# joeyz0z/ConZIC

Measured on AMD Instinct MI355X. Metric: captions/sec (L=10, K=200, seq order), higher is better.
Workload: dtype bf16

## Files before the change

conzic_amd/csrc/bridge.hip:

```cpp
#include "kernels.h"
#include "bridge_hash.h"

namespace czc {

constexpr int BR_THREADS = 64;
constexpr int BR_MAXB = 512;
constexpr int BR_MAXSYM = 64;
constexpr int BR_LEN = 77;
constexpr int BR_MAXP = 64;

__device__ __forceinline__ bool merge_lookup(const BridgeDev& bd, int l, int r, unsigned& rank, int& out) {
  const unsigned long long key = ((unsigned long long)(unsigned)l << 32) | (unsigned)r;
  unsigned h = bridge_hash(key) & bd.hmask;
  for (;;) {
    const unsigned long long k = bd.hkeys[h];
    if (k == key) {
      const unsigned long long v = bd.hvals[h];
      rank = (unsigned)(v >> 32);
      out = (int)(v & 0xFFFFFFFFu);
      return true;
    }
    if (k == ~0ull) return false;
    h = (h + 1) & bd.hmask;
  }
// ... 90 lines not shown
    if (j == 0) {
      j = i + 1;
      if (c == 0) { while (j < n && (cls[j] & 3) == 0) ++j; }
      else if (c == 1) { while (j < n && !(cls[j] & 4)) ++j; }
      else { while (j < n && (cls[j] & 3) == 2) ++j; }
    }
    if (bd.tok_bpe_len && c == 0) {
      while (pp < np && pl_beg[pp] < i) ++pp;
      if (pp < np && pl_beg[pp] == i && pl_end[pp] == j) {
        const int id = pl_id[pp];
        const int tl = bd.tok_bpe_len[id];
        if (tl) {
          for (int q = 0; q < tl && nt < BR_LEN - 2; ++q) outp[1 + nt++] = bd.tok_bpe[id * BR_TOKMAX + q];
          i = j;
          continue;
        }
      }
    }
    int m = j - i;
    if (m > BR_MAXSYM) { ovf = true; m = BR_MAXSYM; }
    for (int q = 0; q < m; ++q) sym[q] = bd.byte_sym[txt[i + q]];
    sym[m - 1] = bd.byte_sym_eow[txt[i + m - 1]];
    while (m > 1) {
      unsigned best = 0xFFFFFFFFu;
      int bi = -1, bo = 0;
      for (int q = 0; q + 1 < m; ++q) {
        unsigned rk; int o;
        if (merge_lookup(bd, sym[q], sym[q + 1], rk, o) && rk < best) { best = rk; bi = q; bo = o; }
      }
      if (bi < 0) break;
      sym[bi] = bo;
      for (int q = bi + 1; q + 1 < m; ++q) sym[q] = sym[q + 1];
      --m;
    }
    for (int q = 0; q < m && nt < BR_LEN - 2; ++q) outp[1 + nt++] = sym[q];
    i = j;
  }
  outp[1 + nt] = bd.eos_id;
  for (int q = nt + 2; q < BR_LEN; ++q) outp[q] = bd.eos_id;
  clip_len[row] = nt + 2;
  if (pos.tag_of_token) {
    for (int w = n_words; w < pos.n; ++w) pos_ok += (pos.masks[w] & 0x8000u) ? 1 : 0;
    if (senti_raw) senti_raw[row] = (float)pos_ok / (float)pos.n;
  } else if (senti_raw) {
    senti_raw[row] = negative ? -senti : senti;
  }
  if (repeats) repeats[row] = (float)(rep - 1);
  if (ovf) atomicAdd(overflow, 1);
}

__global__ void bridge_precompute_kernel(BridgeDev bd, int* tok_ids, uint8_t* tok_len) {
  const int id = blockIdx.x * blockDim.x + threadIdx.x;
  if (id >= bd.bert_vocab) return;
  tok_len[id] = 0;
  const unsigned o0 = bd.piece_off[id], o1 = bd.piece_off[id + 1];
  int m = (int)(o1 - o0);
  if (m <= 0 || m > BR_MAXSYM || (bd.piece_flags[id] & 1u)) return;
  for (unsigned o = o0; o < o1; ++o)
    if ((bd.piece_class[o] & 3) != 0) return;
  int sym[BR_MAXSYM];
  for (int q = 0; q < m; ++q) sym[q] = bd.byte_sym[bd.piece_bytes[o0 + q]];
  sym[m - 1] = bd.byte_sym_eow[bd.piece_bytes[o0 + m - 1]];
  while (m > 1) {
    unsigned best = 0xFFFFFFFFu;
    int bi = -1, bo = 0;
    for (int q = 0; q + 1 < m; ++q) {
      unsigned rk; int o;
      if (merge_lookup(bd, sym[q], sym[q + 1], rk, o) && rk < best) { best = rk; bi = q; bo = o; }
    }
    if (bi < 0) break;
    sym[bi] = bo;
    for (int q = bi + 1; q + 1 < m; ++q) sym[q] = sym[q + 1];
    --m;
  }
  if (m > BR_TOKMAX) return;
  for (int q = 0; q < m; ++q) tok_ids[id * BR_TOKMAX + q] = sym[q];
  tok_len[id] = (uint8_t)m;
}

int launch_bridge_precompute(const BridgeDev& bd, int* tok_ids, uint8_t* tok_len, hipStream_t st) {
  hipLaunchKernelGGL(bridge_precompute_kernel, dim3(cdiv(bd.bert_vocab, 64)), dim3(64), 0, st, bd, tok_ids, tok_len);
  CZC_HIP_CHECK(hipGetLastError());
  return 0;
}

template <bool ROWS, bool HP>
static int launch_bridge_t(const BridgeDev& bd, const int* inp, int B, int T, int gen_idx, const int* gen_rows, const int* row_len, const int* cand, int K,
                           const float* lexicon, const float* lex_pos, const uint8_t* lex_cls, int negative, const RowHyper* hp_rows, const PosDev& pos,
                           int* clip_ids, int* clip_len, float* senti_raw, float* repeats, int* overflow_flag, hipStream_t st) {
  const long rows = (long)B * K;
  if (rows <= 0) return 0;
  const size_t shmem = (size_t)BR_THREADS * (2 * BR_MAXB + BR_MAXSYM * 4 + BR_MAXP * 8);
  CZC_HIP_CHECK(hipFuncSetAttribute((const void*)bridge_kernel<ROWS, HP>, hipFuncAttributeMaxDynamicSharedMemorySize, (int)shmem));
  hipLaunchKernelGGL((bridge_kernel<ROWS, HP>), dim3(cdiv(rows, BR_THREADS)), dim3(BR_THREADS), shmem, st, bd, inp, B, T, gen_idx, gen_rows,
                     row_len, cand, K, lexicon, lex_pos, lex_cls, negative, hp_rows, pos, clip_ids, clip_len, senti_raw, repeats, overflow_flag);
  CZC_HIP_CHECK(hipGetLastError());
  return 0;
}

int launch_bridge(const BridgeDev& bd, const int* inp, int B, int T, int gen_idx, const int* cand, int K,
                  const float* lexicon, const float* lex_pos, const uint8_t* lex_cls, int negative, const PosDev& pos, int* clip_ids, int* clip_len, float* senti_raw,
                  float* repeats, int* overflow_flag, hipStream_t st) {
  return launch_bridge_t<false, false>(bd, inp, B, T, gen_idx, nullptr, nullptr, cand, K, lexicon, lex_pos, lex_cls, negative, nullptr, pos, clip_ids, clip_len,
                                senti_raw, repeats, overflow_flag, st);
}

int launch_bridge_rows(const BridgeDev& bd, const int* inp, int B, int T, const int* gen_rows, const int* cand, int K,
                       const float* lexicon, const float* lex_pos, const uint8_t* lex_cls, int negative, const PosDev& pos, int* clip_ids, int* clip_len,
                       float* senti_raw, float* repeats, int* overflow_flag, hipStream_t st, const int* row_len) {
  if (!gen_rows || !cand) { snprintf(g_err, sizeof(g_err), "bridge: the per-row form needs gen_rows and cand"); return 1; }
  return launch_bridge_t<true, false>(bd, inp, B, T, 0, gen_rows, row_len, cand, K, lexicon, lex_pos, lex_cls, negative, nullptr, pos, clip_ids, clip_len,
                               senti_raw, repeats, overflow_flag, st);
}

int launch_bridge_rows_hp(const BridgeDev& bd, const int* inp, int B, int T, const int* gen_rows, const int* cand, int K,
                          const float* lexicon, const float* lex_pos, const uint8_t* lex_cls, const RowHyper* hp_rows, const PosDev& pos,
                          int* clip_ids, int* clip_len, float* senti_raw, float* repeats, int* overflow_flag, hipStream_t st,
                          const int* row_len) {
  if (!gen_rows || !cand || !hp_rows) { snprintf(g_err, sizeof(g_err), "bridge: the per-row form needs gen_rows, cand and hp_rows"); return 1; }
  return launch_bridge_t<true, true>(bd, inp, B, T, 0, gen_rows, row_len, cand, K, lexicon, lex_pos, lex_cls, 0, hp_rows, pos, clip_ids, clip_len,
                                     senti_raw, repeats, overflow_flag, st);
}

__global__ __launch_bounds__(1024) void scan_kernel(const int* len, int n, int* off, int* totals) {
  __shared__ int part[1024];
  __shared__ int pmax[1024];
  const int tid = threadIdx.x;
  const int per = (n + 1023) / 1024;
  const int lo = tid * per, hi = min(n, lo + per);
  int s = 0, mx = 0;
  for (int i = lo; i < hi; ++i) { s += len[i]; mx = max(mx, len[i]); }
  part[tid] = s;
  pmax[tid] = mx;
  __syncthreads();
  for (int o = 1; o < 1024; o <<= 1) {
    const int v = tid >= o ? part[tid - o] : 0;
    const int w = tid >= o ? pmax[tid - o] : 0;
    __syncthreads();
    part[tid] += v;
    pmax[tid] = max(pmax[tid], w);
    __syncthreads();
  }
  int run = part[tid] - s;
  for (int i = lo; i < hi; ++i) { off[i] = run; run += len[i]; }
  if (tid == 1023) { off[n] = part[1023]; totals[0] = part[1023]; totals[1] = pmax[1023]; }
}

int launch_scan(const int* len, int n, int* off, int* totals, hipStream_t st) {
  hipLaunchKernelGGL(scan_kernel, dim3(1), dim3(1024), 0, st, len, n, off, totals);
  CZC_HIP_CHECK(hipGetLastError());
  return 0;
}

__global__ __launch_bounds__(256) void prefix_plan_kernel(const int* cids, const int* clen, int B, int K, int share,
                                                          int* own_len, int* pre_len, int* seg_src, int* seg_pos0,
                                                          int* max_len_out, int* img_max, int* rep, int* n_dup_out) {
  __shared__ int s_p, s_max, s_keys, s_dup;
  __shared__ unsigned long long s_hash[1024];
  __shared__ short s_len[1024];
  const int b = blockIdx.x, tid = threadIdx.x;
  if (tid == 0) { s_p = 1 << 30; s_max = 0; s_keys = 0; s_dup = 0; }
  __syncthreads();
  const int* r0 = cids + (long)b * K * BR_LEN;
  const int l0 = clen[b * K];
  int p = 1 << 30, mx = 0;
  for (int k = tid; k < K; k += blockDim.x) {
    const int* rk = r0 + (long)k * BR_LEN;
    const int lk = clen[b * K + k];
    const int lim = min(lk, l0);
    int c = 0;
    while (c < lim && rk[c] == r0[c]) ++c;
    p = min(p, min(c, lk - 1));
    mx = max(mx, lk);
    if (rep) {
      unsigned long long h = 1469598103934665603ull ^ (unsigned)lk;
      for (int c2 = 0; c2 < lk; ++c2) { h ^= (unsigned)rk[c2]; h *= 1099511628211ull; }
      s_hash[k] = h;
      s_len[k] = (short)lk;
    }
  }
  atomicMin(&s_p, p);
  atomicMax(&s_max, mx);
  __syncthreads();
  const int pb = share ? s_p : 0;
  if (tid == 0) {
    own_len[b] = pb; pre_len[b] = 0; seg_src[b] = b * K; seg_pos0[b] = 0;
    atomicMax(max_len_out, s_max);
    atomicMax(max_len_out + 1, s_max - pb);
    if (img_max) img_max[b] = s_max - pb;
  }
  int keys = 0;
  int dups = 0;
  for (int k = tid; k < K; k += blockDim.x) {
    const int s = B + b * K + k;
    const int lk = clen[b * K + k];
    int own = lk - pb;
    if (rep) {
      int r = k;
      const unsigned long long hk = s_hash[k];
      const int* rk = r0 + (long)k * BR_LEN;
      for (int j = 0; j < k; ++j) {
        if (s_hash[j] != hk || s_len[j] != lk) continue;
        const int* rj = r0 + (long)j * BR_LEN;
        int c = pb;
        while (c < lk && rj[c] == rk[c]) ++c;
        if (c == lk) { r = j; break; }
      }
      rep[b * K + k] = r;
      if (r != k) { own = 0; ++dups; }
    }
    own_len[s] = own;
    pre_len[s] = pb;
    seg_src[s] = b * K + k;
    seg_pos0[s] = pb;
    keys += own * pb + own * (own + 1) / 2;
  }
  atomicAdd(&s_keys, keys);
  if (dups) atomicAdd(&s_dup, dups);
  __syncthreads();
  if (tid == 0) {
    atomicAdd(max_len_out + 4, s_keys + pb * (pb + 1) / 2);
    if (n_dup_out && s_dup) atomicAdd(n_dup_out, s_dup);
  }
}

int launch_prefix_plan(const int* clip_ids, const int* clip_len, int B, int K, int share, int* own_len, int* pre_len,
                       int* seg_src, int* seg_pos0, int* max_len_out, int* img_max, hipStream_t st, int* rep, int* n_dup_out) {
  if (rep && K > 1024) { snprintf(g_err, sizeof(g_err), "prefix plan: de-duplication needs K <= 1024"); return 1; }
  hipLaunchKernelGGL(prefix_plan_kernel, dim3(B), dim3(256), 0, st, clip_ids, clip_len, B, K, share, own_len, pre_len,
                     seg_src, seg_pos0, max_len_out, img_max, rep, n_dup_out);
  CZC_HIP_CHECK(hipGetLastError());
  return 0;
}

__global__ void prefix_finish_kernel(const int* own_off, const int* own_len, int B, int K, int* pre_off, int* eos_idx,
                                     int* n_trunk_rows, const int* rep) {
  const int i = blockIdx.x * blockDim.x + threadIdx.x;
  if (i == 0 && n_trunk_rows) *n_trunk_rows = own_off[B];
  if (i < B) pre_off[i] = 0;
  if (i < B * K) {
    const int s = B + i;
    pre_off[s] = own_off[i / K];
    const int sr = rep ? B + (i / K) * K + rep[i] : s;
    eos_idx[i] = own_off[sr] + own_len[sr] - 1;
  }
}

int launch_prefix_finish(const int* own_off, const int* own_len, int B, int K, int* pre_off, int* eos_idx,
                         int* n_trunk_rows, hipStream_t st, const int* rep) {
  hipLaunchKernelGGL(prefix_finish_kernel, dim3(cdiv((long)B * K, 256)), dim3(256), 0, st, own_off, own_len, B, K,
                     pre_off, eos_idx, n_trunk_rows, rep);
  CZC_HIP_CHECK(hipGetLastError());
  return 0;
}

__device__ __forceinline__ int layer0_rep(const int* cid, const int* own, int pb, int k, int i) {
  const int id = cid[(long)k * BR_LEN + pb + i];
  for (int j = 0; j < k; ++j)
    if (own[j] > i && cid[(long)j * BR_LEN + pb + i] == id) return j;
  return k;
}

__global__ __launch_bounds__(256) void layer0_count_kernel(const int* cids, const int* own_len, const int* pre_len, int B, int K,
                                                           int* dcount, int* total) {
  __shared__ int s_n;
  const int b = blockIdx.x;
  if (threadIdx.x == 0) s_n = 0;
  __syncthreads();
  const int* cid = cids + (long)b * K * BR_LEN;
  const int* own = own_len + B + b * K;
  const int pb = pre_len[B + b * K];
  int n = 0;
  for (int k = threadIdx.x; k < K; k += blockDim.x)
    for (int i = 0; i < min(own[k], 32); ++i) n += layer0_rep(cid, own, pb, k, i) == k;
  if (n) atomicAdd(&s_n, n);
  __syncthreads();
  if (threadIdx.x == 0) { dcount[b] = s_n; if (s_n) atomicAdd(total, s_n); }
}

int launch_layer0_count(const int* clip_ids, const int* own_len, const int* pre_len, int B, int K, int* dcount, int* total, hipStream_t st) {
  hipLaunchKernelGGL(layer0_count_kernel, dim3(B), dim3(256), 0, st, clip_ids, own_len, pre_len, B, K, dcount, total);
  CZC_HIP_CHECK(hipGetLastError());
  return 0;
}

__global__ __launch_bounds__(256) void layer0_map_kernel(const int* cids, const int* own_off, const int* own_len, const int* pre_len,
                                                         const int* dcount, int B, int K, int* rowmap, int* dist) {
  __shared__ unsigned s_mask[1024];
  __shared__ int s_pref[1024];
  __shared__ int s_base;
  const int b = blockIdx.x;
  if (threadIdx.x == 0) s_base = own_off[B];
  __syncthreads();
  {
    int n = 0;
    for (int j = threadIdx.x; j < b; j += blockDim.x) n += dcount[j];
    if (n) atomicAdd(&s_base, n);
  }
  for (int r = own_off[b] + threadIdx.x; r < own_off[b] + own_len[b]; r += blockDim.x) { rowmap[r] = r; dist[r] = r; }
  const int* cid = cids + (long)b * K * BR_LEN;
  const int* own = own_len + B + b * K;
  const int* off = own_off + B + b * K;
  const int pb = pre_len[B + b * K];
  for (int k = threadIdx.x; k < K; k += blockDim.x) {
    unsigned m = 0;
    for (int i = 0; i < min(own[k], 32); ++i) m |= (unsigned)(layer0_rep(cid, own, pb, k, i) == k) << i;
    s_mask[k] = m;
  }
  __syncthreads();
  if (threadIdx.x == 0) {
    int run = 0;
    for (int k = 0; k < K; ++k) { s_pref[k] = run; run += __popc(s_mask[k]); }
  }
  __syncthreads();
  const int base = s_base;
  for (int k = threadIdx.x; k < K; k += blockDim.x) {
    for (int i = 0; i < min(own[k], 32); ++i) {
      const int j = (s_mask[k] >> i) & 1 ? k : layer0_rep(cid, own, pb, k, i);
      const int c = base + s_pref[j] + __popc(s_mask[j] & ((1u << i) - 1u));
      rowmap[off[k] + i] = c;
      if (j == k) dist[c] = off[k] + i;
    }
  }
}

int launch_layer0_map(const int* clip_ids, const int* own_off, const int* own_len, const int* pre_len, const int* dcount, int B, int K,
                      int* rowmap, int* dist, hipStream_t st) {
  if (K > 1024) { snprintf(g_err, sizeof(g_err), "layer-0 row map: K <= 1024"); return 1; }
  hipLaunchKernelGGL(layer0_map_kernel, dim3(B), dim3(256), 0, st, clip_ids, own_off, own_len, pre_len, dcount, B, K, rowmap, dist);
  CZC_HIP_CHECK(hipGetLastError());
  return 0;
}

__global__ __launch_bounds__(256) void refine_plan_kernel(const int* clen, const int* trunk_len, const int* list, const int* count,
                                                          const int* count_off, const int* kr, int B, int K, int* own_len, int* pre_len,
                                                          int* seg_src, int* seg_pos0, int* rlist, int* max_len_out, int* img_max) {
  __shared__ int s_mxb;
  const int b = blockIdx.x, tid = threadIdx.x;
  if (tid == 0) s_mxb = 0;
  __syncthreads();
  const int n = count[b], o = count_off[b], Kr = *kr;
  const int pb = n > 0 ? trunk_len[b] : 0;
  if (tid == 0) { own_len[b] = pb; pre_len[b] = 0; seg_src[b] = b * K; seg_pos0[b] = 0; }
  int mx = 0, mxb = 0;
  for (int i = tid; i < Kr; i += blockDim.x) {
    const int s = B + b * Kr + i;
    if (i >= n) {
      pre_len[s] = pb; seg_src[s] = b * K; seg_pos0[s] = pb;
      continue;
    }
    const int flat = b * K + list[(long)b * K + i];
    const int len = clen[flat];
    own_len[s] = len - pb;
    pre_len[s] = pb;
    seg_src[s] = flat;
    seg_pos0[s] = pb;
    rlist[o + i] = flat;
    mx = max(mx, len);
    mxb = max(mxb, len - pb);
    atomicAdd(max_len_out + 4, (len - pb) * pb + (len - pb) * (len - pb + 1) / 2);
  }
  if (tid == 0 && n > 0) atomicAdd(max_len_out + 4, pb * (pb + 1) / 2);
  if (mx) { atomicMax(max_len_out, mx); atomicMax(max_len_out + 1, mxb); atomicMax(&s_mxb, mxb); }
  __syncthreads();
  if (tid == 0 && img_max) img_max[b] = s_mxb;
}

int launch_refine_plan(const int* clip_len, const int* trunk_len, const int* list, const int* count, const int* count_off,
                       const int* kr_dev, int B, int K, int* own_len, int* pre_len, int* seg_src, int* seg_pos0, int* rlist,
                       int* max_len_out, int* img_max, hipStream_t st) {
  hipLaunchKernelGGL(refine_plan_kernel, dim3(B), dim3(256), 0, st, clip_len, trunk_len, list, count, count_off, kr_dev, B, K, own_len,
                     pre_len, seg_src, seg_pos0, rlist, max_len_out, img_max);
  CZC_HIP_CHECK(hipGetLastError());
  return 0;
}

__global__ void refine_finish_kernel(const int* own_off, const int* own_len, const int* count, const int* count_off, const int* kr,
                                     int B, int* pre_off, int* eos_idx) {
  const int i = blockIdx.x * blockDim.x + threadIdx.x;
  const int Kr = *kr;
  if (i < B) pre_off[i] = 0;
  if (i < B * Kr) {
    const int b = i / Kr, j = i - b * Kr;
    const int s = B + i;
    pre_off[s] = own_off[b];
    if (j < count[b]) eos_idx[count_off[b] + j] = own_off[s] + own_len[s] - 1;
  }
}

int launch_refine_finish(const int* own_off, const int* own_len, const int* count, const int* count_off, const int* kr_dev, int B, int K,
                         int* pre_off, int* eos_idx, hipStream_t st) {
  hipLaunchKernelGGL(refine_finish_kernel, dim3(cdiv((long)B * K, 256)), dim3(256), 0, st, own_off, own_len, count, count_off, kr_dev, B,
                     pre_off, eos_idx);
  CZC_HIP_CHECK(hipGetLastError());
  return 0;
}

}
```

conzic_amd/csrc/engine.hip:

```cpp
#include <algorithm>
#include <map>
#include <string>
#include <vector>
#include <cmath>
#include <cstddef>
#include <cstring>

#include "../../include/conzic_hip.h"
#include "kernels.h"
#include "bridge_hash.h"

namespace czc {
thread_local char g_err[512] = {0};
thread_local int g_gemm_family = 0;
}
using namespace czc;

namespace {

struct Tensor {
  float* p = nullptr;
  std::vector<int64_t> shape;
  size_t numel = 0;
};

struct LayerW {
  void* qkv_w = nullptr; float* qkv_b = nullptr;
  void* o_w = nullptr; float* o_b = nullptr;
  float *ln1_g = nullptr, *ln1_b = nullptr;
  void* fc1_w = nullptr; float* fc1_b = nullptr;
  void* fc2_w = nullptr; float* fc2_b = nullptr;
  float *ln2_g = nullptr, *ln2_b = nullptr;
  void *qkv_wf = nullptr, *fc1_wf = nullptr;
  float *qkv_bf = nullptr, *fc1_bf = nullptr;
};

struct Buf {
  void* p = nullptr;
  size_t bytes = 0;
};

struct ProfKind {
  std::vector<hipEvent_t> ev;
  size_t used = 0;
  double flops = 0;
  int64_t launches = 0;
};

struct RowRecords {
  const RowHyper* hp = nullptr;
  const RowDraw* draw = nullptr; unsigned step = 0;
  const int* rival = nullptr; const float* delta = nullptr; int M = 0;
  const float* img_all = nullptr; int n_img = 0;
  const int* vset = nullptr; const unsigned* vbits = nullptr; int vwords = 0; const RowHyper* vhp = nullptr;
};

}

struct czc_engine {
  czc_config cfg;
  int dev = 0;
  hipStream_t st = nullptr;
  bool shares_weights = false;
  hipEvent_t prof_ref = nullptr;
  char err[512] = {0};
  bool finalized = false;
  size_t esz = 2;
  int pb = PREC_F32, pc = PREC_BF16;
  int pv = PREC_BF16;
  size_t eb = 4;
  bool refine = false;
  float refine_theta_x = 2.0f;
  float refine_theta_gen = 4.0f;
  bool in_generate = false;
  int refine_samples = 12;
  int refine_samples_step = 24;
  float refine_guard_dev = 2.0e-4f;
  float guard_max_dev = 0.f; int64_t guard_trips = 0;
  float refine_gate_delta = 4.0e-4f;
  int refine_rows16 = 1;
  float refine_rows16_factor = 1.75f;
  bool gate_now = false, gate_need_cos = true;
  int64_t stat_gated = 0, stat_gate_images = 0;

  std::map<std::string, Tensor> w;
  std::vector<LayerW> bert, ctext, cvis, ctext_x;
  void* mlm_dense_w = nullptr; void* decoder_w = nullptr; void* tproj_w = nullptr; void* vproj_w = nullptr;
  void* patch_w = nullptr; void* tproj_wx = nullptr;

  std::map<std::string, Buf> ws;
  float* d_mask = nullptr; int mask_vocab = 0;
  float* d_lex = nullptr;
  float* d_lex_pos = nullptr; uint8_t* d_lex_cls = nullptr;
  uint8_t* d_pos_tags = nullptr; uint16_t* d_pos_masks = nullptr; int pos_n = 0;
  BridgeDev bd; bool has_bridge = false;
  std::vector<void*> bridge_allocs;
  float* d_img_n = nullptr; int img_B = 0;
  float logit_scale_exp = 1.f;
  double plan_pairs = 0;
  int* h_totals = nullptr;
  int last_BT = 0, last_B = 0, last_T = 0;
  int bert_prune = 1;
  int bert_pruned_idx = -1;
  const int32_t* bert_pruned_rows = nullptr;
  int bert_fuse_splitk_ln = 1;
  int share_prefix = 1;
  int dedup = 1;
  float* d_staged = nullptr; int staged_cap = 0, staged_n = 0;
  int pack_branches = 1;
  int pool_last_layer = 1;
  int share_layer0 = 1;
  int pool_last_qkv = 1;
  int fuse_ln = 1;
  int resid16 = 1;
  int fold_ln = 1;
  int prof = 0;
  std::map<std::string, ProfKind> pk;
  int64_t stat_clip_rows = 0, stat_clip_seqs = 0, stat_bert_rows = 0, stat_steps = 0;
  int64_t stat_refine_rows = 0, stat_refine_seqs = 0;
  int64_t stat_dedup_seqs = 0;
  czc_control_fn ctl_fn = nullptr; void* ctl_user = nullptr;
  int32_t* h_ctl_ids = nullptr; float* h_ctl_scores = nullptr; size_t h_ctl_cap = 0;
  int memo = 0;
  RowRecords rec;
  int memo_branch_floor = 0;
  int64_t stat_memo_hits = 0, stat_memo_images = 0;
  int memo_rows = 0;
  int64_t stat_memo_row_hits = 0, stat_memo_row_steps = 0;
  int32_t* h_memo_list = nullptr; size_t h_memo_list_cap = 0;
  split_t* d_index = nullptr; int64_t index_n = 0;
  int index_groups = 0;
  int fluency_chunk = 1024;
  int regions_chunk = 64;
};

namespace {

constexpr int PRUNED_ROWS = 1 << 30;

#define E_CHECK(expr)                                                                         \
  do {                                                                                        \
    int _r = (expr);                                                                          \
    if (_r) {                                                                                 \
      if (!e->err[0]) snprintf(e->err, sizeof(e->err), "%s", czc::g_err);                     \
      return _r;                                                                              \
    }                                                                                         \
  } while (0)

#define E_HIP(expr)                                                                           \
  do {                                                                                        \
    hipError_t _h = (expr);                                                                   \
    if (_h != hipSuccess) {                                                                   \
      snprintf(e->err, sizeof(e->err), "%s:%d %s -> %s", __FILE__, __LINE__, #expr,           \
               hipGetErrorString(_h));                                                        \
      return CZC_ERR_HIP;                                                                     \
    }                                                                                         \
  } while (0)

int fail(czc_engine* e, int code, const char* fmt, const char* a = "") {
  snprintf(e->err, sizeof(e->err), fmt, a);
  return code;
}

int ensure(czc_engine* e, const char* name, size_t bytes, void** out) {
  Buf& b = e->ws[name];
  if (b.bytes < bytes) {
    if (b.p) {
      E_HIP(hipStreamSynchronize(e->st));
      E_HIP(hipFree(b.p));
    }
    size_t want = bytes + bytes / 4 + 256;
    E_HIP(hipMalloc(&b.p, want));
    b.bytes = want;
  }
  *out = b.p;
  return 0;
}

struct ProfScope {
  czc_engine* e;
  ProfKind* k = nullptr;
  ProfScope(czc_engine* e_, const char* kind, double flops) : e(e_) {
    if (!e->prof) return;
    if (e->prof == 2 && strncmp(kind, "gemm_clip_text", 14) != 0 && strcmp(kind, "gemm_clip_refine") != 0 &&
        !strstr(kind, "_clip_text")) return;
    k = &e->pk[kind];
    if (k->used + 2 > k->ev.size()) {
      for (int i = 0; i < 2; ++i) {
        hipEvent_t ev;
        if (hipEventCreate(&ev) != hipSuccess) { k = nullptr; return; }
        k->ev.push_back(ev);
      }
    }
    k->flops += flops;
    k->launches += 1;
    (void)hipEventRecord(k->ev[k->used], e->st);
  }
  ~ProfScope() {
    if (!k) return;
    (void)hipEventRecord(k->ev[k->used + 1], e->st);
    k->used += 2;
  }
};

const Tensor* find(czc_engine* e, const std::string& n) {
  auto it = e->w.find(n);
  return it == e->w.end() ? nullptr : &it->second;
}

int need(czc_engine* e, const std::string& n, size_t numel, float** out) {
  const Tensor* t = find(e, n);
  if (!t) return fail(e, CZC_ERR_STATE, "missing tensor %s", n.c_str());
  if (t->numel != numel) return fail(e, CZC_ERR_STATE, "tensor %s has the wrong size", n.c_str());
  *out = t->p;
  return 0;
}

int to_act(czc_engine* e, int prec, const float* src, size_t numel, void** out) {
  void* p = nullptr;
  E_HIP(hipMalloc(&p, numel * prec_bytes(prec)));
  E_CHECK(launch_convert(prec, src, p, (long)numel, e->st));
  *out = p;
  return 0;
}

int build_layers(czc_engine* e, std::vector<LayerW>& L, int n_layers, int H, int I, bool bert_style,
                 const std::string& prefix, int prec) {
  const size_t es = prec_bytes(prec);
  L.resize(n_layers);
  for (int n = 0; n < n_layers; ++n) {
    LayerW& l = L[n];
    std::string p = prefix + std::to_string(n);
    std::string q, k, v, o, ln1, fc1, fc2, ln2;
    if (bert_style) {
      q = p + ".attention.self.query"; k = p + ".attention.self.key"; v = p + ".attention.self.value";
      o = p + ".attention.output.dense"; ln1 = p + ".attention.output.LayerNorm";
      fc1 = p + ".intermediate.dense"; fc2 = p + ".output.dense"; ln2 = p + ".output.LayerNorm";
    } else {
      q = p + ".self_attn.q_proj"; k = p + ".self_attn.k_proj"; v = p + ".self_attn.v_proj";
      o = p + ".self_attn.out_proj"; ln1 = p + ".layer_norm1";
      fc1 = p + ".mlp.fc1"; fc2 = p + ".mlp.fc2"; ln2 = p + ".layer_norm2";
    }
    float *qw, *kw, *vw, *qb, *kb, *vb, *t;
    E_CHECK(need(e, q + ".weight", (size_t)H * H, &qw));
    E_CHECK(need(e, k + ".weight", (size_t)H * H, &kw));
    E_CHECK(need(e, v + ".weight", (size_t)H * H, &vw));
    E_CHECK(need(e, q + ".bias", H, &qb));
    E_CHECK(need(e, k + ".bias", H, &kb));
    E_CHECK(need(e, v + ".bias", H, &vb));
    E_HIP(hipMalloc(&l.qkv_w, (size_t)3 * H * H * es));
    char* base = (char*)l.qkv_w;
    E_CHECK(launch_convert(prec, qw, base, (long)H * H, e->st));
    E_CHECK(launch_convert(prec, kw, base + (size_t)H * H * es, (long)H * H, e->st));
    E_CHECK(launch_convert(prec, vw, base + (size_t)2 * H * H * es, (long)H * H, e->st));
    E_HIP(hipMalloc((void**)&l.qkv_b, (size_t)3 * H * 4));
    E_HIP(hipMemcpyAsync(l.qkv_b, qb, (size_t)H * 4, hipMemcpyDeviceToDevice, e->st));
    E_HIP(hipMemcpyAsync(l.qkv_b + H, kb, (size_t)H * 4, hipMemcpyDeviceToDevice, e->st));
    E_HIP(hipMemcpyAsync(l.qkv_b + 2 * H, vb, (size_t)H * 4, hipMemcpyDeviceToDevice, e->st));
    E_CHECK(need(e, o + ".weight", (size_t)H * H, &t)); E_CHECK(to_act(e, prec, t, (size_t)H * H, &l.o_w));
    E_CHECK(need(e, o + ".bias", H, &l.o_b));
    E_CHECK(need(e, ln1 + ".weight", H, &l.ln1_g)); E_CHECK(need(e, ln1 + ".bias", H, &l.ln1_b));
    E_CHECK(need(e, fc1 + ".weight", (size_t)I * H, &t)); E_CHECK(to_act(e, prec, t, (size_t)I * H, &l.fc1_w));
    E_CHECK(need(e, fc1 + ".bias", I, &l.fc1_b));
    E_CHECK(need(e, fc2 + ".weight", (size_t)H * I, &t)); E_CHECK(to_act(e, prec, t, (size_t)H * I, &l.fc2_w));
    E_CHECK(need(e, fc2 + ".bias", H, &l.fc2_b));
    E_CHECK(need(e, ln2 + ".weight", H, &l.ln2_g)); E_CHECK(need(e, ln2 + ".bias", H, &l.ln2_b));
  }
  return 0;
}

int gemm(czc_engine* e, int prec, const char* kind, const void* A, int lda, const void* W, int ldw, const float* bias,
         const float* resid, int ldr, void* out_act, float* out_f32, int ldc, int M, int N, int K, int act) {
  GemmArgs g;
  g.A = A; g.lda = lda; g.W = W; g.ldw = ldw; g.bias = bias; g.resid = resid; g.ldr = ldr;
  g.out_act = out_act; g.out_f32 = out_f32; g.ldc = ldc; g.M = M; g.N = N; g.K = K; g.act = act;
  ProfScope ps(e, kind, 2.0 * M * (double)N * K);
  E_CHECK(launch_gemm(prec, g, e->st));
  return 0;
}

int gemm_x16(czc_engine* e, int prec, const char* kind, const void* A, int lda, const void* W, const float* bias, void* x16, int M,
             int N, int K, float* part = nullptr, long part_ld = 0) {
  GemmArgs g;
  g.A = A; g.lda = lda; g.W = W; g.ldw = K; g.bias = bias; g.resid = (const float*)x16; g.ldr = N;
  g.out_act = nullptr; g.out_f32 = (float*)x16; g.ldc = N; g.M = M; g.N = N; g.K = K; g.act = ACT_NONE; g.x16 = 1;
  g.row_part = part; g.part_ld = part_ld;
  ProfScope ps(e, kind, 2.0 * M * (double)N * K);
  E_CHECK(launch_gemm(prec, g, e->st));
  return 0;
}

int gemm_ex(czc_engine* e, int prec, const char* kind, const GemmArgs& g) {
  ProfScope ps(e, kind, 2.0 * g.M * (double)g.N * g.K);
  E_CHECK(launch_gemm(prec, g, e->st));
  return 0;
}

struct Layer0Rows { const int* rowmap = nullptr; const int* dist = nullptr; int n = 0; };

int clip_stack(czc_engine* e, int P, const char* gk, std::vector<LayerW>& L, float* x, int M, int H, int I, int heads,
               float eps, const SegTable& tab, int max_keys, int causal, int plan_B = 0, int plan_K = 0,
               int plan_max_own = 0, const int* pool_idx = nullptr, int n_pool = 0, float** pooled = nullptr, bool r16 = false,
               const float* ln_stat0 = nullptr, const Layer0Rows& l0 = Layer0Rows(), const int* pool_rep = nullptr) {
  const size_t esz = prec_bytes(P);
  void *y, *qkv, *ctx, *hbuf;
  E_CHECK(ensure(e, "cs_y", (size_t)M * H * esz, &y));
  E_CHECK(ensure(e, "cs_qkv", (size_t)M * 3 * H * esz, &qkv));
  E_CHECK(ensure(e, "cs_ctx", (size_t)M * H * esz, &ctx));
  E_CHECK(ensure(e, "cs_h", (size_t)M * I * esz, &hbuf));
  const float scale = 1.0f / sqrtf(64.0f);
  const bool text = !strcmp(gk, "gemm_clip_text") || !strcmp(gk, "gemm_clip_refine");
  const char* ak = text ? "attention_clip_text" : "attention";
  const char* rk = text ? "rowops_clip_text" : "rowops";
  const double attn_flops = text ? 4.0 * H * e->plan_pairs : 0.0;
  const bool rowln = !r16 && prec_is_half(P) && e->fuse_ln && H == 512 && M >= g_rowln_min_m && I % 32 == 0;
  const bool fold = r16 && e->fold_ln && !L.empty() && L[0].qkv_wf && ln_stat0;
  float *part = nullptr, *stat = nullptr;
  if (fold) {
    E_CHECK(ensure(e, "cs_part", (size_t)(H / 32) * M * 8, (void**)&part));
    E_CHECK(ensure(e, "cs_stat", (size_t)M * 8 + 256, (void**)&stat));
  }
  auto finalize = [&](int rows, int N) -> int {
    if (gemm_wreg_stats_in_kernel(rows, N)) return 0;
    ProfScope ps(e, rk, 0);
    E_CHECK(launch_ln_finalize(part, M, H / 32, rows, eps, stat, e->st));
    return 0;
  };
  auto folded_gemm = [&](const void* Ax, const void* Wf, const float* bf, const float* st_, void* out, int rows, int N,
                         int act, int ldc = 0) -> int {
    GemmArgs g;
    g.A = Ax; g.lda = H; g.W = Wf; g.ldw = H; g.bias = bf; g.resid = nullptr; g.ldr = 0; g.out_act = out; g.out_f32 = nullptr; g.ldc = ldc ? ldc : N;
    g.M = rows; g.N = N; g.K = H; g.act = act;
    g.ln_stat = st_ ? st_ : stat;
    if (!st_ && gemm_wreg_stats_in_kernel(rows, N)) { g.ln_part = part; g.ln_part_ld = M; g.ln_eps = eps; }
    ProfScope ps(e, gk, 2.0 * rows * (double)N * H);
    E_CHECK(launch_gemm(P, g, e->st));
    return 0;
  };
  auto ln = [&](const float* gm, const float* bt, int rows, const void* src, void* dst) -> int {
    ProfScope ps(e, rk, 0);
    if (r16) E_CHECK(launch_layernorm_x16(P, src, nullptr, gm, bt, eps, rows, H, dst, e->st));
    else E_CHECK(launch_layernorm(P, (const float*)src, nullptr, gm, bt, eps, rows, H, dst, nullptr, e->st));
    return 0;
  };
  auto resid_gemm = [&](const void* A, int lda, const void* W, const float* b, int K) -> int {
    if (r16) return gemm_x16(e, P, gk, A, lda, W, b, x, M, H, K);
    return gemm(e, P, gk, A, lda, W, K, b, x, H, nullptr, x, H, M, H, K, ACT_NONE);
  };
  auto resid_ln_gemm = [&](const void* A, int lda, const void* W, const float* b, int K, const float* gm,
                           const float* bt) -> int {
    GemmArgs g;
    g.A = A; g.lda = lda; g.W = W; g.ldw = K; g.bias = b; g.resid = x; g.ldr = H; g.out_act = y; g.out_f32 = x;
    g.ldc = H; g.M = M; g.N = H; g.K = K; g.act = ACT_NONE; g.f16 = P == PREC_F16;
    g.ln_gamma = gm; g.ln_beta = bt; g.ln_eps = eps;
    ProfScope ps(e, gk, 2.0 * M * (double)H * K);
    E_CHECK(launch_gemm_rowln(g, e->st));
    return 0;
  };
  const bool pool_qkv = pool_idx && e->pool_last_layer && e->pool_last_qkv && fold && plan_B > 0 && n_pool == plan_B * plan_K &&
                        prec_is_half(P) && g_use_mfma_attention && e->pack_branches &&
                        attention_image_serves(plan_B, plan_K, plan_max_own, max_keys, heads);
  bool have_y = false;
  for (size_t n = 0; n < L.size(); ++n) {
    LayerW& l = L[n];
    if (pool_qkv && n + 1 == L.size()) {
      void *ctx_e, *q_e, *h_e; float *x_e, *stat_e;
      E_CHECK(ensure(e, "cs_ctx_e", (size_t)n_pool * H * esz, &ctx_e));
      E_CHECK(ensure(e, "cs_q_e", (size_t)n_pool * H * esz, &q_e));
      E_CHECK(ensure(e, "cs_h_e", (size_t)n_pool * I * esz, &h_e));
      E_CHECK(ensure(e, "cs_x_e", (size_t)n_pool * H * 4, (void**)&x_e));
      E_CHECK(ensure(e, "cs_stat_e", (size_t)n_pool * 8 + 256, (void**)&stat_e));
      const float* st_all = n == 0 ? ln_stat0 : stat;
      { ProfScope ps(e, rk, 0);
        E_CHECK(launch_gather_rows_bytes(x, pool_idx, n_pool, H * 2, x_e, e->st));
        E_CHECK(launch_gather_rows_w32(st_all, pool_idx, n_pool, 2, stat_e, e->st)); }
      E_CHECK(folded_gemm(x, (const char*)l.qkv_wf + (size_t)H * H * 2, l.qkv_bf + H, st_all, (char*)qkv + (size_t)H * esz, M, 2 * H,
                          ACT_NONE, 3 * H));
      E_CHECK(folded_gemm(x_e, l.qkv_wf, l.qkv_bf, stat_e, q_e, n_pool, H, ACT_NONE));
      { ProfScope ps(e, ak, attn_flops);
        E_CHECK(launch_attention_image_pooled(qkv, q_e, tab, pool_rep, plan_B, plan_K, plan_max_own, max_keys, heads, scale, ctx_e,
                                              e->st, P == PREC_F16)); }
      E_CHECK(gemm_x16(e, P, gk, ctx_e, H, l.o_w, l.o_b, x_e, n_pool, H, H, part, M));
      E_CHECK(finalize(n_pool, I));
      E_CHECK(folded_gemm(x_e, l.fc1_wf, l.fc1_bf, nullptr, h_e, n_pool, I, ACT_QUICK_GELU));
      E_CHECK(gemm_x16(e, P, gk, h_e, I, l.fc2_w, l.fc2_b, x_e, n_pool, H, I));
      *pooled = x_e;
      return 0;
    }
    const bool l0_rows = fold && n == 0 && l0.n > 0;
    if (l0_rows) {
      void* xg; float* sg;
      E_CHECK(ensure(e, "cs_xg", (size_t)l0.n * H * 2, &xg));
      E_CHECK(ensure(e, "cs_sg", (size_t)l0.n * 8 + 256, (void**)&sg));
      { ProfScope ps(e, rk, 0);
        E_CHECK(launch_gather_rows_bytes(x, l0.dist, l0.n, H * 2, xg, e->st));
        E_CHECK(launch_gather_rows_w32(ln_stat0, l0.dist, l0.n, 2, sg, e->st)); }
      E_CHECK(folded_gemm(xg, l.qkv_wf, l.qkv_bf, sg, qkv, l0.n, 3 * H, ACT_NONE));
    } else if (fold) {
      E_CHECK(folded_gemm(x, l.qkv_wf, l.qkv_bf, n == 0 ? ln_stat0 : nullptr, qkv, M, 3 * H, ACT_NONE));
    } else {
      if (!have_y) E_CHECK(ln(l.ln1_g, l.ln1_b, M, x, y));
      E_CHECK(gemm(e, P, gk, y, H, l.qkv_w, H, l.qkv_b, nullptr, 0, qkv, nullptr, 3 * H, M, 3 * H, H, ACT_NONE));
    }
    { ProfScope ps(e, ak, attn_flops);
      int rc = -1;
      if (l0_rows)
        rc = launch_attention_shared_mapped(qkv, l0.n, l0.rowmap, tab, plan_B, plan_K, plan_max_own, max_keys, heads, scale, ctx, e->st,
                                            P == PREC_F16);
      else if (plan_B > 0 && prec_is_half(P) && g_use_mfma_attention && e->pack_branches)
        rc = launch_attention_shared(qkv, tab, plan_B, plan_K, plan_max_own, max_keys, heads, scale, ctx, e->st, P == PREC_F16);
      else if (plan_B > 0 && P == PREC_F16X3 && g_use_mfma_attention && e->pack_branches)
        rc = launch_attention_shared_split(qkv, tab, plan_B, plan_K, plan_max_own, max_keys, heads, scale, ctx, e->st);
      if (rc > 0) E_CHECK(rc);
      if (rc < 0) E_CHECK(launch_attention(P, qkv, tab, max_keys, heads, causal, scale, ctx, e->st)); }
    if (pool_idx && n + 1 == L.size() && e->pool_last_layer) {
      void *ctx_e, *y_e, *h_e; float* x_e;
      E_CHECK(ensure(e, "cs_ctx_e", (size_t)n_pool * H * esz, &ctx_e));
      E_CHECK(ensure(e, "cs_y_e", (size_t)n_pool * H * esz, &y_e));
      E_CHECK(ensure(e, "cs_h_e", (size_t)n_pool * I * esz, &h_e));
      E_CHECK(ensure(e, "cs_x_e", (size_t)n_pool * H * 4, (void**)&x_e));
      { ProfScope ps(e, rk, 0);
        E_CHECK(launch_gather_rows_bytes(ctx, pool_idx, n_pool, H * (int)esz, ctx_e, e->st));
        if (r16) E_CHECK(launch_gather_rows_bytes(x, pool_idx, n_pool, H * 2, x_e, e->st));
        else E_CHECK(launch_gather_rows_f32(x, pool_idx, n_pool, H, x_e, e->st)); }
      if (fold) {
        E_CHECK(gemm_x16(e, P, gk, ctx_e, H, l.o_w, l.o_b, x_e, n_pool, H, H, part, M));
        E_CHECK(finalize(n_pool, I));
        E_CHECK(folded_gemm(x_e, l.fc1_wf, l.fc1_bf, nullptr, h_e, n_pool, I, ACT_QUICK_GELU));
      } else {
        if (r16) E_CHECK(gemm_x16(e, P, gk, ctx_e, H, l.o_w, l.o_b, x_e, n_pool, H, H));
        else E_CHECK(gemm(e, P, gk, ctx_e, H, l.o_w, H, l.o_b, x_e, H, nullptr, x_e, H, n_pool, H, H, ACT_NONE));
        E_CHECK(ln(l.ln2_g, l.ln2_b, n_pool, x_e, y_e));
        E_CHECK(gemm(e, P, gk, y_e, H, l.fc1_w, H, l.fc1_b, nullptr, 0, h_e, nullptr, I, n_pool, I, H, ACT_QUICK_GELU));
      }
      if (r16) E_CHECK(gemm_x16(e, P, gk, h_e, I, l.fc2_w, l.fc2_b, x_e, n_pool, H, I));
      else E_CHECK(gemm(e, P, gk, h_e, I, l.fc2_w, I, l.fc2_b, x_e, H, nullptr, x_e, H, n_pool, H, I, ACT_NONE));
      *pooled = x_e;
      return 0;
    }
    if (fold) {
      E_CHECK(gemm_x16(e, P, gk, ctx, H, l.o_w, l.o_b, x, M, H, H, part, M));
      E_CHECK(finalize(M, I));
      E_CHECK(folded_gemm(x, l.fc1_wf, l.fc1_bf, nullptr, hbuf, M, I, ACT_QUICK_GELU));
      const bool more = n + 1 < L.size();
      E_CHECK(gemm_x16(e, P, gk, hbuf, I, l.fc2_w, l.fc2_b, x, M, H, I, more ? part : nullptr, M));
      if (more && pool_qkv && n + 2 == L.size()) {
        ProfScope ps(e, rk, 0);
        E_CHECK(launch_ln_finalize(part, M, H / 32, M, eps, stat, e->st));
      } else if (more) E_CHECK(finalize(M, 3 * H));
      continue;
    }
    if (rowln) E_CHECK(resid_ln_gemm(ctx, H, l.o_w, l.o_b, H, l.ln2_g, l.ln2_b));
    else {
      E_CHECK(resid_gemm(ctx, H, l.o_w, l.o_b, H));
      E_CHECK(ln(l.ln2_g, l.ln2_b, M, x, y));
    }
    E_CHECK(gemm(e, P, gk, y, H, l.fc1_w, H, l.fc1_b, nullptr, 0, hbuf, nullptr, I, M, I, H, ACT_QUICK_GELU));
    have_y = rowln && e->fuse_ln >= 2 && n + 1 < L.size();
    if (have_y) E_CHECK(resid_ln_gemm(hbuf, I, l.fc2_w, l.fc2_b, I, L[n + 1].ln1_g, L[n + 1].ln1_b));
    else E_CHECK(resid_gemm(hbuf, I, l.fc2_w, l.fc2_b, I));
  }
  return 0;
}

struct Ragged { const int* off; const int* len; int M; int max_T; };

int bert_forward(czc_engine* e, const int* d_inp, int B, int T, int keep_idx = -1, const int* keep_rows = nullptr,
                 const int32_t* keep_rows_host = nullptr, const Ragged* rag = nullptr) {
  const czc_config& c = e->cfg;
  const int P = e->pb, M = rag ? rag->M : B * T, H = c.bert_hidden, I = c.bert_inter;
  if (rag && keep_idx >= 0 && !keep_rows) return fail(e, CZC_ERR_STATE, "ragged BERT rows keep a row per sequence (keep_rows)%s");
  void *xa, *qkv, *ctx, *hbuf; float *x, *tmp;
  E_CHECK(ensure(e, "b_x", (size_t)M * H * 4, (void**)&x));
  E_CHECK(ensure(e, "b_tmp", (size_t)M * H * 4, (void**)&tmp));
  E_CHECK(ensure(e, "b_xa", (size_t)M * H * e->eb, &xa));
  E_CHECK(ensure(e, "b_qkv", (size_t)M * 3 * H * e->eb, &qkv));
  E_CHECK(ensure(e, "b_ctx", (size_t)M * H * e->eb, &ctx));
  E_CHECK(ensure(e, "b_h", (size_t)M * I * e->eb, &hbuf));
  float *word, *pos, *typ, *g, *b;
  E_CHECK(need(e, "bert.embeddings.word_embeddings.weight", (size_t)c.bert_vocab * H, &word));
  E_CHECK(need(e, "bert.embeddings.position_embeddings.weight", (size_t)c.bert_max_pos * H, &pos));
  E_CHECK(need(e, "bert.embeddings.token_type_embeddings.weight", (size_t)2 * H, &typ));
  E_CHECK(need(e, "bert.embeddings.LayerNorm.weight", H, &g));
  E_CHECK(need(e, "bert.embeddings.LayerNorm.bias", H, &b));
  { ProfScope ps(e, "rowops", 0);
    if (rag) E_CHECK(launch_bert_embed_ragged(P, d_inp, T, nullptr, rag->off, rag->len, B, rag->max_T, H, word, pos, typ, g, b, c.bert_eps, xa, x, e->st));
    else E_CHECK(launch_bert_embed(P, d_inp, B, T, H, word, pos, typ, g, b, c.bert_eps, xa, x, e->st)); }
  const float scale = 1.0f / sqrtf(64.0f);
  e->bert_pruned_idx = -1;
  e->bert_pruned_rows = nullptr;
  auto fc2_ln = [&](const void* h, LayerW& l, float* xr, int rows) -> int {
    SplitkPending pend;
    GemmArgs g;
    g.A = h; g.lda = I; g.W = l.fc2_w; g.ldw = I; g.bias = l.fc2_b; g.resid = xr; g.ldr = H; g.out_act = nullptr; g.out_f32 = tmp; g.ldc = H;
    g.M = rows; g.N = H; g.K = I; g.act = ACT_NONE;
    g.splitk_pending = e->bert_fuse_splitk_ln ? &pend : nullptr;
    E_CHECK(gemm_ex(e, P, "gemm_bert", g));
    ProfScope ps(e, "rowops", 0);
    if (pend.nslab > 0) E_CHECK(launch_layernorm_splitk(P, pend, l.fc2_b, xr, H, l.ln2_g, l.ln2_b, c.bert_eps, rows, H, xa, xr, e->st));
    else E_CHECK(launch_layernorm(P, tmp, nullptr, l.ln2_g, l.ln2_b, c.bert_eps, rows, H, xa, xr, e->st));
    return 0;
  };
  for (int n = 0; n < c.bert_layers; ++n) {
    LayerW& l = e->bert[n];
    E_CHECK(gemm(e, P, "gemm_bert", xa, H, l.qkv_w, H, l.qkv_b, nullptr, 0, qkv, nullptr, 3 * H, M, 3 * H, H, ACT_NONE));
    { ProfScope ps(e, "attention", 0);
      SegTable tab{nullptr, nullptr, rag ? rag->off : nullptr, rag ? rag->len : nullptr, B, rag ? 0 : T};
      E_CHECK(launch_attention(P, qkv, tab, rag ? rag->max_T : T, c.bert_heads, 0, scale, ctx, e->st)); }
    if (keep_idx >= 0 && n + 1 == c.bert_layers) {
      int* idx; void* ctx_g; float* x_g;
      E_CHECK(ensure(e, "b_pidx", (size_t)B * 4, (void**)&idx));
      E_CHECK(ensure(e, "b_cg", (size_t)B * H * e->eb, &ctx_g));
      E_CHECK(ensure(e, "b_xg", (size_t)B * H * 4, (void**)&x_g));
      { ProfScope ps(e, "rowops", 0);
        if (rag) E_CHECK(launch_ragged_row_index(idx, B, rag->off, keep_rows, e->st));
        else if (keep_rows) E_CHECK(launch_make_row_index_rows(idx, B, T, keep_rows, e->st));
        else E_CHECK(launch_make_row_index(idx, B, T, keep_idx, e->st));
        E_CHECK(launch_gather_rows_bytes(ctx, idx, B, H * (int)e->eb, ctx_g, e->st));
        E_CHECK(launch_gather_rows_f32(x, idx, B, H, x_g, e->st)); }
      E_CHECK(gemm(e, P, "gemm_bert", ctx_g, H, l.o_w, H, l.o_b, x_g, H, nullptr, tmp, H, B, H, H, ACT_NONE));
      { ProfScope ps(e, "rowops", 0); E_CHECK(launch_layernorm(P, tmp, nullptr, l.ln1_g, l.ln1_b, c.bert_eps, B, H, xa, x_g, e->st)); }
      E_CHECK(gemm(e, P, "gemm_bert", xa, H, l.fc1_w, H, l.fc1_b, nullptr, 0, hbuf, nullptr, I, B, I, H, ACT_GELU_ERF));
      E_CHECK(fc2_ln(hbuf, l, x_g, B));
      e->bert_pruned_idx = keep_rows ? PRUNED_ROWS : keep_idx;
      e->bert_pruned_rows = keep_rows ? keep_rows_host : nullptr;
      break;
    }
    E_CHECK(gemm(e, P, "gemm_bert", ctx, H, l.o_w, H, l.o_b, x, H, nullptr, tmp, H, M, H, H, ACT_NONE));
    { ProfScope ps(e, "rowops", 0); E_CHECK(launch_layernorm(P, tmp, nullptr, l.ln1_g, l.ln1_b, c.bert_eps, M, H, xa, x, e->st)); }
    E_CHECK(gemm(e, P, "gemm_bert", xa, H, l.fc1_w, H, l.fc1_b, nullptr, 0, hbuf, nullptr, I, M, I, H, ACT_GELU_ERF));
    E_CHECK(fc2_ln(hbuf, l, x, M));
  }
  return 0;
}

int mlm_head(czc_engine* e, int B, int T, int gen_idx, float** logits_out, const int* gen_rows = nullptr,
             const int32_t* gen_rows_host = nullptr, const Ragged* rag = nullptr) {
  const czc_config& c = e->cfg;
  const int P = e->pb, H = c.bert_hidden, V = c.bert_vocab;
  float* x = (float*)e->ws["b_x"].p;
  int* idx; float *gx, *t32, *logits; void *ga, *ta;
  E_CHECK(ensure(e, "h_idx", (size_t)B * 4, (void**)&idx));
  E_CHECK(ensure(e, "h_gx", (size_t)B * H * 4, (void**)&gx));
  E_CHECK(ensure(e, "h_ga", (size_t)B * H * e->eb, &ga));
  E_CHECK(ensure(e, "h_t32", (size_t)B * H * 4, (void**)&t32));
  E_CHECK(ensure(e, "h_ta", (size_t)B * H * e->eb, &ta));
  E_CHECK(ensure(e, "b_logits", (size_t)B * V * 4, (void**)&logits));
  float *db, *g, *b, *bias;
  E_CHECK(need(e, "cls.predictions.transform.dense.bias", H, &db));
  E_CHECK(need(e, "cls.predictions.transform.LayerNorm.weight", H, &g));
  E_CHECK(need(e, "cls.predictions.transform.LayerNorm.bias", H, &b));
  E_CHECK(need(e, "cls.predictions.bias", V, &bias));
  const bool kept_same = gen_rows ? (e->bert_pruned_idx == PRUNED_ROWS && e->bert_pruned_rows && gen_rows_host &&
                                     !memcmp(e->bert_pruned_rows, gen_rows_host, (size_t)B * 4))
                                  : e->bert_pruned_idx == gen_idx;
  if (e->bert_pruned_idx >= 0 && !kept_same)
    return fail(e, CZC_ERR_STATE, "n_mask=0 re-use of a forward that kept one row only (it follows an n_mask >= 2 step, gen_utils.py:164-166)%s");
  { ProfScope ps(e, "rowops", 0);
    if (e->bert_pruned_idx >= 0) {
      gx = (float*)e->ws["b_xg"].p;
    } else {
      if (rag && !gen_rows) return fail(e, CZC_ERR_STATE, "ragged BERT rows are read by a row per sequence (gen_rows)%s");
      if (rag) E_CHECK(launch_ragged_row_index(idx, B, rag->off, gen_rows, e->st));
      else if (gen_rows) E_CHECK(launch_make_row_index_rows(idx, B, T, gen_rows, e->st));
      else E_CHECK(launch_make_row_index(idx, B, T, gen_idx, e->st));
      E_CHECK(launch_gather_rows_f32(x, idx, B, H, gx, e->st));
    }
    E_CHECK(launch_convert(P, gx, ga, (long)B * H, e->st)); }
  E_CHECK(gemm(e, P, "gemm_bert", ga, H, e->mlm_dense_w, H, db, nullptr, 0, nullptr, t32, H, B, H, H, ACT_GELU_ERF));
  { ProfScope ps(e, "rowops", 0); E_CHECK(launch_layernorm(P, t32, nullptr, g, b, c.bert_eps, B, H, ta, nullptr, e->st)); }
  E_CHECK(gemm(e, P, "gemm_bert", ta, H, e->decoder_w, H, bias, nullptr, 0, nullptr, logits, V, B, V, H, ACT_NONE));
  *logits_out = logits;
  return 0;
}

constexpr int HT_PLAN = 48;
constexpr int PLAN_TOTALS = 48;
struct PlanBufs { int *own_len, *pre_len, *src, *pos0, *own_off, *pre_off, *eidx, *img_max, *rep; };

static inline bool refine_rows16_now(const czc_engine* e) {
  return e->refine && e->in_generate && e->refine_rows16 && e->cfg.clip_hidden == 512;
}

int plan_bufs(czc_engine* e, int B, int K, PlanBufs* p, const char* pfx = "p") {
  const int n_seq = B * K, S = B + n_seq;
  const std::string q(pfx);
  E_CHECK(ensure(e, (q + "_own_len").c_str(), (size_t)S * 4, (void**)&p->own_len));
  E_CHECK(ensure(e, (q + "_pre_len").c_str(), (size_t)S * 4, (void**)&p->pre_len));
  E_CHECK(ensure(e, (q + "_src").c_str(), (size_t)S * 4, (void**)&p->src));
  E_CHECK(ensure(e, (q + "_pos0").c_str(), (size_t)S * 4, (void**)&p->pos0));
  E_CHECK(ensure(e, (q + "_own_off").c_str(), (size_t)(S + 1) * 4, (void**)&p->own_off));
  E_CHECK(ensure(e, (q + "_pre_off").c_str(), (size_t)S * 4, (void**)&p->pre_off));
  E_CHECK(ensure(e, (q + "_eidx").c_str(), (size_t)n_seq * 4, (void**)&p->eidx));
  E_CHECK(ensure(e, (q + "_img_max").c_str(), (size_t)B * 4, (void**)&p->img_max));
  E_CHECK(ensure(e, (q + "_rep").c_str(), (size_t)n_seq * 4, (void**)&p->rep));
  return 0;
}

int clip_plan(czc_engine* e, const int* cids, const int* clen, int B, int K, int share, int* totals) {
  PlanBufs p;
  E_CHECK(plan_bufs(e, B, K, &p));
  const int S = B + B * K;
  { ProfScope ps(e, "bridge", 0);
    int* rep = e->dedup && share && K > 1 ? p.rep : nullptr;
    E_CHECK(launch_prefix_plan(cids, clen, B, K, share, p.own_len, p.pre_len, p.src, p.pos0, totals + 3, p.img_max, e->st, rep, totals + 5));
    E_CHECK(launch_scan(p.own_len, S, p.own_off, totals, e->st));
    E_CHECK(launch_prefix_finish(p.own_off, p.own_len, B, K, p.pre_off, p.eidx, totals + 6, e->st, rep));
    if (e->share_layer0 && share && K > 1 && K <= 1024 && e->fold_ln && e->pack_branches) {
      int* dcount;
      E_CHECK(ensure(e, "p_dcount", (size_t)B * 4, (void**)&dcount));
      E_CHECK(launch_layer0_count(cids, p.own_len, p.pre_len, B, K, dcount, totals + 8, e->st));
    } }
  E_HIP(hipMemcpyAsync(e->h_totals + HT_PLAN, totals, PLAN_TOTALS, hipMemcpyDeviceToHost, e->st));
  int* flag;
  E_CHECK(ensure(e, "s_nonfinite", 32, (void**)&flag));
  E_HIP(hipMemcpyAsync(e->h_totals + 8, flag, 4, hipMemcpyDeviceToHost, e->st));
  return 0;
}

int clip_tower_on(czc_engine* e, int P, std::vector<LayerW>& L, const void* tproj, const char* gk, const int* cids,
                  const PlanBufs& p, int n_seg, int n_pool, int M, int max_len, int plan_B, int plan_K, int max_branch,
                  const char* feat_name, float** feat_out, int n_dist = 0, const int* rep = nullptr) {
  const czc_config& c = e->cfg;
  const int H = c.clip_hidden;
  float *x, *feat, *tok, *pos, *fg, *fb; void* pa;
  E_CHECK(ensure(e, "c_x", (size_t)M * H * 4, (void**)&x));
  E_CHECK(ensure(e, "c_pa", (size_t)n_pool * H * prec_bytes(P), &pa));
  E_CHECK(ensure(e, feat_name, (size_t)n_pool * c.clip_proj * 4, (void**)&feat));
  E_CHECK(need(e, "text_model.embeddings.token_embedding.weight", (size_t)c.clip_vocab * H, &tok));
  E_CHECK(need(e, "text_model.embeddings.position_embedding.weight", (size_t)c.clip_max_pos * H, &pos));
  E_CHECK(need(e, "text_model.final_layer_norm.weight", H, &fg));
  E_CHECK(need(e, "text_model.final_layer_norm.bias", H, &fb));
  const bool r16 = H == 512 && ((e->resid16 >= 1 && P == PREC_BF16) || (e->resid16 >= 2 && P == PREC_F16) ||
                                (P == PREC_F16 && refine_rows16_now(e)));
  float* stat0 = nullptr;
  if (r16 && e->fold_ln && !L.empty() && L[0].qkv_wf) E_CHECK(ensure(e, "c_stat0", (size_t)M * 8 + 256, (void**)&stat0));
  { ProfScope ps(e, "rowops_clip_text", 0);
    E_CHECK(launch_clip_embed(cids, CZC_CLIP_MAX_LEN, p.src, p.pos0, p.own_off, p.own_len, n_seg, max_len, H, tok, pos, x, e->st, r16 ? 1 : 0,
                              stat0, c.clip_eps)); }
  SegTable tab{p.pre_off, p.pre_len, p.own_off, p.own_len, n_seg, 0, plan_B > 0 ? p.img_max : nullptr};
  float* pooled = nullptr;
  Layer0Rows l0;
  if (n_dist > 0 && n_dist <= M && e->share_layer0 && stat0 && L.size() > 1 && plan_B > 0 && prec_is_half(P) && g_use_mfma_attention &&
      e->pack_branches && attention_image_serves(plan_B, plan_K, max_branch, max_len, c.clip_heads) &&
      (long)n_dist * 3 * H * 2 < (1L << 31)) {
    int *rowmap, *dist, *dcount;
    E_CHECK(ensure(e, "c_l0map", (size_t)M * 4, (void**)&rowmap));
    E_CHECK(ensure(e, "c_l0dist", (size_t)n_dist * 4, (void**)&dist));
    E_CHECK(ensure(e, "p_dcount", (size_t)plan_B * 4, (void**)&dcount));
    { ProfScope ps(e, "bridge", 0);
      E_CHECK(launch_layer0_map(cids, p.own_off, p.own_len, p.pre_len, dcount, plan_B, plan_K, rowmap, dist, e->st)); }
    l0.rowmap = rowmap; l0.dist = dist; l0.n = n_dist;
  }
  E_CHECK(clip_stack(e, P, gk, L, x, M, H, c.clip_inter, c.clip_heads, c.clip_eps, tab, max_len, 1, plan_B,
                     plan_K, max_branch, p.eidx, n_pool, &pooled, r16, stat0, l0, rep));
  { ProfScope ps(e, "rowops_clip_text", 0);
    if (r16) {
      if (pooled) E_CHECK(launch_layernorm_x16(P, pooled, nullptr, fg, fb, c.clip_eps, n_pool, H, pa, e->st));
      else E_CHECK(launch_layernorm_x16(P, x, p.eidx, fg, fb, c.clip_eps, n_pool, H, pa, e->st));
    } else if (pooled) E_CHECK(launch_layernorm(P, pooled, nullptr, fg, fb, c.clip_eps, n_pool, H, pa, nullptr, e->st));
    else E_CHECK(launch_layernorm(P, x, p.eidx, fg, fb, c.clip_eps, n_pool, H, pa, nullptr, e->st)); }
  E_CHECK(gemm(e, P, gk, pa, H, tproj, H, nullptr, nullptr, 0, nullptr, feat, c.clip_proj, n_pool, c.clip_proj, H, ACT_NONE));
  *feat_out = feat;
  return 0;
}

int clip_tower(czc_engine* e, const int* cids, int B, int K, int share, int M, int max_len, int max_branch, int n_trunk, int n_dist,
               float** feat_out, bool exact = false) {
  PlanBufs p;
  E_CHECK(plan_bufs(e, B, K, &p));
  const bool x = exact && e->refine;
  return clip_tower_on(e, x ? (int)PREC_F16X3 : e->pc, x ? e->ctext_x : e->ctext, x ? e->tproj_wx : e->tproj_w, "gemm_clip_text",
                       cids, p, B + B * K, B * K, M, max_len, B, K, max_branch, "c_feat", feat_out,
                       n_dist > 0 ? n_trunk + n_dist : 0, e->dedup && share && K > 1 ? p.rep : nullptr);
}

int read_totals(czc_engine* e, int* M, int* max_len, int* max_branch, int* n_trunk, int* n_dist) {
  const czc_config& c = e->cfg;
  const int* t = e->h_totals + HT_PLAN;
  *M = t[0]; *max_len = t[3]; *max_branch = t[4]; *n_trunk = t[6];
  *n_dist = t[8];
  if (e->memo_branch_floor > 32 && *max_branch < e->memo_branch_floor) *max_branch = e->memo_branch_floor;
  e->plan_pairs = (double)t[7];
  if (e->h_totals[8]) return fail(e, CZC_ERR_OVERFLOW, "non-finite CLIP cosine: an fp16 quantity overflowed in a tower (fp16 residual rows: set option resid16 = 0 on the bf16 engine, refine_rows16 = 0 on the refine engine; fp16 operands: use CZC_PREC_SPLIT)%s");
  if (t[2]) return fail(e, CZC_ERR_OVERFLOW, "text bridge overflow (row text > CZC_BRIDGE_MAX_BYTES)%s");
  if (*max_len > c.clip_max_pos || *max_len > CZC_CLIP_MAX_LEN)
    return fail(e, CZC_ERR_ARG, "CLIP sequence longer than max_position_embeddings%s");
  return 0;
}

int clip_text_forward(czc_engine* e, const int* cids, const int* clen, int B, int K, int share, int* totals,
                      float** feat_out, bool exact = false) {
  E_CHECK(clip_plan(e, cids, clen, B, K, share, totals));
  E_HIP(hipStreamSynchronize(e->st));
  int M, max_len, max_branch, n_trunk, n_dist;
  E_CHECK(read_totals(e, &M, &max_len, &max_branch, &n_trunk, &n_dist));
  E_CHECK(clip_tower(e, cids, B, K, share, M, max_len, max_branch, n_trunk, n_dist, feat_out, exact));
  e->stat_clip_rows += M;
  e->stat_clip_seqs += B * K;
  return 0;
}

struct StepArgs {
  int* d_inp; int B, T, gen_idx, n_mask, dot_allowed, K;
  czc_hyper hp;
  const int* gen_rows = nullptr; const int* dot_rows = nullptr; const int32_t* gen_rows_host = nullptr;
  const Ragged* rag = nullptr; int ctl_T = 0;
};
struct StepBufs { float *probs, *senti, *reps; int *idxs, *cand, *cids, *clen, *totals; };

int step_bufs(czc_engine* e, int n_seq, StepBufs* b) {
  E_CHECK(ensure(e, "s_probs", (size_t)n_seq * 4, (void**)&b->probs));
  E_CHECK(ensure(e, "s_idxs", (size_t)n_seq * 4, (void**)&b->idxs));
  E_CHECK(ensure(e, "s_cand", (size_t)n_seq * 4, (void**)&b->cand));
  E_CHECK(ensure(e, "s_cids", (size_t)n_seq * CZC_CLIP_MAX_LEN * 4, (void**)&b->cids));
  E_CHECK(ensure(e, "s_clen", (size_t)n_seq * 4, (void**)&b->clen));
  E_CHECK(ensure(e, "s_tot", PLAN_TOTALS, (void**)&b->totals));
  E_CHECK(ensure(e, "s_senti", (size_t)n_seq * 4, (void**)&b->senti));
  E_CHECK(ensure(e, "s_reps", (size_t)n_seq * 4, (void**)&b->reps));
  return 0;
}

int step_phase_a(czc_engine* e, const StepArgs& a) {
  const czc_config& c = e->cfg;
  const czc_hyper* hp = &a.hp;
  if (a.n_mask > 0) {
    const bool prune = e->bert_prune && a.n_mask == 1;
    if (a.gen_rows) {
      E_CHECK(launch_mask_positions_rows(a.d_inp, a.B, a.T, a.gen_rows, a.n_mask, c.mask_id, e->st));
      E_CHECK(bert_forward(e, a.d_inp, a.B, a.T, prune ? a.gen_idx : -1, prune ? a.gen_rows : nullptr, a.gen_rows_host, a.rag));
    } else {
      E_CHECK(launch_mask_positions(a.d_inp, a.B, a.T, a.gen_idx, a.n_mask, c.mask_id, e->st));
      E_CHECK(bert_forward(e, a.d_inp, a.B, a.T, prune ? a.gen_idx : -1));
    }
  }
  float* logits;
  E_CHECK(mlm_head(e, a.B, a.T, a.gen_idx, &logits, a.gen_rows, a.gen_rows_host, a.rag));
  StepBufs b;
  E_CHECK(step_bufs(e, a.B * a.K, &b));
  { ProfScope ps(e, "topk", 0);
    if (e->rec.vset) E_CHECK(launch_softmax_mask_topk_rows_vocab(logits, a.B, c.bert_vocab, a.K, e->d_mask, e->rec.hp ? e->rec.hp : e->rec.vhp, c.dot_id,
                                                                 a.dot_rows, e->rec.vset, e->rec.vbits, e->rec.vwords, b.probs, b.idxs, b.cand, e->st));
    else if (e->rec.hp) E_CHECK(launch_softmax_mask_topk_rows_hp(logits, a.B, c.bert_vocab, a.K, e->d_mask, e->rec.hp, c.dot_id, a.dot_rows,
                                                             b.probs, b.idxs, b.cand, e->st));
    else if (a.dot_rows) E_CHECK(launch_softmax_mask_topk_rows(logits, a.B, c.bert_vocab, a.K, e->d_mask, hp->temperature, c.dot_id, a.dot_rows,
                                                          b.probs, b.idxs, b.cand, e->st));
    else E_CHECK(launch_softmax_mask_topk(logits, a.B, c.bert_vocab, a.K, e->d_mask, hp->temperature, c.dot_id, a.dot_allowed,
                                          b.probs, b.idxs, b.cand, e->st)); }
  E_HIP(hipMemsetAsync(b.totals, 0, PLAN_TOTALS, e->st));
  { ProfScope ps(e, "bridge", 0);
    PosDev pos{hp->control == 2 ? e->d_pos_tags : nullptr, e->d_pos_masks, e->pos_n};
    if (e->rec.hp) E_CHECK(launch_bridge_rows_hp(e->bd, a.d_inp, a.B, a.T, a.gen_rows, b.cand, a.K, e->d_lex, e->d_lex_pos, e->d_lex_cls, e->rec.hp,
                                                  PosDev{e->d_pos_tags, e->d_pos_masks, e->pos_n}, b.cids, b.clen, b.senti, b.reps,
                                                  b.totals + 2, e->st, a.rag ? a.rag->len : nullptr));
    else if (a.gen_rows) E_CHECK(launch_bridge_rows(e->bd, a.d_inp, a.B, a.T, a.gen_rows, b.cand, a.K, hp->control == 1 ? e->d_lex : nullptr,
                                               hp->control == 1 ? e->d_lex_pos : nullptr, e->d_lex_cls, hp->negative,
                                               pos, b.cids, b.clen, b.senti, b.reps, b.totals + 2, e->st, a.rag ? a.rag->len : nullptr));
    else E_CHECK(launch_bridge(e->bd, a.d_inp, a.B, a.T, a.gen_idx, b.cand, a.K, hp->control == 1 ? e->d_lex : nullptr,
                               hp->control == 1 ? e->d_lex_pos : nullptr, e->d_lex_cls, hp->negative,
                               pos, b.cids, b.clen, b.senti, b.reps, b.totals + 2, e->st)); }
  E_CHECK(clip_plan(e, b.cids, b.clen, a.B, a.K, e->share_prefix, b.totals));
  return 0;
}

int control_pinned(czc_engine* e, size_t n_inp, size_t n_seq) {
  const size_t want = (n_inp + n_seq) * 4 + n_seq * 4;
  if (e->h_ctl_cap < want) {
    E_HIP(hipStreamSynchronize(e->st));
    if (e->h_ctl_ids) (void)hipHostFree(e->h_ctl_ids);
    e->h_ctl_ids = nullptr; e->h_ctl_cap = 0;
    E_HIP(hipHostMalloc((void**)&e->h_ctl_ids, want + want / 4));
    e->h_ctl_cap = want + want / 4;
  }
  e->h_ctl_scores = (float*)(e->h_ctl_ids + n_inp + n_seq);
  return 0;
}

int control_fetch(czc_engine* e, const StepArgs& a) {
  StepBufs b;
  const int Tc = a.ctl_T > 0 ? a.ctl_T : a.T;
  const size_t n_seq = (size_t)a.B * a.K, n_inp = (size_t)a.B * Tc;
  E_CHECK(step_bufs(e, (int)n_seq, &b));
  E_CHECK(control_pinned(e, n_inp, n_seq));
  if (Tc == a.T) E_HIP(hipMemcpyAsync(e->h_ctl_ids, a.d_inp, n_inp * 4, hipMemcpyDeviceToHost, e->st));
  else E_HIP(hipMemcpy2DAsync(e->h_ctl_ids, (size_t)Tc * 4, a.d_inp, (size_t)a.T * 4, (size_t)Tc * 4, a.B, hipMemcpyDeviceToHost, e->st));
  E_HIP(hipMemcpyAsync(e->h_ctl_ids + n_inp, b.cand, n_seq * 4, hipMemcpyDeviceToHost, e->st));
  return 0;
}

int control_score(czc_engine* e, const StepArgs& a) {
  StepBufs b;
  const int Tc = a.ctl_T > 0 ? a.ctl_T : a.T;
  const size_t n_seq = (size_t)a.B * a.K, n_inp = (size_t)a.B * Tc;
  E_CHECK(step_bufs(e, (int)n_seq, &b));
  memset(e->h_ctl_scores, 0, n_seq * 4);
  const int rc = e->ctl_fn(e->ctl_user, e->h_ctl_ids, e->h_ctl_ids + n_inp, a.B, Tc, a.K, a.gen_idx, e->h_ctl_scores);
  if (rc) return fail(e, CZC_ERR_STATE, "the control callback reported an error%s");
  E_HIP(hipMemcpyAsync(b.senti, e->h_ctl_scores, n_seq * 4, hipMemcpyHostToDevice, e->st));
  return 0;
}

int step_phase_b(czc_engine* e, const StepArgs& a, int M, int max_len, int max_branch, int n_trunk, int n_dist) {
  const czc_config& c = e->cfg;
  const czc_hyper* hp = &a.hp;
  const int n_seq = a.B * a.K;
// ... 1807 lines not shown
  { int* flag; E_CHECK(ensure(e, "s_nonfinite", 32, (void**)&flag)); E_HIP(hipMemsetAsync(flag, 0, 32, e->st)); }
  E_CHECK(ensure(e, "sc_rows", n * 4, (void**)&d_rows));
  E_CHECK(ensure(e, "sc_cos", (size_t)R * 4, (void**)&d_cos));
  E_HIP(hipMemcpyAsync(d_rows, rows, n * 4, hipMemcpyDefault, e->st));
  std::vector<int32_t> len_t;
  if (len_of_row_host) {
    len_t.resize(R);
    for (int r = 0; r < R; ++r) len_t[r] = seed_len + len_of_row_host[r] + 1;
    E_CHECK(ensure(e, "sc_len", (size_t)R * 4, (void**)&d_len));
    E_HIP(hipMemcpyAsync(d_len, len_t.data(), (size_t)R * 4, hipMemcpyHostToDevice, e->st));
  }
  if (image_of_row_host) {
    E_CHECK(ensure(e, "sc_ior", (size_t)R * 4, (void**)&d_ior));
    E_CHECK(ensure(e, "sc_img_r", (size_t)R * D * 4, (void**)&img_r));
    E_HIP(hipMemcpyAsync(d_ior, image_of_row_host, (size_t)R * 4, hipMemcpyHostToDevice, e->st));
    E_CHECK(launch_gather_rows_f32(e->d_img_n, d_ior, R, D, img_r, e->st));
  }
  int* d_rival = nullptr; float* d_disc = nullptr;
  if (rival_of_row_host) {
    E_CHECK(ensure(e, "sc_rival", (size_t)R * M * 4, (void**)&d_rival));
    E_CHECK(ensure(e, "sc_disc", (size_t)R * 4, (void**)&d_disc));
    E_HIP(hipMemcpyAsync(d_rival, rival_of_row_host, (size_t)R * M * 4, hipMemcpyHostToDevice, e->st));
  }
  E_CHECK(score_rows_device(e, d_rows, R, T, d_len, img_r, d_cos, d_rival, M, d_disc));
  if (out_cos) E_HIP(hipMemcpyAsync(out_cos, d_cos, (size_t)R * 4, hipMemcpyDefault, e->st));
  if (out_disc && d_disc) E_HIP(hipMemcpyAsync(out_disc, d_disc, (size_t)R * 4, hipMemcpyDefault, e->st));
  if (out_disc && !d_disc)
    for (int r = 0; r < R; ++r) out_disc[r] = 1.0f;
  E_HIP(hipMemcpyAsync(e->h_totals + 9, e->ws["s_nonfinite"].p, 4, hipMemcpyDeviceToHost, e->st));
  E_HIP(hipStreamSynchronize(e->st));
  if (e->h_totals[9]) return fail(e, CZC_ERR_OVERFLOW, "non-finite CLIP cosine: an fp16 quantity overflowed in a tower (fp16 residual rows: set option resid16 = 0 on the bf16 engine, refine_rows16 = 0 on the refine engine; fp16 operands: use CZC_PREC_SPLIT)%s");
  return CZC_OK;
}

int czc_fluency_rows(czc_engine* e, const int32_t* rows, int R, int T, int seed_len, const int32_t* len_of_row_host, float temperature,
                     float* out_logp, int32_t* out_rank, float* out_pll) {
  if (!e || !rows) return CZC_ERR_ARG;
  E_HIP(hipSetDevice(e->dev));
  e->err[0] = 0;
  if (R < 1 || R > CZC_MAX_ROWS || T < 1 || T > CZC_MAX_BERT_LEN || seed_len < 0 || T - seed_len - 1 < 1)
    return fail(e, CZC_ERR_ARG, "fluency_rows: R outside [1, CZC_MAX_ROWS], T outside [1, CZC_MAX_BERT_LEN], seed_len < 0 or T - seed_len - 1 < 1%s");
  if (!out_logp && !out_rank && !out_pll) return fail(e, CZC_ERR_ARG, "fluency_rows: every output is NULL%s");
  if (!std::isfinite(temperature) || !(temperature > 0.f)) return fail(e, CZC_ERR_ARG, "fluency_rows: temperature must be finite and > 0%s");
  const czc_config& c = e->cfg;
  const int Lmax = T - seed_len - 1, V = c.bert_vocab;
  bool dense = true;
  if (len_of_row_host)
    for (int r = 0; r < R; ++r) {
      if (len_of_row_host[r] < 1 || len_of_row_host[r] > Lmax) return fail(e, CZC_ERR_ARG, "fluency_rows: len_of_row outside [1, T - seed_len - 1]%s");
      dense = dense && len_of_row_host[r] == Lmax;
    }
  if (!e->finalized) return fail(e, CZC_ERR_STATE, "weights not finalized%s");
  if (c.bert_layers <= 0) return fail(e, CZC_ERR_STATE, "this engine was created without the BERT tower%s");
  const size_t n_ids = (size_t)R * T;
  std::vector<int32_t> host;
  const int32_t* h = rows;
  if (is_device_ptr(rows)) {
    host.resize(n_ids);
    E_HIP(hipMemcpyAsync(host.data(), rows, n_ids * 4, hipMemcpyDeviceToHost, e->st));
    E_HIP(hipStreamSynchronize(e->st));
    h = host.data();
  }
  for (int r = 0; r < R; ++r) {
    const int Tr = len_of_row_host ? seed_len + len_of_row_host[r] + 1 : T;
    for (int t = 0; t < Tr; ++t)
      if (h[(size_t)r * T + t] < 0 || h[(size_t)r * T + t] >= V) return fail(e, CZC_ERR_ARG, "fluency_rows: a row holds an id outside the BERT vocabulary%s");
  }
  std::vector<int32_t> tab((size_t)R * Lmax * 2);
  const int N = fluency_expand_tables(R, seed_len, Lmax, len_of_row_host, tab.data(), tab.data() + (size_t)R * Lmax);
  const int chunk = e->fluency_chunk, n_chunk = (N + chunk - 1) / chunk;
  {
    std::vector<int32_t> t2((size_t)5 * N + n_chunk + R);
    int32_t *ros = t2.data(), *cos_ = ros + N, *oidx = cos_ + N, *slen = oidx + N, *soff = slen + N, *lrow = soff + N + n_chunk;
    memcpy(ros, tab.data(), (size_t)N * 4);
    memcpy(cos_, tab.data() + (size_t)R * Lmax, (size_t)N * 4);
    for (int n = 0; n < N; ++n) {
      oidx[n] = ros[n] * Lmax + (cos_[n] - seed_len);
      slen[n] = len_of_row_host ? seed_len + len_of_row_host[ros[n]] + 1 : T;
    }
    for (int k = 0; k < n_chunk; ++k) {
      const int n0 = k * chunk, cn = std::min(chunk, N - n0);
      int32_t* off = soff + n0 + k;
      off[0] = 0;
      for (int i = 0; i < cn; ++i) off[i + 1] = off[i] + slen[n0 + i];
    }
    for (int r = 0; r < R; ++r) lrow[r] = len_of_row_host ? len_of_row_host[r] : Lmax;
    tab.swap(t2);
  }
  const int32_t *h_col = tab.data() + N, *h_slen = tab.data() + (size_t)3 * N, *h_soff = tab.data() + (size_t)4 * N;
  int *d_tab, *d_rows, *d_ids, *d_target, *d_gen, *d_rank, *flag; float *d_logp, *d_pll;
  E_CHECK(ensure(e, "s_nonfinite", 32, (void**)&flag));
  E_CHECK(ensure(e, "fl_tab", tab.size() * 4, (void**)&d_tab));
  E_CHECK(ensure(e, "fl_rows", n_ids * 4, (void**)&d_rows));
  E_CHECK(ensure(e, "fl_ids", (size_t)std::min(chunk, N) * T * 4, (void**)&d_ids));
  E_CHECK(ensure(e, "fl_target", (size_t)std::min(chunk, N) * 4, (void**)&d_target));
  E_CHECK(ensure(e, "fl_gen", (size_t)std::min(chunk, N) * 4, (void**)&d_gen));
  E_CHECK(ensure(e, "fl_logp", (size_t)R * Lmax * 4, (void**)&d_logp));
  E_CHECK(ensure(e, "fl_rank", (size_t)R * Lmax * 4, (void**)&d_rank));
  E_CHECK(ensure(e, "fl_pll", (size_t)R * 4, (void**)&d_pll));
  const int *d_ros = d_tab, *d_col = d_tab + N, *d_oidx = d_tab + (size_t)2 * N, *d_slen = d_tab + (size_t)3 * N,
            *d_soff = d_tab + (size_t)4 * N, *d_lrow = d_tab + (size_t)5 * N + n_chunk;
  struct EndReuse {
    czc_engine* e;
    ~EndReuse() { (void)hipStreamSynchronize(e->st); e->bert_pruned_idx = PRUNED_ROWS; e->bert_pruned_rows = nullptr; }
  } end_reuse{e};
  E_HIP(hipMemsetAsync(flag, 0, 32, e->st));
  E_HIP(hipMemcpyAsync(d_tab, tab.data(), tab.size() * 4, hipMemcpyHostToDevice, e->st));
  E_HIP(hipMemcpyAsync(d_rows, rows, n_ids * 4, hipMemcpyDefault, e->st));
  E_HIP(hipMemsetAsync(d_logp, 0, (size_t)R * Lmax * 4, e->st));
  E_HIP(hipMemsetAsync(d_rank, 0xff, (size_t)R * Lmax * 4, e->st));
  const bool prune = e->bert_prune != 0;
  for (int k = 0; k < n_chunk; ++k) {
    const int n0 = k * chunk, cn = std::min(chunk, N - n0);
    { ProfScope ps(e, "rowops", 0);
      E_CHECK(launch_expand_mask_rows(d_rows, T, d_ros + n0, d_col + n0, cn, c.mask_id, d_ids, d_target, d_gen, e->st)); }
    Ragged rag{d_soff + n0 + k, d_slen + n0, h_soff[n0 + k + cn], 0};
    for (int i = 0; i < cn; ++i) rag.max_T = std::max(rag.max_T, h_slen[n0 + i]);
    const Ragged* rg = dense ? nullptr : &rag;
    E_CHECK(bert_forward(e, d_ids, cn, T, prune ? h_col[n0] : -1, prune ? d_gen : nullptr, h_col + n0, rg));
    float* logits;
    E_CHECK(mlm_head(e, cn, T, h_col[n0], &logits, d_gen, h_col + n0, rg));
    { ProfScope ps(e, "topk", 0);
      E_CHECK(launch_logprob_target(logits, cn, V, d_target, temperature, d_oidx + n0, d_logp, d_rank, flag, e->st)); }
  }
  if (out_pll) {
    ProfScope ps(e, "rowops", 0);
    E_CHECK(launch_pll_sum(d_logp, R, Lmax, d_lrow, d_pll, e->st));
    E_HIP(hipMemcpyAsync(out_pll, d_pll, (size_t)R * 4, hipMemcpyDefault, e->st));
  }
  if (out_logp) E_HIP(hipMemcpyAsync(out_logp, d_logp, (size_t)R * Lmax * 4, hipMemcpyDefault, e->st));
  if (out_rank) E_HIP(hipMemcpyAsync(out_rank, d_rank, (size_t)R * Lmax * 4, hipMemcpyDefault, e->st));
  E_HIP(hipMemcpyAsync(e->h_totals + 9, flag, 4, hipMemcpyDeviceToHost, e->st));
  E_HIP(hipStreamSynchronize(e->st));
  if (e->h_totals[9]) return fail(e, CZC_ERR_OVERFLOW, "fluency_rows: non-finite log-probability (a non-finite BERT logit)%s");
  return CZC_OK;
}

int czc_set_control_callback(czc_engine* e, czc_control_fn fn, void* user) {
  if (!e) return CZC_ERR_ARG;
  e->ctl_fn = fn;
  e->ctl_user = fn ? user : nullptr;
  return CZC_OK;
}

int czc_set_option(czc_engine* e, const char* name, int value) {
  if (!e || !name) return CZC_ERR_ARG;
  if (!strcmp(name, "share_prefix")) { e->share_prefix = value ? 1 : 0; return CZC_OK; }
  if (!strcmp(name, "dedup")) { e->dedup = value ? 1 : 0; return CZC_OK; }
  if (!strcmp(name, "bert_prune")) { e->bert_prune = value ? 1 : 0; return CZC_OK; }
  if (!strcmp(name, "bert_fuse_splitk_ln")) { e->bert_fuse_splitk_ln = value ? 1 : 0; return CZC_OK; }
  if (!strcmp(name, "pack_branches")) { e->pack_branches = value ? 1 : 0; return CZC_OK; }
  if (!strcmp(name, "pool_last_layer")) { e->pool_last_layer = value ? 1 : 0; return CZC_OK; }
  if (!strcmp(name, "share_layer0")) { e->share_layer0 = value ? 1 : 0; return CZC_OK; }
  if (!strcmp(name, "pool_last_qkv")) { e->pool_last_qkv = value ? 1 : 0; return CZC_OK; }
  if (!strcmp(name, "fuse_ln")) { e->fuse_ln = value; return CZC_OK; }
  const auto fold_ready = [&]() -> int {
    if (e->finalized && wants_folded_ln(e) && (e->ctext.empty() || !e->ctext[0].qkv_wf))
      return fail(e, CZC_ERR_STATE, "option %s: this engine was finalized without the folded-LayerNorm operands (set it before czc_finalize_weights)", name);
    return CZC_OK;
  };
  if (!strcmp(name, "resid16")) { const int old = e->resid16; e->resid16 = value < 0 ? 0 : value; const int rc = fold_ready(); if (rc) e->resid16 = old; return rc; }
  if (!strcmp(name, "fold_ln")) { const int old = e->fold_ln; e->fold_ln = value ? 1 : 0; const int rc = fold_ready(); if (rc) e->fold_ln = old; return rc; }
  if (!strcmp(name, "refine_samples")) { e->refine_samples = value < 0 ? 0 : value; return CZC_OK; }
  if (!strcmp(name, "refine_samples_step")) { e->refine_samples_step = value < 0 ? 0 : value; return CZC_OK; }
  if (!strcmp(name, "refine_theta_x1000")) { e->refine_theta_x = (float)value / 1000.f; return CZC_OK; }
  if (!strcmp(name, "refine_theta_gen_x1000")) { e->refine_theta_gen = (float)value / 1000.f; return CZC_OK; }
  if (!strcmp(name, "refine_guard_x1e6")) { e->refine_guard_dev = (float)value * 1e-6f; return CZC_OK; }
  if (!strcmp(name, "refine_gate_x1e6")) { e->refine_gate_delta = value < 0 ? 0.f : (float)value * 1e-6f; return CZC_OK; }
  if (!strcmp(name, "refine_rows16")) { const int old = e->refine_rows16; e->refine_rows16 = value ? 1 : 0; const int rc = fold_ready(); if (rc) e->refine_rows16 = old; return rc; }
  if (!strcmp(name, "memo")) { e->memo = value ? 1 : 0; return CZC_OK; }
  if (!strcmp(name, "memo_rows")) { e->memo_rows = value ? 1 : 0; return CZC_OK; }
  if (!strcmp(name, "index_groups")) {
    if (value < 0 || value > 1024) return fail(e, CZC_ERR_ARG, "option %s: 0 (chosen by the launcher) or 1..1024", name);
    e->index_groups = value;
    return CZC_OK;
  }
  if (!strcmp(name, "fluency_chunk")) {
    if (value < 1 || value > 16384) return fail(e, CZC_ERR_ARG, "option %s: 1..16384", name);
    e->fluency_chunk = value;
    return CZC_OK;
  }
  if (!strcmp(name, "regions_chunk")) {
    if (value < 1 || value > CZC_MAX_REGIONS) return fail(e, CZC_ERR_ARG, "option %s: 1..1024", name);
    e->regions_chunk = value;
    return CZC_OK;
  }
  if (!strcmp(name, "refine_rows16_x1000")) { e->refine_rows16_factor = value < 1000 ? 1.f : (float)value / 1000.f; return CZC_OK; }
  return fail(e, CZC_ERR_ARG, "unknown option %s", name);
}

int czc_get_option(czc_engine* e, const char* name, int* value) {
  if (!e || !name || !value) return CZC_ERR_ARG;
  const bool r16 = e->refine && e->refine_rows16 && e->cfg.clip_hidden == 512;
  const float f16x = r16 ? e->refine_rows16_factor : 1.f;
  struct { const char* n; int v; } tab[] = {
      {"share_prefix", e->share_prefix}, {"bert_prune", e->bert_prune}, {"pack_branches", e->pack_branches},
      {"dedup", e->dedup}, {"pool_last_layer", e->pool_last_layer}, {"pool_last_qkv", e->pool_last_qkv}, {"share_layer0", e->share_layer0}, {"bert_fuse_splitk_ln", e->bert_fuse_splitk_ln}, {"fuse_ln", e->fuse_ln}, {"resid16", e->resid16}, {"fold_ln", e->fold_ln},
      {"refine_samples", e->refine_samples}, {"refine_samples_step", e->refine_samples_step}, {"refine_theta_x1000", (int)lrintf(e->refine_theta_x * 1000.f)},
      {"refine_theta_gen_x1000", (int)lrintf(e->refine_theta_gen * 1000.f)},
      {"refine_guard_x1e6", (int)lrintf(e->refine_guard_dev * 1e6f)}, {"refine_gate_x1e6", (int)lrintf(e->refine_gate_delta * 1e6f)},
      {"refine_rows16", e->refine_rows16}, {"memo", e->memo}, {"memo_rows", e->memo_rows}, {"index_groups", e->index_groups}, {"fluency_chunk", e->fluency_chunk}, {"regions_chunk", e->regions_chunk}, {"refine_rows16_x1000", (int)lrintf(e->refine_rows16_factor * 1000.f)},
      {"refine_guard_generate_x1e6", (int)lrintf(e->refine_guard_dev * f16x * 1e6f)},
      {"refine_gate_generate_x1e6", (int)lrintf(e->refine_gate_delta * f16x * 1e6f)},
      {"has_folded_ln_weights", !e->ctext.empty() && e->ctext[0].qkv_wf ? 1 : 0},
  };
  for (auto& t : tab) if (!strcmp(name, t.n)) { *value = t.v; return CZC_OK; }
  return fail(e, CZC_ERR_ARG, "unknown option %s", name);
}

int czc_sync(czc_engine* e) {
  if (!e) return CZC_ERR_ARG;
  E_HIP(hipSetDevice(e->dev));
  E_HIP(hipStreamSynchronize(e->st));
  return CZC_OK;
}

int czc_profile_enable(czc_engine* e, int on) {
  if (!e) return CZC_ERR_ARG;
  e->prof = on < 0 ? 0 : (on > 2 ? 1 : on);
  return CZC_OK;
}

int czc_profile_reset(czc_engine* e) {
  if (!e) return CZC_ERR_ARG;
  (void)hipSetDevice(e->dev);
  (void)hipStreamSynchronize(e->st);
  if (!e->prof_ref) (void)hipEventCreate(&e->prof_ref);
  if (e->prof_ref) (void)hipEventRecord(e->prof_ref, e->st);
  for (auto& kv : e->pk) { kv.second.used = 0; kv.second.flops = 0; kv.second.launches = 0; }
  e->stat_clip_rows = e->stat_clip_seqs = e->stat_bert_rows = e->stat_steps = 0;
  e->stat_refine_rows = e->stat_refine_seqs = 0;
  e->stat_dedup_seqs = 0;
  e->stat_gated = e->stat_gate_images = 0;
  e->stat_memo_hits = e->stat_memo_images = 0;
  e->stat_memo_row_hits = e->stat_memo_row_steps = 0;
  return CZC_OK;
}

int czc_profile_get(czc_engine* e, const char* kind, double* total_ms, int64_t* launches, double* flops) {
  if (!e || !kind) return CZC_ERR_ARG;
  E_HIP(hipSetDevice(e->dev));
  E_HIP(hipStreamSynchronize(e->st));
  double ms = 0;
  int64_t n = 0;
  double fl = 0;
  auto it = e->pk.find(kind);
  if (it != e->pk.end()) {
    ProfKind& k = it->second;
    for (size_t i = 0; i + 1 < k.used; i += 2) {
      float t = 0;
      if (hipEventElapsedTime(&t, k.ev[i], k.ev[i + 1]) == hipSuccess) ms += t;
    }
    n = k.launches;
    fl = k.flops;
  }
  if (total_ms) *total_ms = ms;
  if (launches) *launches = n;
  if (flops) *flops = fl;
  return CZC_OK;
}

int czc_profile_intervals(czc_engine* e, czc_engine* ref, const char* kind, double* start_ms, double* end_ms, int cap,
                          int* n_out) {
  if (!e || !ref || !kind || !n_out || cap < 0 || (cap > 0 && (!start_ms || !end_ms))) return CZC_ERR_ARG;
  if (!ref->prof_ref) return fail(e, CZC_ERR_STATE, "czc_profile_intervals: czc_profile_reset the reference engine first%s");
  if (ref->dev != e->dev) return fail(e, CZC_ERR_ARG, "czc_profile_intervals: engines on different devices%s");
  E_HIP(hipSetDevice(e->dev));
  E_HIP(hipStreamSynchronize(e->st));
  E_HIP(hipStreamSynchronize(ref->st));
  int n = 0;
  auto it = e->pk.find(kind);
  if (it != e->pk.end()) {
    ProfKind& k = it->second;
    for (size_t i = 0; i + 1 < k.used; i += 2, ++n) {
      if (n >= cap) continue;
      float a = 0, b = 0;
      E_HIP(hipEventElapsedTime(&a, ref->prof_ref, k.ev[i]));
      E_HIP(hipEventElapsedTime(&b, ref->prof_ref, k.ev[i + 1]));
      start_ms[n] = a; end_ms[n] = b;
    }
  }
  *n_out = n;
  return CZC_OK;
}

int czc_stats(czc_engine* e, int64_t* clip_rows, int64_t* clip_seqs, int64_t* bert_rows, int64_t* steps) {
  if (!e) return CZC_ERR_ARG;
  if (clip_rows) *clip_rows = e->stat_clip_rows;
  if (clip_seqs) *clip_seqs = e->stat_clip_seqs;
  if (bert_rows) *bert_rows = e->stat_bert_rows;
  if (steps) *steps = e->stat_steps;
  return CZC_OK;
}

int czc_dedup_stats(czc_engine* e, int64_t* dedup_seqs, int64_t* clip_seqs) {
  if (!e) return CZC_ERR_ARG;
  if (dedup_seqs) *dedup_seqs = e->stat_dedup_seqs;
  if (clip_seqs) *clip_seqs = e->stat_clip_seqs;
  return CZC_OK;
}

int czc_refine_stats(czc_engine* e, int64_t* refine_seqs, int64_t* refine_rows) {
  if (!e) return CZC_ERR_ARG;
  if (refine_seqs) *refine_seqs = e->stat_refine_seqs;
  if (refine_rows) *refine_rows = e->stat_refine_rows;
  return CZC_OK;
}

int czc_refine_gate_stats(czc_engine* e, int64_t* gated, int64_t* image_steps) {
  if (!e) return CZC_ERR_ARG;
  if (gated) *gated = e->stat_gated;
  if (image_steps) *image_steps = e->stat_gate_images;
  return CZC_OK;
}

int czc_memo_stats(czc_engine* e, int64_t* hit_image_steps, int64_t* image_steps) {
  if (!e) return CZC_ERR_ARG;
  if (hit_image_steps) *hit_image_steps = e->stat_memo_hits;
  if (image_steps) *image_steps = e->stat_memo_images;
  return CZC_OK;
}

int czc_memo_rows_stats(czc_engine* e, int64_t* hit_row_steps, int64_t* row_steps) {
  if (!e) return CZC_ERR_ARG;
  if (hit_row_steps) *hit_row_steps = e->stat_memo_row_hits;
  if (row_steps) *row_steps = e->stat_memo_row_steps;
  return CZC_OK;
}

int czc_refine_guard(czc_engine* e, int reset, float* max_dev, int64_t* tripped) {
  if (!e) return CZC_ERR_ARG;
  if (max_dev) *max_dev = e->guard_max_dev;
  if (tripped) *tripped = e->guard_trips;
  if (reset) { e->guard_max_dev = 0.f; e->guard_trips = 0; }
  return CZC_OK;
}

static int test_text_tower(void* engine, const int32_t* clip_ids, const int32_t* clip_len, int B, int K, float* out, int32_t* n_dup) {
  czc_engine* e = (czc_engine*)engine;
  if (!e || !clip_ids || !clip_len || B <= 0 || K <= 0 || K > CZC_MAX_TOPK || !out) return CZC_ERR_ARG;
  if (!e->finalized) return fail(e, CZC_ERR_STATE, "weights not finalized%s");
  E_HIP(hipSetDevice(e->dev));
  e->err[0] = 0;
  const int n = B * K;
  int *cids, *clen, *totals;
  E_CHECK(ensure(e, "s_cids", (size_t)n * CZC_CLIP_MAX_LEN * 4, (void**)&cids));
  E_CHECK(ensure(e, "s_clen", (size_t)n * 4, (void**)&clen));
  E_CHECK(ensure(e, "s_tot", PLAN_TOTALS, (void**)&totals));
  E_HIP(hipMemcpyAsync(cids, clip_ids, (size_t)n * CZC_CLIP_MAX_LEN * 4, hipMemcpyDefault, e->st));
  E_HIP(hipMemcpyAsync(clen, clip_len, (size_t)n * 4, hipMemcpyDefault, e->st));
  E_HIP(hipMemsetAsync(totals, 0, PLAN_TOTALS, e->st));
  { int* flag; E_CHECK(ensure(e, "s_nonfinite", 32, (void**)&flag)); E_HIP(hipMemsetAsync(flag, 0, 32, e->st)); }
  float* feat;
  E_CHECK(clip_text_forward(e, cids, clen, B, K, e->share_prefix, totals, &feat));
  if (n_dup) *n_dup = e->h_totals[HT_PLAN + 5];
  E_HIP(hipMemcpyAsync(out, feat, (size_t)n * e->cfg.clip_proj * 4, hipMemcpyDefault, e->st));
  E_HIP(hipStreamSynchronize(e->st));
  return CZC_OK;
}

const void* czc_internal_hooks(int abi) {
  static const Hooks h = {
      []() -> char* { return czc::g_err; },
      &launch_gemm, &launch_gemm_rowln, &launch_layernorm, &launch_convert, &launch_act_to_f32, &launch_attention,
      &launch_attention_shared, &launch_attention_shared_split,
      &launch_softmax_mask_topk, &launch_bridge_precompute, &launch_bridge, &launch_l2_normalize, &launch_combine,
      &launch_layernorm_x16, &launch_ln_finalize, &launch_fold_ln, &gemm_wreg_stats_in_kernel,
      &g_use_gemm256, &g_use_skinny, &g_use_splitk, &g_gemm_deep, &g_gemm_small_tiles, &g_use_wreg, &g_use_gemm256s,
      &g_rowln_min_m, &g_wreg_min_m, &g_gemm256_min_m, &g_use_mfma_attention, &g_use_attention_image, &g_wreg_resid_min_m,
      &g_wreg_stats_in_kernel, &g_gemm256s_min_m,
      &launch_scan, &launch_prefix_plan, &launch_prefix_finish, &launch_refine_select, &launch_refine_select_rows,
      &launch_refine_select_draw, &launch_refine_plan, &launch_refine_finish, &launch_refine_cosine,
      &launch_attention_image_pooled, &launch_attention_shared_mapped, &launch_layer0_count, &launch_layer0_map,
      &test_text_tower,
      &launch_layernorm_splitk, &launch_bert_embed, &launch_bert_embed_ragged, &launch_clip_embed, &launch_im2col, &launch_vision_assemble,
      &launch_gather_rows_f32, &launch_gather_rows_bytes, &launch_gather_rows_w32, &launch_mask_positions, &launch_mask_positions_rows,
      &launch_tie_rows, &launch_memo_check, &launch_memo_gather, &launch_memo_scatter, &launch_memo_fill, &launch_memo_rows_check,
      &launch_memo_rows_gather, &launch_memo_rows_scatter, &launch_memo_rows_fill,
      &fluency_expand_tables, &launch_expand_mask_rows, &launch_logprob_target,
      &launch_bridge_rows, &launch_bridge_rows_hp, &launch_softmax_mask_topk_rows, &launch_softmax_mask_topk_rows_hp,
      &launch_softmax_mask_topk_rows_vocab,
      []() -> int { return czc::g_gemm_family; }};
  return abi == HOOKS_ABI ? &h : nullptr;
}

}
```

conzic_amd/csrc/kernels.h:

```cpp
#pragma once
#include <vector>

#include "common.h"

namespace czc {

struct GemmArgs {
  const void* A = nullptr; int lda = 0;
  const void* W = nullptr; int ldw = 0;
  const float* bias = nullptr;
  const float* resid = nullptr; int ldr = 0;
  void* out_act = nullptr; float* out_f32 = nullptr; int ldc = 0;
  int M = 0, N = 0, K = 0;
  int act = 0;
  int f16 = 0;
  int x16 = 0;
  float* row_part = nullptr;
  long part_ld = 0;
  const float* ln_stat = nullptr;
  const float* ln_part = nullptr;
  long ln_part_ld = 0;
  const float* ln_gamma = nullptr;
  const float* ln_beta = nullptr;
  float ln_eps = 0.f;
  struct SplitkPending* splitk_pending = nullptr;
};
struct SplitkPending { const float* slabs = nullptr; int nslab = 0; long slab_stride = 0; int ld = 0; };
enum GemmFamily {
  GF_NONE = 0, GF_TILED_VEC = 1, GF_TILED_SCALAR = 2, GF_SPLITK = 3, GF_SKINNY = 4, GF_RING_LOADER = 5, GF_RING_PINGPONG = 6,
  GF_RING_SPLIT = 7, GF_WREG = 8, GF_WREG_LNF = 9, GF_WREG_RESID = 10, GF_ROWLN = 11
};
int launch_gemm(int prec, const GemmArgs& g, hipStream_t st);
bool gemm256_eligible(const GemmArgs& g);
int launch_gemm256(const GemmArgs& g, hipStream_t st);
extern int g_use_gemm256;
bool gemm256s_eligible(const GemmArgs& g);
int launch_gemm256s(const GemmArgs& g, hipStream_t st);
extern int g_use_gemm256s, g_gemm256s_min_m;
bool gemm_rowln_eligible(const GemmArgs& g);
int launch_gemm_rowln(const GemmArgs& g, hipStream_t st);
extern int g_rowln_min_m;
extern int g_use_skinny;
extern int g_use_splitk;
extern int g_gemm_deep;
extern int g_gemm_small_tiles;
bool gemm_wreg_eligible(const GemmArgs& g);
int launch_gemm_wreg(const GemmArgs& g, hipStream_t st);
bool gemm_wreg_resid_eligible(const GemmArgs& g);
int launch_gemm_wreg_resid(const GemmArgs& g, hipStream_t st);
extern int g_use_wreg;
extern int g_wreg_resid_min_m;
extern int g_wreg_stats_in_kernel;
bool gemm_wreg_stats_in_kernel(int M, int N);
extern int g_wreg_min_m, g_gemm256_min_m;

size_t imageproc_scratch_bytes(int H, int W, int S);
int launch_clip_preprocess(const unsigned char* rgb_dev, int H, int W, int S, const float* mean, const float* stdv,
                           unsigned char* scratch, float* out, hipStream_t st);
struct RegionsPlan {
  std::vector<unsigned char> host;
  size_t tables_off = 0, tmp_off = 0, scratch_bytes = 0;
  int n = 0, max_rows = 0, any_h = 0;
};
int plan_clip_regions(int S, const int* boxes, int n, RegionsPlan& plan);
int launch_clip_regions(const unsigned char* rgb_dev, int W, int S, const RegionsPlan& plan, const float* mean, const float* stdv,
                        unsigned char* scratch, float* out, hipStream_t st);

int launch_layernorm_splitk(int prec, const SplitkPending& sk, const float* bias, const float* resid, int ldr, const float* gamma,
                            const float* beta, float eps, int M, int H, void* y_act, float* y_f32, hipStream_t st);
int launch_layernorm(int prec, const float* x, const int* row_idx, const float* gamma, const float* beta, float eps,
                     int M, int H, void* y_act, float* y_f32, hipStream_t st);
int launch_layernorm_x16(int prec, const void* x16, const int* row_idx, const float* gamma, const float* beta, float eps, int M,
                         int H, void* y_act, hipStream_t st);
int launch_bert_embed(int prec, const int* ids, int B, int T, int H, const float* word, const float* pos,
                      const float* type0, const float* gamma, const float* beta, float eps, void* y_act, float* y_f32,
                      hipStream_t st);
int launch_clip_embed(const int* ids, int ids_stride, const int* seg_src, const int* seg_pos0, const int* own_off,
                      const int* own_len, int n_seg, int max_len, int H, const float* tok, const float* pos, float* x,
                      hipStream_t st, int x16 = 0, float* stat = nullptr, float eps = 0.f);
int launch_ln_finalize(const float* part, long part_ld, int nblk, int M, float eps, float* stat, hipStream_t st);
int launch_fold_ln(const float* W, const float* gamma, const float* beta, const float* b, int N, int K, void* Wf16, float* rowsum, float* bf,
                   hipStream_t st);
int launch_im2col(int prec, const float* pixels, int B, int S, int p, void* out, hipStream_t st);
int launch_vision_assemble(const float* patch_out, int B, int P, int H, const float* cls, const float* pos, float* x,
                           hipStream_t st);
int launch_convert(int prec, const float* src, void* dst, long n, hipStream_t st);
int launch_act_to_f32(int prec, const void* src, float* dst, long n, hipStream_t st);
int launch_gather_rows_f32(const float* src, const int* idx, int M, int H, float* dst, hipStream_t st);
int launch_gather_rows_bytes(const void* src, const int* idx, int M, int row_bytes, void* dst, hipStream_t st);
int launch_make_row_index(int* idx, int B, int T, int gen_idx, hipStream_t st);
int launch_make_row_index_rows(int* idx, int B, int T, const int* gen, hipStream_t st);
int launch_eos_index(const int* off, const int* len, int n, int* idx, hipStream_t st);
int launch_l2_normalize(const float* x, int M, int D, float* y, hipStream_t st);
int launch_mask_positions(int* inp, int B, int T, int gen_idx, int n_mask, int mask_id, hipStream_t st);
int launch_mask_positions_rows(int* inp, int B, int T, const int* gen, int n_mask, int mask_id, hipStream_t st);
int launch_broadcast_rows_i32(const int* row, int T, int B, int* dst, hipStream_t st);
int launch_gather_rows_w32(const void* src, const int* idx, int M, int W, void* dst, hipStream_t st);
int launch_tie_rows(int* inp, int R, int T, const int* col, const int* grp_of_row, const int* grp_off, const int* grp_rows, hipStream_t st);

int launch_bert_embed_ragged(int prec, const int* ids, int ids_stride, const int* run, const int* row_off, const int* row_len, int n,
                             int max_T, int H, const float* word, const float* pos, const float* type0, const float* gamma,
                             const float* beta, float eps, void* y_act, float* y_f32, hipStream_t st);
int launch_ragged_row_index(int* idx, int n, const int* row_off, const int* gen, hipStream_t st);

int launch_memo_check(const int* inp, int B, int T, int gen_idx, int n_mask, int mask_id, const int* key, const int* img_max,
                      int n_sub, int* hit, int* list, int* tot, hipStream_t st);
int launch_memo_gather(const int* inp, const int* list, int n, int T, int gen_idx, int n_mask, int mask_id, int* key, int* inp_c,
                       const float* img_n, int D, float* img_c, hipStream_t st);
int launch_memo_scatter(const int* rows, const float* bcos, const int* img_max, const int* list, int n, int T, int* inp,
                        float* bcos_full, int* out_rows, float* out_cos, int* out_max, hipStream_t st);
int launch_memo_fill(const int* hit, int B, int T, const int* out_rows, const float* out_cos, int* inp, float* bcos_full,
                     hipStream_t st);

constexpr int MEMO_ROWS_SUB = 2;
struct MemoRowsTab {
  int* valid; int* sig;
  int* key;
  int* rows; float* cos; int* imax;
  int R, T, L, seed_len;
};
struct RowDraw;
int launch_memo_rows_check(const int* inp, const MemoRowsTab& m, const int* col0, const int* col1, int n_mask0, int n_sub,
                           int mask_id, int* hit, int* cnt, int* list, int* tot, hipStream_t st, const RowDraw* draw_rows = nullptr);
int launch_memo_rows_gather(const int* inp, const int* list, int n, const MemoRowsTab& m, const int* col0, const int* col1,
                            int n_mask0, int n_sub, int mask_id, int record, const int* col, const int* dot, int* inp_c,
                            const float* img_n, int D, float* img_c, int* col_c, int* dot_c, hipStream_t st);
int launch_memo_rows_scatter(const int* rows, const float* bcos, const int* img_max, const int* list, int n, const MemoRowsTab& m,
                             const int* col0, int j, int record, int* inp, float* bcos_full, hipStream_t st);
int launch_memo_rows_fill(const int* hit, const MemoRowsTab& m, const int* col0, int j, int* inp, float* bcos_full, hipStream_t st);

struct SegTable {
  const int* pre_off; const int* pre_len; const int* own_off; const int* own_len;
  int n_seg; int fixed_T;
  const int* img_max = nullptr;
};
int launch_attention(int prec, const void* qkv, const SegTable& tab, int max_keys, int heads, int causal, float scale,
                     void* out, hipStream_t st);
extern int g_use_mfma_attention;
extern int g_use_attention_image;
int launch_attention_shared(const void* qkv, const SegTable& tab, int B, int K, int max_own, int max_keys, int heads,
                            float scale, void* out, hipStream_t st, int f16 = 0);
bool attention_image_serves(int B, int K, int max_own, int max_keys, int heads);
int launch_attention_shared_mapped(const void* qkv, int n_rows, const int* rowmap, const SegTable& tab, int B, int K, int max_own,
                                   int max_keys, int heads, float scale, void* out, hipStream_t st, int f16 = 0);
int launch_attention_image_pooled(const void* qkv, const void* qc, const SegTable& tab, const int* rep, int B, int K, int max_own,
                                  int max_keys, int heads, float scale, void* ctx_c, hipStream_t st, int f16 = 0);

int launch_attention_shared_split(const void* qkv, const SegTable& tab, int B, int K, int max_own, int max_keys, int heads,
                                  float scale, void* out, hipStream_t st);

struct RowHyper { float alpha, beta, gamma, temperature; int control, negative; };

int launch_gather_row_hyper(const RowHyper* src, const int* idx, int n, RowHyper* dst, hipStream_t st);

struct RowDraw { unsigned seed_lo, seed_hi; float tau; unsigned step0; };

int launch_gather_row_draw(const RowDraw* src, const int* idx, int n, RowDraw* dst, hipStream_t st);

int launch_softmax_mask_topk(const float* logits, int B, int V, int K, const float* mask, float temperature, int dot_id,
                             int dot_allowed, float* probs, int* idxs, int* cand, hipStream_t st);
int launch_softmax_mask_topk_rows(const float* logits, int B, int V, int K, const float* mask, float temperature, int dot_id,
                                  const int* dot_rows, float* probs, int* idxs, int* cand, hipStream_t st);
int launch_softmax_mask_topk_rows_hp(const float* logits, int B, int V, int K, const float* mask, const RowHyper* hp_rows, int dot_id,
                                     const int* dot_rows, float* probs, int* idxs, int* cand, hipStream_t st);
int launch_softmax_mask_topk_rows_vocab(const float* logits, int B, int V, int K, const float* mask, const RowHyper* hp_rows, int dot_id,
                                        const int* dot_rows, const int* set_rows, const unsigned* bits, int W, float* probs, int* idxs,
                                        int* cand, hipStream_t st);

struct BridgeDev {
  int bert_vocab;
  const uint32_t* piece_off;
  const uint8_t* piece_bytes;
  const uint8_t* piece_class;
  const uint8_t* piece_flags;
  const int* byte_sym;
  const int* byte_sym_eow;
  const unsigned long long* hkeys;
  const unsigned long long* hvals;
  unsigned hmask;
  int bos_id, eos_id;
  const int* tok_bpe = nullptr;
  const uint8_t* tok_bpe_len = nullptr;
};
constexpr int BR_TOKMAX = 8;
int launch_bridge_precompute(const BridgeDev& bd, int* tok_ids, uint8_t* tok_len, hipStream_t st);
struct PosDev {
  const uint8_t* tag_of_token;
  const uint16_t* masks;
  int n;
};
int launch_bridge(const BridgeDev& bd, const int* inp, int B, int T, int gen_idx, const int* cand, int K,
                  const float* lexicon, const float* lex_pos, const uint8_t* lex_cls, int negative, const PosDev& pos, int* clip_ids, int* clip_len, float* senti_raw,
                  float* repeats, int* overflow_flag, hipStream_t st);
int launch_bridge_rows(const BridgeDev& bd, const int* inp, int B, int T, const int* gen_rows, const int* cand, int K,
                       const float* lexicon, const float* lex_pos, const uint8_t* lex_cls, int negative, const PosDev& pos, int* clip_ids, int* clip_len,
                       float* senti_raw, float* repeats, int* overflow_flag, hipStream_t st, const int* row_len = nullptr);
int launch_bridge_rows_hp(const BridgeDev& bd, const int* inp, int B, int T, const int* gen_rows, const int* cand, int K,
                          const float* lexicon, const float* lex_pos, const uint8_t* lex_cls, const RowHyper* hp_rows, const PosDev& pos,
                          int* clip_ids, int* clip_len, float* senti_raw, float* repeats, int* overflow_flag, hipStream_t st,
                          const int* row_len = nullptr);
int launch_scan(const int* len, int n, int* off, int* totals, hipStream_t st);
int launch_prefix_plan(const int* clip_ids, const int* clip_len, int B, int K, int share, int* own_len, int* pre_len,
                       int* seg_src, int* seg_pos0, int* max_len_out, int* img_max, hipStream_t st,
                       int* rep = nullptr, int* n_dup_out = nullptr);
int launch_layer0_count(const int* clip_ids, const int* own_len, const int* pre_len, int B, int K, int* dcount, int* total, hipStream_t st);
int launch_layer0_map(const int* clip_ids, const int* own_off, const int* own_len, const int* pre_len, const int* dcount, int B, int K,
                      int* rowmap, int* dist, hipStream_t st);
int launch_prefix_finish(const int* own_off, const int* own_len, int B, int K, int* pre_off, int* eos_idx,
                         int* n_trunk_rows, hipStream_t st, const int* rep = nullptr);

struct CombineArgs {
  const float* text_feat;
  const float* img_n;
  float logit_scale_exp;
  const float* probs;
  const int* cand;
  const float* senti_raw;
  const float* repeats;
  float alpha, beta, gamma;
  int use_senti;
  int B, K, D;
  float* clip_score; float* clip_ref; float* final_score;
  int* best; float* best_cos;
  int* inp; int T; int gen_idx;
  int* nonfinite = nullptr;
  const int* refine_kind = nullptr;
  const float* refine_cos = nullptr;
  float refine_guard = 0.f;
  const int* gen_rows = nullptr;
  const RowHyper* hp_rows = nullptr;
  const RowDraw* draw_rows = nullptr;
  unsigned draw_step = 0;
  const int* rival_idx = nullptr;
  int M = 0;
  const float* rival_delta = nullptr;
  const float* img_all = nullptr;
  int n_img = 0;
  float* disc = nullptr;
};
constexpr int CB_MAX_RIVALS = 16;
constexpr int CB_RIVAL_FLOATS = 8192;
int launch_combine(const CombineArgs& a, hipStream_t st);
int launch_cosine_rival(const float* text_feat, const float* img_n, int B, int K, int D, const int* rival_idx, int M, const float* img_all,
                        int n_img, float logit_scale_exp, float* cos_out, float* disc, int* nonfinite, hipStream_t st);
int launch_cosine(const float* text_feat, const float* img_n, int B, int K, int D, float* cos_out, int* nonfinite, hipStream_t st);
int launch_refine_select(const float* clip_score, const float* final_score, int B, int K, float theta, int m_samples, float gate_h,
                         float beta, int need_cos, int* gated, int* kind, int* list, int* count, hipStream_t st);
int launch_refine_select_rows(const float* clip_score, const float* final_score, int B, int K, float theta_base, float scale,
                              int m_samples, float gate_h, const RowHyper* hp_rows, int need_cos, int* gated, int* kind, int* list,
                              int* count, hipStream_t st);
int launch_refine_select_draw(const float* clip_score, const float* final_score, int B, int K, float theta, float theta_base, float scale,
                              int m_samples, float gate_h, float beta, const RowHyper* hp_rows, const RowDraw* draw_rows, int need_cos,
                              int* gated, int* kind, int* list, int* count, hipStream_t st);
int launch_refine_cosine(const float* text_feat, const float* img_n, const int* rlist, const int* n_rows_dev, int n_rows_max, int K, int D,
                         float* cos_out, int* nonfinite, hipStream_t st);
int launch_refine_plan(const int* clip_len, const int* trunk_len, const int* list, const int* count, const int* count_off,
                       const int* kr_dev, int B, int K, int* own_len, int* pre_len, int* seg_src, int* seg_pos0, int* rlist,
                       int* max_len_out, int* img_max, hipStream_t st);
int launch_refine_finish(const int* own_off, const int* own_len, const int* count, const int* count_off, const int* kr_dev, int B, int K,
                         int* pre_off, int* eos_idx, hipStream_t st);

int launch_normalize_split(const float* src, long n, int D, split_t* dst, int* bad, int bad_stride, hipStream_t st);
int index_scan_groups(int n, int D, int k, int groups);
int launch_index_search(const split_t* index, int n, int D, const split_t* queries, int Q, int k, int G,
                        unsigned long long* part, int* out_ids, float* out_cos, hipStream_t st);

int fluency_expand_tables(int R, int seed_len, int Lmax, const int32_t* len_of_row, int32_t* row_of_seq, int32_t* col_of_seq);
int launch_expand_mask_rows(const int* rows, int T, const int* row_of_seq, const int* col_of_seq, int N, int mask_id, int* ids_out,
                            int* target, int* gen_rows, hipStream_t st);
int launch_logprob_target(const float* logits, int N, int V, const int* target, float temperature, const int* out_idx, float* logp,
                          int* rank, int* nonfinite, hipStream_t st);
int launch_pll_sum(const float* logp, int R, int Lmax, const int* len_of_row, float* pll, hipStream_t st);

constexpr int HOOKS_ABI = 0x060d;
struct Hooks {
  char* (*err_buf)();
  decltype(&launch_gemm) gemm;
  decltype(&launch_gemm_rowln) gemm_rowln;
  decltype(&launch_layernorm) layernorm;
  decltype(&launch_convert) convert;
  decltype(&launch_act_to_f32) act_to_f32;
  decltype(&launch_attention) attention;
  decltype(&launch_attention_shared) attention_shared;
  decltype(&launch_attention_shared_split) attention_shared_split;
  decltype(&launch_softmax_mask_topk) softmax_mask_topk;
  decltype(&launch_bridge_precompute) bridge_precompute;
  decltype(&launch_bridge) bridge;
  decltype(&launch_l2_normalize) l2_normalize;
  decltype(&launch_combine) combine;
  decltype(&launch_layernorm_x16) layernorm_x16;
  decltype(&launch_ln_finalize) ln_finalize;
  decltype(&launch_fold_ln) fold_ln;
  decltype(&gemm_wreg_stats_in_kernel) wreg_stats_ok;
  int *use_gemm256, *use_skinny, *use_splitk, *gemm_deep, *gemm_small_tiles, *use_wreg, *use_gemm256s, *rowln_min_m,
      *wreg_min_m, *gemm256_min_m, *use_mfma_attention, *use_attention_image, *wreg_resid_min_m, *wreg_stats_in_kernel,
      *gemm256s_min_m;
  decltype(&launch_scan) scan;
  decltype(&launch_prefix_plan) prefix_plan;
  decltype(&launch_prefix_finish) prefix_finish;
  decltype(&launch_refine_select) refine_select;
  decltype(&launch_refine_select_rows) refine_select_rows;
  decltype(&launch_refine_select_draw) refine_select_draw;
  decltype(&launch_refine_plan) refine_plan;
  decltype(&launch_refine_finish) refine_finish;
  decltype(&launch_refine_cosine) refine_cosine;
  decltype(&launch_attention_image_pooled) attention_image_pooled;
  decltype(&launch_attention_shared_mapped) attention_shared_mapped;
  decltype(&launch_layer0_count) layer0_count;
  decltype(&launch_layer0_map) layer0_map;
  int (*text_tower)(void* engine, const int32_t* clip_ids, const int32_t* clip_len, int B, int K, float* out, int32_t* n_dup);
  decltype(&launch_layernorm_splitk) layernorm_splitk;
  decltype(&launch_bert_embed) bert_embed;
  decltype(&launch_bert_embed_ragged) bert_embed_ragged;
  decltype(&launch_clip_embed) clip_embed;
  decltype(&launch_im2col) im2col;
  decltype(&launch_vision_assemble) vision_assemble;
  decltype(&launch_gather_rows_f32) gather_rows_f32;
  decltype(&launch_gather_rows_bytes) gather_rows_bytes;
  decltype(&launch_gather_rows_w32) gather_rows_w32;
  decltype(&launch_mask_positions) mask_positions;
  decltype(&launch_mask_positions_rows) mask_positions_rows;
  decltype(&launch_tie_rows) tie_rows;
  decltype(&launch_memo_check) memo_check;
  decltype(&launch_memo_gather) memo_gather;
  decltype(&launch_memo_scatter) memo_scatter;
  decltype(&launch_memo_fill) memo_fill;
  decltype(&launch_memo_rows_check) memo_rows_check;
  decltype(&launch_memo_rows_gather) memo_rows_gather;
  decltype(&launch_memo_rows_scatter) memo_rows_scatter;
  decltype(&launch_memo_rows_fill) memo_rows_fill;
  decltype(&fluency_expand_tables) fluency_expand_tables;
  decltype(&launch_expand_mask_rows) expand_mask_rows;
  decltype(&launch_logprob_target) logprob_target;
  decltype(&launch_bridge_rows) bridge_rows;
  decltype(&launch_bridge_rows_hp) bridge_rows_hp;
  decltype(&launch_softmax_mask_topk_rows) softmax_mask_topk_rows;
  decltype(&launch_softmax_mask_topk_rows_hp) softmax_mask_topk_rows_hp;
  decltype(&launch_softmax_mask_topk_rows_vocab) softmax_mask_topk_rows_vocab;
  int (*gemm_family)();
};

}

extern "C" __attribute__((visibility("default"))) const void* czc_internal_hooks(int abi);
```

conzic_amd/csrc/rowops.hip:

```cpp
#include "kernels.h"

namespace czc {

__device__ __forceinline__ float wave_sum_rowln_order(float v) {
#define CZC_SWZ_XOR(M_) __builtin_bit_cast(float, __builtin_amdgcn_ds_swizzle(__builtin_bit_cast(int, v), 0x1f | ((M_) << 10)))
  v += CZC_SWZ_XOR(1);
  v += CZC_SWZ_XOR(2);
  v += CZC_SWZ_XOR(4);
  v += CZC_SWZ_XOR(8);
  v += CZC_SWZ_XOR(16);
#undef CZC_SWZ_XOR
  v += __shfl_xor(v, 32, 64);
  return v;
}

template <typename T>
__global__ __launch_bounds__(256) void layernorm512_kernel(const float* x, const int* row_idx, const float* gamma,
                                                           const float* beta, float eps, int M, T* y_act, float* y_f32) {
  const int lane = threadIdx.x & 63;
  const int m = blockIdx.x * 4 + (threadIdx.x >> 6);
  if (m >= M) return;
  const long src = row_idx ? row_idx[m] : m;
  const float* xr = x + src * 512L;
  const int c0 = (lane >> 3) * 64 + (lane & 7) * 4;
// ... 196 lines not shown
    if (rowsum) rowsum[j] = (float)r;
    bf[j] = (b ? b[j] : 0.f) + wb;
  }
}

int launch_fold_ln(const float* W, const float* gamma, const float* beta, const float* b, int N, int K, void* Wf16, float* rowsum, float* bf,
                   hipStream_t st) {
  if (K > 512) { snprintf(g_err, sizeof(g_err), "fold_ln: K = %d > 512", K); return 1; }
  hipLaunchKernelGGL(fold_ln_kernel, dim3(cdiv(N, 4)), dim3(256), 0, st, W, gamma, beta, b, N, K, (f16_t*)Wf16, rowsum, bf);
  CZC_HIP_CHECK(hipGetLastError());
  return 0;
}

int launch_layernorm(int prec, const float* x, const int* row_idx, const float* gamma, const float* beta, float eps,
                     int M, int H, void* y_act, float* y_f32, hipStream_t st) {
  if (M <= 0) return 0;
  if (H <= 0 || H % 4 || H > LN_MAXV * 256 || (prec == PREC_F16X3 && y_act && H % 8)) {
    snprintf(g_err, sizeof(g_err), "layernorm: unsupported H=%d", H);
    return 1;
  }
  dim3 grid(cdiv(M, 4)), block(256);
  if (H == 512 && prec == PREC_BF16)
    hipLaunchKernelGGL(layernorm512_kernel<bf16_t>, grid, block, 0, st, x, row_idx, gamma, beta, eps, M, (bf16_t*)y_act, y_f32);
  else if (H == 512 && prec == PREC_F16)
    hipLaunchKernelGGL(layernorm512_kernel<f16_t>, grid, block, 0, st, x, row_idx, gamma, beta, eps, M, (f16_t*)y_act, y_f32);
  else if (prec == PREC_BF16)
    hipLaunchKernelGGL(layernorm_kernel<bf16_t>, grid, block, 0, st, x, row_idx, gamma, beta, eps, M, H,
                       (bf16_t*)y_act, y_f32);
  else if (prec == PREC_F16)
    hipLaunchKernelGGL(layernorm_kernel<f16_t>, grid, block, 0, st, x, row_idx, gamma, beta, eps, M, H,
                       (f16_t*)y_act, y_f32);
  else if (prec == PREC_F16X3)
    hipLaunchKernelGGL(layernorm_kernel<split_t>, grid, block, 0, st, x, row_idx, gamma, beta, eps, M, H,
                       (split_t*)y_act, y_f32);
  else
    hipLaunchKernelGGL(layernorm_kernel<float>, grid, block, 0, st, x, row_idx, gamma, beta, eps, M, H, (float*)y_act,
                       y_f32);
  CZC_HIP_CHECK(hipGetLastError());
  return 0;
}

template <typename T>
__global__ __launch_bounds__(256) void layernorm_splitk_kernel(const float* slabs, int nslab, long slab_stride, int ld, const float* bias,
                                                               const float* resid, int ldr, const float* gamma, const float* beta,
                                                               float eps, int M, int H, T* y_act, float* y_f32) {
  const int lane = threadIdx.x & 63;
  const int m = blockIdx.x * 4 + (threadIdx.x >> 6);
  if (m >= M) return;
  float4 v[LN_MAXV];
#pragma unroll
  for (int i = 0; i < LN_MAXV; ++i) {
    const int c = (i * 64 + lane) * 4;
    if (c < H) {
      float4 a = *(const float4*)(slabs + (long)m * ld + c);
      for (int z = 1; z < nslab; ++z) {
        const float4 p = *(const float4*)(slabs + z * slab_stride + (long)m * ld + c);
        a.x += p.x; a.y += p.y; a.z += p.z; a.w += p.w;
      }
      if (bias) { const float4 b = *(const float4*)(bias + c); a.x += b.x; a.y += b.y; a.z += b.z; a.w += b.w; }
      if (resid) { const float4 r = *(const float4*)(resid + (long)m * ldr + c); a.x += r.x; a.y += r.y; a.z += r.z; a.w += r.w; }
      v[i] = a;
    } else {
      v[i] = make_float4(0, 0, 0, 0);
    }
  }
  ln_row<LN_MAXV>(v, H, lane, gamma, beta, eps);
#pragma unroll
  for (int i = 0; i < LN_MAXV; ++i) {
    const int c = (i * 64 + lane) * 4;
    if (c < H) {
      if (y_f32) *(float4*)(y_f32 + (long)m * H + c) = v[i];
      if (y_act) Act<T>::st4(y_act, (long)m * H + c, v[i].x, v[i].y, v[i].z, v[i].w);
    }
  }
}

int launch_layernorm_splitk(int prec, const SplitkPending& sk, const float* bias, const float* resid, int ldr, const float* gamma,
                            const float* beta, float eps, int M, int H, void* y_act, float* y_f32, hipStream_t st) {
  if (M <= 0) return 0;
  if (H <= 0 || H % 4 || H > LN_MAXV * 256 || (prec == PREC_F16X3 && y_act && H % 8) || sk.nslab <= 0 || !sk.slabs || sk.ld % 4 || (resid && ldr % 4) || (prec != PREC_F16X3 && prec != PREC_F32)) {
    snprintf(g_err, sizeof(g_err), "layernorm_splitk: unsupported shape / precision (H=%d, slabs=%d)", H, sk.nslab);
    return 1;
  }
  dim3 grid(cdiv(M, 4)), block(256);
  if (prec == PREC_F16X3)
    hipLaunchKernelGGL(layernorm_splitk_kernel<split_t>, grid, block, 0, st, sk.slabs, sk.nslab, sk.slab_stride, sk.ld, bias, resid, ldr, gamma,
                       beta, eps, M, H, (split_t*)y_act, y_f32);
  else
    hipLaunchKernelGGL(layernorm_splitk_kernel<float>, grid, block, 0, st, sk.slabs, sk.nslab, sk.slab_stride, sk.ld, bias, resid, ldr, gamma,
                       beta, eps, M, H, (float*)y_act, y_f32);
  CZC_HIP_CHECK(hipGetLastError());
  return 0;
}

template <typename T>
__global__ __launch_bounds__(256) void bert_embed_kernel(const int* ids, int M, int T_, int H, const float* word,
                                                         const float* pos, const float* type0, const float* gamma,
                                                         const float* beta, float eps, T* y_act, float* y_f32) {
  const int lane = threadIdx.x & 63;
  const int m = blockIdx.x * 4 + (threadIdx.x >> 6);
  if (m >= M) return;
  const int id = ids[m];
  const int p = m % T_;
  const float* wr = word + (long)id * H;
  const float* pr = pos + (long)p * H;
  float4 v[LN_MAXV];
#pragma unroll
  for (int i = 0; i < LN_MAXV; ++i) {
    const int c = (i * 64 + lane) * 4;
    if (c < H) {
      const float4 a = *(const float4*)(wr + c), b = *(const float4*)(type0 + c), d = *(const float4*)(pr + c);
      v[i] = make_float4((a.x + b.x) + d.x, (a.y + b.y) + d.y, (a.z + b.z) + d.z, (a.w + b.w) + d.w);
    } else {
      v[i] = make_float4(0, 0, 0, 0);
    }
  }
  ln_row<LN_MAXV>(v, H, lane, gamma, beta, eps);
#pragma unroll
  for (int i = 0; i < LN_MAXV; ++i) {
    const int c = (i * 64 + lane) * 4;
    if (c < H) {
      if (y_f32) *(float4*)(y_f32 + (long)m * H + c) = v[i];
      if (y_act) Act<T>::st4(y_act, (long)m * H + c, v[i].x, v[i].y, v[i].z, v[i].w);
    }
  }
}

int launch_bert_embed(int prec, const int* ids, int B, int T_, int H, const float* word, const float* pos,
                      const float* type0, const float* gamma, const float* beta, float eps, void* y_act, float* y_f32,
                      hipStream_t st) {
  const int M = B * T_;
  if (M <= 0) return 0;
  if (H <= 0 || H % 4 || H > LN_MAXV * 256 || (prec == PREC_F16X3 && y_act && H % 8)) {
    snprintf(g_err, sizeof(g_err), "bert_embed: unsupported H=%d", H);
    return 1;
  }
  dim3 grid(cdiv(M, 4)), block(256);
  if (prec == PREC_BF16)
    hipLaunchKernelGGL(bert_embed_kernel<bf16_t>, grid, block, 0, st, ids, M, T_, H, word, pos, type0, gamma, beta, eps,
                       (bf16_t*)y_act, y_f32);
  else if (prec == PREC_F16)
    hipLaunchKernelGGL(bert_embed_kernel<f16_t>, grid, block, 0, st, ids, M, T_, H, word, pos, type0, gamma, beta, eps,
                       (f16_t*)y_act, y_f32);
  else if (prec == PREC_F16X3)
    hipLaunchKernelGGL(bert_embed_kernel<split_t>, grid, block, 0, st, ids, M, T_, H, word, pos, type0, gamma, beta, eps,
                       (split_t*)y_act, y_f32);
  else
    hipLaunchKernelGGL(bert_embed_kernel<float>, grid, block, 0, st, ids, M, T_, H, word, pos, type0, gamma, beta, eps,
                       (float*)y_act, y_f32);
  CZC_HIP_CHECK(hipGetLastError());
  return 0;
}

__global__ __launch_bounds__(256) void clip_embed_kernel(const int* ids, int ids_stride, const int* seg_src,
                                                         const int* seg_pos0, const int* own_off, const int* own_len,
                                                         int n_seg, int max_len, int H, const float* tok,
                                                         const float* pos, float* x, int x16, float* stat, float eps) {
  const int lane = threadIdx.x & 63;
  const long w = (long)blockIdx.x * 4 + (threadIdx.x >> 6);
  const int s = (int)(w / max_len), i = (int)(w % max_len);
  if (s >= n_seg || i >= own_len[s]) return;
  const int p = seg_pos0[s] + i;
  const int id = ids[(long)seg_src[s] * ids_stride + p];
  const float* tr = tok + (long)id * H;
  const float* pr = pos + (long)p * H;
  if (x16) {
    f16_t* xh = (f16_t*)x + ((long)own_off[s] + i) * H;
    float sm = 0.f;
    float4 keep[LN_MAXV];
#pragma unroll
    for (int t = 0; t < LN_MAXV; ++t) {
      const int c = lane * 4 + t * 256;
      keep[t] = make_float4(0.f, 0.f, 0.f, 0.f);
      if (c < H) {
        const float4 a = *(const float4*)(tr + c), b = *(const float4*)(pr + c);
        const uint2 pk = make_uint2(pack2_f16(a.x + b.x, a.y + b.y), pack2_f16(a.z + b.z, a.w + b.w));
        *(uint2*)(xh + c) = pk;
        keep[t] = make_float4(f16lo(pk.x), f16hi(pk.x), f16lo(pk.y), f16hi(pk.y));
        sm += (keep[t].x + keep[t].y) + (keep[t].z + keep[t].w);
      }
    }
    if (stat) {
      const float mean = wave_sum(sm) / (float)H;
      float q = 0.f;
#pragma unroll
      for (int t = 0; t < LN_MAXV; ++t) {
        if (lane * 4 + t * 256 < H) {
          const float a = keep[t].x - mean, b = keep[t].y - mean, c2 = keep[t].z - mean, d = keep[t].w - mean;
          q += (a * a + b * b) + (c2 * c2 + d * d);
        }
      }
      const float rstd = rsqrtf(wave_sum(q) / (float)H + eps);
      if (lane == 0) *(float2*)(stat + ((long)own_off[s] + i) * 2) = make_float2(mean, rstd);
    }
    return;
  }
  float* xr = x + ((long)own_off[s] + i) * H;
  for (int c = lane * 4; c < H; c += 256) {
    const float4 a = *(const float4*)(tr + c), b = *(const float4*)(pr + c);
    *(float4*)(xr + c) = make_float4(a.x + b.x, a.y + b.y, a.z + b.z, a.w + b.w);
  }
}

int launch_clip_embed(const int* ids, int ids_stride, const int* seg_src, const int* seg_pos0, const int* own_off,
                      const int* own_len, int n_seg, int max_len, int H, const float* tok, const float* pos, float* x,
                      hipStream_t st, int x16, float* stat, float eps) {
  if (n_seg <= 0 || max_len <= 0) return 0;
  if (H <= 0 || H % 4 || (x16 && H > LN_MAXV * 256)) {
    snprintf(g_err, sizeof(g_err), "clip_embed: unsupported H=%d (x16=%d)", H, x16);
    return 1;
  }
  dim3 grid(cdiv((long)n_seg * max_len, 4)), block(256);
  hipLaunchKernelGGL(clip_embed_kernel, grid, block, 0, st, ids, ids_stride, seg_src, seg_pos0, own_off, own_len, n_seg,
                     max_len, H, tok, pos, x, x16, stat, eps);
  CZC_HIP_CHECK(hipGetLastError());
  return 0;
}

template <typename T>
__global__ void im2col_kernel(const float* pix, int B, int S, int p, T* out) {
  const int G = S / p, P = G * G, Kc = 3 * p * p;
  const long total = (long)B * P * Kc;
  for (long i = (long)blockIdx.x * blockDim.x + threadIdx.x; i < total; i += (long)gridDim.x * blockDim.x) {
    const int k = (int)(i % Kc);
    const long bp = i / Kc;
    const int pp = (int)(bp % P), b = (int)(bp / P);
    const int c = k / (p * p), iy = (k / p) % p, ix = k % p;
    const int py = pp / G, px = pp % G;
    const float v = pix[(((long)b * 3 + c) * S + (py * p + iy)) * S + (px * p + ix)];
    Act<T>::st(out, i, v);
  }
}

int launch_im2col(int prec, const float* pixels, int B, int S, int p, void* out, hipStream_t st) {
  if (B <= 0 || S <= 0) return 0;
  if (p <= 0 || S % p) { snprintf(g_err, sizeof(g_err), "im2col: patch %d does not tile a %d-pixel side", p, S); return 1; }
  const long total = (long)B * (S / p) * (S / p) * 3 * p * p;
  dim3 grid((unsigned)((total + 255) / 256 < 8192 ? (total + 255) / 256 : 8192)), block(256);
  if (prec == PREC_BF16)
    hipLaunchKernelGGL(im2col_kernel<bf16_t>, grid, block, 0, st, pixels, B, S, p, (bf16_t*)out);
  else if (prec == PREC_F16)
    hipLaunchKernelGGL(im2col_kernel<f16_t>, grid, block, 0, st, pixels, B, S, p, (f16_t*)out);
  else if (prec == PREC_F16X3)
    hipLaunchKernelGGL(im2col_kernel<split_t>, grid, block, 0, st, pixels, B, S, p, (split_t*)out);
  else
    hipLaunchKernelGGL(im2col_kernel<float>, grid, block, 0, st, pixels, B, S, p, (float*)out);
  CZC_HIP_CHECK(hipGetLastError());
  return 0;
}

__global__ void vision_assemble_kernel(const float* patch_out, int B, int P, int H, const float* cls, const float* pos,
                                       float* x) {
  const long total = (long)B * (P + 1) * H;
  for (long i = (long)blockIdx.x * blockDim.x + threadIdx.x; i < total; i += (long)gridDim.x * blockDim.x) {
    const int c = (int)(i % H);
    const long bt = i / H;
    const int t = (int)(bt % (P + 1)), b = (int)(bt / (P + 1));
    const float e = t == 0 ? cls[c] : patch_out[((long)b * P + (t - 1)) * H + c];
    x[i] = e + pos[(long)t * H + c];
  }
}

int launch_vision_assemble(const float* patch_out, int B, int P, int H, const float* cls, const float* pos, float* x,
                           hipStream_t st) {
  const long total = (long)B * (P + 1) * H;
  if (B <= 0 || P < 0 || H <= 0) return 0;
  dim3 grid((unsigned)((total + 255) / 256 < 8192 ? (total + 255) / 256 : 8192)), block(256);
  hipLaunchKernelGGL(vision_assemble_kernel, grid, block, 0, st, patch_out, B, P, H, cls, pos, x);
  CZC_HIP_CHECK(hipGetLastError());
  return 0;
}

template <typename T>
__global__ void convert_kernel(const float* src, T* dst, long n) {
  for (long i = (long)blockIdx.x * blockDim.x + threadIdx.x; i < n; i += (long)gridDim.x * blockDim.x)
    Act<T>::st(dst, i, src[i]);
}

int launch_convert(int prec, const float* src, void* dst, long n, hipStream_t st) {
  if (n <= 0) return 0;
  dim3 grid((unsigned)((n + 255) / 256 < 16384 ? (n + 255) / 256 : 16384)), block(256);
  if (prec == PREC_BF16)
    hipLaunchKernelGGL(convert_kernel<bf16_t>, grid, block, 0, st, src, (bf16_t*)dst, n);
  else if (prec == PREC_F16)
    hipLaunchKernelGGL(convert_kernel<f16_t>, grid, block, 0, st, src, (f16_t*)dst, n);
  else if (prec == PREC_F16X3)
    hipLaunchKernelGGL(convert_kernel<split_t>, grid, block, 0, st, src, (split_t*)dst, n);
  else
    hipLaunchKernelGGL(convert_kernel<float>, grid, block, 0, st, src, (float*)dst, n);
  CZC_HIP_CHECK(hipGetLastError());
  return 0;
}

template <typename T>
__global__ void act_to_f32_kernel(const T* src, float* dst, long n) {
  for (long i = (long)blockIdx.x * blockDim.x + threadIdx.x; i < n; i += (long)gridDim.x * blockDim.x)
    dst[i] = Act<T>::ld(src, i);
}

int launch_act_to_f32(int prec, const void* src, float* dst, long n, hipStream_t st) {
  if (n <= 0) return 0;
  dim3 grid((unsigned)((n + 255) / 256 < 16384 ? (n + 255) / 256 : 16384)), block(256);
  if (prec == PREC_BF16) hipLaunchKernelGGL(act_to_f32_kernel<bf16_t>, grid, block, 0, st, (const bf16_t*)src, dst, n);
  else if (prec == PREC_F16) hipLaunchKernelGGL(act_to_f32_kernel<f16_t>, grid, block, 0, st, (const f16_t*)src, dst, n);
  else if (prec == PREC_F16X3) hipLaunchKernelGGL(act_to_f32_kernel<split_t>, grid, block, 0, st, (const split_t*)src, dst, n);
  else hipLaunchKernelGGL(act_to_f32_kernel<float>, grid, block, 0, st, (const float*)src, dst, n);
  CZC_HIP_CHECK(hipGetLastError());
  return 0;
}

__global__ void gather_rows_kernel(const float* src, const int* idx, int M, int H, float* dst) {
  const int lane = threadIdx.x & 63;
  const int m = blockIdx.x * 4 + (threadIdx.x >> 6);
  if (m >= M) return;
  const float* s = src + (long)idx[m] * H;
  float* d = dst + (long)m * H;
  for (int c = lane * 4; c < H; c += 256) *(float4*)(d + c) = *(const float4*)(s + c);
}

__global__ void gather_rows_bytes_kernel(const unsigned char* src, const int* idx, int M, int row_bytes,
                                         unsigned char* dst) {
  const int lane = threadIdx.x & 63;
  const int m = blockIdx.x * 4 + (threadIdx.x >> 6);
  if (m >= M) return;
  const unsigned char* s = src + (long)idx[m] * row_bytes;
  unsigned char* d = dst + (long)m * row_bytes;
  for (int c = lane * 16; c < row_bytes; c += 1024) *(uint4*)(d + c) = *(const uint4*)(s + c);
}

int launch_gather_rows_bytes(const void* src, const int* idx, int M, int row_bytes, void* dst, hipStream_t st) {
  if (M <= 0 || row_bytes <= 0) return 0;
  if (row_bytes % 16) { snprintf(g_err, sizeof(g_err), "gather_rows_bytes: rows of %d bytes are not whole 16-byte vectors", row_bytes); return 1; }
  hipLaunchKernelGGL(gather_rows_bytes_kernel, dim3(cdiv(M, 4)), dim3(256), 0, st, (const unsigned char*)src, idx, M,
                     row_bytes, (unsigned char*)dst);
  CZC_HIP_CHECK(hipGetLastError());
  return 0;
}

__global__ void gather_row_hyper_kernel(const RowHyper* src, const int* idx, int n, RowHyper* dst) {
  const int i = blockIdx.x * blockDim.x + threadIdx.x;
  if (i < n) dst[i] = src[idx[i]];
}

int launch_gather_row_hyper(const RowHyper* src, const int* idx, int n, RowHyper* dst, hipStream_t st) {
  if (n <= 0) return 0;
  hipLaunchKernelGGL(gather_row_hyper_kernel, dim3(cdiv(n, 256)), dim3(256), 0, st, src, idx, n, dst);
  CZC_HIP_CHECK(hipGetLastError());
  return 0;
}

__global__ void gather_row_draw_kernel(const RowDraw* src, const int* idx, int n, RowDraw* dst) {
  const int i = blockIdx.x * blockDim.x + threadIdx.x;
  if (i < n) dst[i] = src[idx[i]];
}

int launch_gather_row_draw(const RowDraw* src, const int* idx, int n, RowDraw* dst, hipStream_t st) {
  if (n <= 0) return 0;
  hipLaunchKernelGGL(gather_row_draw_kernel, dim3(cdiv(n, 256)), dim3(256), 0, st, src, idx, n, dst);
  CZC_HIP_CHECK(hipGetLastError());
  return 0;
}

int launch_gather_rows_f32(const float* src, const int* idx, int M, int H, float* dst, hipStream_t st) {
  if (M <= 0 || H <= 0) return 0;
  if (H % 4) { snprintf(g_err, sizeof(g_err), "gather_rows_f32: H=%d is not a multiple of 4 (launch_gather_rows_w32 takes any width)", H); return 1; }
  hipLaunchKernelGGL(gather_rows_kernel, dim3(cdiv(M, 4)), dim3(256), 0, st, src, idx, M, H, dst);
  CZC_HIP_CHECK(hipGetLastError());
// ... 131 lines not shown
```

conzic_amd/native.py:

```python
from __future__ import annotations

import ctypes as C
import os
from typing import Optional

_HERE = os.path.dirname(os.path.abspath(__file__))
LIB_PATH = os.environ.get("CZC_LIB_PATH") or os.path.join(_HERE, "lib", "libconzic_hip.so")
HEADER_PATH = os.path.join(os.path.dirname(_HERE), "include", "conzic_hip.h")
TEST_LIB_PATH = os.environ.get("CZC_TEST_LIB_PATH") or (LIB_PATH[:-3] + "_test.so" if LIB_PATH.endswith(".so")
                                                        else os.path.join(os.path.dirname(LIB_PATH), "libconzic_hip_test.so"))
TEST_HEADER_PATH = os.path.join(os.path.dirname(_HERE), "include", "conzic_hip_test.h")

PREC_BF16 = 0
PREC_F32 = 1
PREC_ALL_BF16 = 2
PREC_SPLIT = 3
PREC_FP16 = 4
PREC_REFINE = 5
CLIP_MAX_LEN = 77
MAX_BERT_LEN = 64
MAX_VOCAB_SETS = 4096
MAX_RIVALS = 16
MAX_REGIONS = 1024
INDEX_MAX_K = 64
POS_IDLE = -1


ERR_ARG, ERR_HIP, ERR_STATE, ERR_OVERFLOW = 1, 2, 3, 4


class NativeError(RuntimeError):

    def __init__(self, msg, code=None):
        super().__init__(msg)
        self.code = code


class Config(C.Structure):
    _fields_ = [
        ("bert_vocab", C.c_int32), ("bert_hidden", C.c_int32), ("bert_layers", C.c_int32), ("bert_heads", C.c_int32),
        ("bert_inter", C.c_int32), ("bert_max_pos", C.c_int32), ("bert_eps", C.c_float),
        ("clip_vocab", C.c_int32), ("clip_hidden", C.c_int32), ("clip_layers", C.c_int32), ("clip_heads", C.c_int32),
        ("clip_inter", C.c_int32), ("clip_max_pos", C.c_int32), ("clip_proj", C.c_int32), ("clip_eps", C.c_float),
        ("clip_bos_id", C.c_int32), ("clip_eos_id", C.c_int32),
        ("vis_hidden", C.c_int32), ("vis_layers", C.c_int32), ("vis_heads", C.c_int32), ("vis_inter", C.c_int32),
        ("vis_image", C.c_int32), ("vis_patch", C.c_int32),
        ("pad_id", C.c_int32), ("unk_id", C.c_int32), ("cls_id", C.c_int32), ("sep_id", C.c_int32),
        ("mask_id", C.c_int32), ("dot_id", C.c_int32),
        ("precision", C.c_int32),
    ]


class BridgeTables(C.Structure):
    _fields_ = [
        ("bert_vocab", C.c_int32),
        ("piece_off", C.c_void_p), ("piece_bytes", C.c_void_p), ("piece_class", C.c_void_p), ("piece_flags", C.c_void_p),
        ("clip_vocab", C.c_int32),
        ("byte_sym", C.c_void_p), ("byte_sym_eow", C.c_void_p),
        ("n_merges", C.c_int32),
        ("merge_left", C.c_void_p), ("merge_right", C.c_void_p), ("merge_out", C.c_void_p),
        ("bos_id", C.c_int32), ("eos_id", C.c_int32),
    ]


class Hyper(C.Structure):
    _fields_ = [("alpha", C.c_float), ("beta", C.c_float), ("gamma", C.c_float), ("temperature", C.c_float),
                ("control", C.c_int32), ("negative", C.c_int32)]


class Draw(C.Structure):
    _fields_ = [("seed", C.c_uint64), ("tau", C.c_float), ("step0", C.c_uint32)]


STEP_OUT_FIELDS = ["probs", "idxs", "cand_ids", "clip_ids", "clip_len", "clip_score", "clip_ref", "senti_raw",
                   "repeats", "final_score", "best", "best_cos", "logits"]


class StepOut(C.Structure):
    _fields_ = [(n, C.c_void_p) for n in STEP_OUT_FIELDS]


CONTROL_FN = C.CFUNCTYPE(C.c_int, C.c_void_p, C.POINTER(C.c_int32), C.POINTER(C.c_int32), C.c_int, C.c_int, C.c_int,
                         C.c_int, C.POINTER(C.c_float))

_P = C.c_void_p
_I = C.c_int
SIGNATURES = {
    "czc_create": (_I, [C.POINTER(Config), _I, C.POINTER(_P)]),
    "czc_destroy": (_I, [_P]),
    "czc_last_error": (C.c_char_p, [_P]),
    "czc_version": (_I, []),
    "czc_load_tensor": (_I, [_P, C.c_char_p, _I, _I, C.POINTER(C.c_int64), _P]),
    "czc_finalize_weights": (_I, [_P]),
    "czc_set_token_mask": (_I, [_P, _P, _I]),
    "czc_set_bridge": (_I, [_P, C.POINTER(BridgeTables)]),
    "czc_set_lexicon": (_I, [_P, _P, _I]),
    "czc_set_lexicon_pos": (_I, [_P, _P, _P, _I]),
    "czc_set_pos": (_I, [_P, _P, _I, _P, _I]),
    "czc_set_control_callback": (_I, [_P, _P, _P]),
    "czc_encode_images": (_I, [_P, _P, _I, _P]),
    "czc_preprocess_u8": (_I, [_P, _P, _I, _I, _P, _P, _I, _P]),
    "czc_preprocess_regions_u8": (_I, [_P, _P, _I, _I, _P, _I, _P, _P, _I, _P]),
    "czc_encode_staged": (_I, [_P, _I, _P]),
    "czc_set_image_embeds": (_I, [_P, _P, _I]),
    "czc_encode_text": (_I, [_P, _P, _P, _I, _P]),
    "czc_similarity": (_I, [_P, _P, _P, _I, _I, _P, _P]),
    "czc_index_set": (_I, [_P, _P, C.c_int64]),
    "czc_index_size": (_I, [_P, C.POINTER(C.c_int64)]),
    "czc_index_search": (_I, [_P, _P, _I, _I, _P, _P]),
    "czc_step": (_I, [_P, _P, _I, _I, _I, _I, _I, _I, C.POINTER(Hyper), C.POINTER(StepOut)]),
    "czc_generate": (_I, [_P, _I, _I, _I, _I, _P, _I, _I, _P, _P, _I, C.POINTER(Hyper), _P, _P]),
    "czc_generate_rows": (_I, [_P, _I, _I, _I, _I, _P, _P, _I, _I, _P, _P, _I, C.POINTER(Hyper), _P, _P]),
    "czc_generate_rows_from": (_I, [_P, _I, _I, _I, _I, _P, _P, _I, _I, _P, _P, _I, C.POINTER(Hyper), _P, _P]),
    "czc_generate_rows_len": (_I, [_P, _I, _I, _I, _P, _P, _P, _I, _I, _P, _P, _I, C.POINTER(Hyper), _P, _P]),
    "czc_generate_rows_hp": (_I, [_P, _I, _I, _I, _P, _P, _P, _I, _I, _P, _P, _I, C.POINTER(Hyper), _P, _P]),
    "czc_generate_rows_draw": (_I, [_P, _I, _I, _I, _P, _P, _P, _I, _I, _P, _P, _I, C.POINTER(Hyper), C.POINTER(Draw), _P, _P]),
    "czc_generate_rows_tied": (_I, [_P, _I, _I, _I, _P, _P, _P, _P, _I, _I, _P, _P, _I, C.POINTER(Hyper), C.POINTER(Draw), _P, _P]),
    "czc_score_rows": (_I, [_P, _P, _I, _I, _I, _P, _P, _P]),
    "czc_generate_rows_vs": (_I, [_P, _I, _I, _I, _P, _P, _P, _P, _I, _I, _P, _P, _I, C.POINTER(Hyper), C.POINTER(Draw), _P, _I, _P,
                                  _P, _P]),
    "czc_generate_rows_vocab": (_I, [_P, _I, _I, _I, _P, _P, _P, _P, _I, _I, _P, _P, _I, C.POINTER(Hyper), C.POINTER(Draw), _P, _I, _P,
                                     _P, _I, _P, _P, _P]),
    "czc_score_rows_vs": (_I, [_P, _P, _I, _I, _I, _P, _P, _P, _I, _P, _P]),
    "czc_fluency_rows": (_I, [_P, _P, _I, _I, _I, _P, C.c_float, _P, _P, _P]),
    "czc_set_option": (_I, [_P, C.c_char_p, _I]),
    "czc_get_option": (_I, [_P, C.c_char_p, C.POINTER(_I)]),
    "czc_profile_enable": (_I, [_P, _I]),
    "czc_profile_reset": (_I, [_P]),
    "czc_profile_get": (_I, [_P, C.c_char_p, C.POINTER(C.c_double), C.POINTER(C.c_int64), C.POINTER(C.c_double)]),
    "czc_profile_intervals": (_I, [_P, _P, C.c_char_p, _P, _P, _I, C.POINTER(C.c_int)]),
    "czc_replicate": (_I, [_P, C.POINTER(C.c_void_p)]),
    "czc_sync": (_I, [_P]),
    "czc_stats": (_I, [_P, C.POINTER(C.c_int64), C.POINTER(C.c_int64), C.POINTER(C.c_int64), C.POINTER(C.c_int64)]),
    "czc_refine_stats": (_I, [_P, C.POINTER(C.c_int64), C.POINTER(C.c_int64)]),
    "czc_dedup_stats": (_I, [_P, C.POINTER(C.c_int64), C.POINTER(C.c_int64)]),
    "czc_refine_guard": (_I, [_P, _I, C.POINTER(C.c_float), C.POINTER(C.c_int64)]),
    "czc_refine_gate_stats": (_I, [_P, C.POINTER(C.c_int64), C.POINTER(C.c_int64)]),
    "czc_memo_stats": (_I, [_P, C.POINTER(C.c_int64), C.POINTER(C.c_int64)]),
    "czc_memo_rows_stats": (_I, [_P, C.POINTER(C.c_int64), C.POINTER(C.c_int64)]),
}
PRIVATE_SIGNATURES = {"czc_internal_hooks": (_P, [_I])}


class GemmLayout(C.Structure):
    _fields_ = ([(n, C.c_int32) for n in ("precision", "form", "M", "N", "K", "act", "lda", "ldw", "ldc", "ldr", "c0", "flags",
                                          "part_ld")] + [("eps", C.c_float)] +
                [(n, C.c_void_p) for n in ("A", "W", "bias", "resid", "gamma", "beta", "ln_part", "out_f32", "out_act", "part_out")])


TEST_SIGNATURES = {
    "czc_test_gemm": (_I, [_I, _I, _I, _I, _P, _P, _P, _P, _I, _P]),
    "czc_test_gemm_x16": (_I, [_I, _I, _I, _I, _P, _P, _P, _P, _P, _P]),
    "czc_test_ln_fold_gemm": (_I, [_I, _I, _I, _P, _P, _P, _P, _P, _P, C.c_float, _I, _P, _P]),
    "czc_test_layernorm_x16": (_I, [_I, _I, _P, _P, _P, C.c_float, _P]),
    "czc_test_gemm_rowln": (_I, [_I, _I, _I, _P, _P, _P, _P, _P, _P, C.c_float, _P, _P]),
    "czc_bench_gemm": (_I, [_I, _I, _I, _I, _I, _I, _I, _I, C.POINTER(C.c_double)]),
    "czc_test_set_option": (_I, [C.c_char_p, _I]),
    "czc_test_layernorm": (_I, [_I, _I, _I, _P, _P, _P, C.c_float, _P]),
    "czc_test_attention": (_I, [_I, _I, _P, _I, _I, C.c_float, _P, _P]),
    "czc_test_attention_plan": (_I, [_I, _I, _I, _I, _I, C.c_float, _P, _P, _I, _P, _P]),
    "czc_test_attention_pooled": (_I, [_I, _I, _I, _I, C.c_float, _P, _P, _P, _P, _P, _P]),
    "czc_test_attention_mapped": (_I, [_I, _I, _I, _I, C.c_float, _P, _P, _P, _I, _P, _P]),
    "czc_test_layer0_plan": (_I, [_I, _I, _P, _P, _I, _P, _P, _P, _P, _I, _P, _I, _P]),
    "czc_test_text_tower": (_I, [_P, _I, _I, _P, _P, _P, _P]),
    "czc_test_topk": (_I, [_I, _I, _I, _P, _P, C.c_float, _I, _I, _P, _P, _P]),
    "czc_test_bridge": (_I, [C.POINTER(BridgeTables), C.POINTER(Config), _I, _I, _P, _P, _P]),
    "czc_test_combine": (_I, [_I, _I, _I, _P, _P, C.c_float, _P, _P, _P, C.POINTER(Hyper), _P, _P, _P, _P]),
    "czc_test_combine_draw": (_I, [_I, _I, _I, _P, _P, C.c_float, _P, _P, _P, C.POINTER(Hyper), C.POINTER(Draw), C.c_uint32, _P, _P]),
    "czc_test_scan": (_I, [_I, _P, _P, _P]),
    "czc_test_prefix_plan": (_I, [_I, _I, _I, _I] + [_P] * 12),
    "czc_test_refine_select": (_I, [_I, _I, _I, _P, _P, C.c_float, C.c_float, C.c_float, _I, C.c_float, C.c_float, _I, _P, _P,
                                    _P, _P, _P, _P]),
    "czc_test_refine_plan": (_I, [_I, _I] + [_P] * 15),
    "czc_test_refine_cosine": (_I, [_I, _I, _I, _I, _I, _P, _P, _P, _P, _P]),
    "czc_test_combine_refine": (_I, [_I, _I, C.c_float, _P, _P, C.POINTER(Hyper), _P, _P, C.c_float, _P, _P, _P, _P, _P, _P]),
    "czc_test_combine_rivals": (_I, [_I, _I, _I, _P, _P, _I, _P, _P, _I, _P, C.c_float, _P, C.POINTER(Hyper), C.POINTER(Draw),
                                     C.c_uint32, _P, _P, _P, _P, _P]),
    "czc_test_layernorm_rows": (_I, [_I, _I, _I, _I, _P, _P, _P, _P, C.c_float, _I, _P, _P]),
    "czc_test_layernorm_x16_rows": (_I, [_I, _I, _I, _I, _P, _P, _P, _P, C.c_float, _P]),
    "czc_test_layernorm_splitk": (_I, [_I, _I, _I, _I, _I, _P, _P, _P, _I, _P, _P, C.c_float, _P, _P]),
    "czc_test_ln_finalize": (_I, [_I, _I, _I, _P, C.c_float, _P]),
    "czc_test_bert_embed": (_I, [_I, _I, _I, _I, _I, _I, _P, _P, _P, _P, _P, _P, C.c_float, _P, _P]),
    "czc_test_bert_embed_ragged": (_I, [_I] * 8 + [_P] * 4 + [_I] + [_P] * 5 + [C.c_float, _P, _P]),
    "czc_test_clip_embed": (_I, [_I] * 6 + [_P] * 5 + [_I, _I, _P, _P, _I, C.c_float, _P, _P]),
    "czc_test_im2col": (_I, [_I, _I, _I, _I, _P, _P]),
    "czc_test_vision_assemble": (_I, [_I, _I, _I, _P, _P, _P, _P]),
    "czc_test_l2_normalize": (_I, [_I, _I, _P, _P]),
    "czc_test_gather_rows": (_I, [_I, _I, _I, _I, _P, _P, _P]),
    "czc_test_mask_positions": (_I, [_I, _I, _I, _P, _I, _I, _P, _P]),
    "czc_test_tie_rows": (_I, [_I, _I, _I] + [_P] * 6),
    "czc_test_memo_chain": (_I, [_I] * 10 + [_P] * 22),
    "czc_test_memo_rows_chain": (_I, [_I] * 12 + [_P] * 33),
    "czc_test_logprob": (_I, [_I, _I, _P, _P, C.c_float, _P, _P, _P]),
    "czc_test_expand_mask": (_I, [_I, _I, _I, _I, _P, _P, _P, _P, _P, _P]),
    "czc_test_bridge_cand": (_I, [C.POINTER(BridgeTables), _I, _I, _I, _I, _P, _I, _P, _P, _P, _P, _P, _P, _P, _P, _I, _I, _P,
                                  _P, _P, _P, _P, _P]),
    "czc_test_topk_rows": (_I, [_I, _I, _I, _I, _P, _P, C.c_float, _I, _P, _P, _P, _P, _P]),
    "czc_test_topk_rows_vocab": (_I, [_I, _I, _I, _P, _P, _I, _P, _P, _P, _P, _I, _I, _P, _P, _P]),
    "czc_test_gemm_family": (_I, []),
    "czc_test_gemm_layout": (_I, [C.POINTER(GemmLayout)]),
}

_lib: Optional[C.CDLL] = None
_test_lib: Optional[C.CDLL] = None


def load() -> C.CDLL:
    global _lib
    if _lib is not None:
        return _lib
    if not os.path.exists(LIB_PATH):
        raise NativeError(f"{LIB_PATH} not found: build it with `python -c 'import __graft_entry__ as g; g.build()'` "
                          "(there is no CPU fallback)")
    lib = C.CDLL(LIB_PATH, mode=C.RTLD_GLOBAL)
    for name, (res, args) in list(SIGNATURES.items()) + list(PRIVATE_SIGNATURES.items()):
        fn = getattr(lib, name)
        fn.restype = res
        fn.argtypes = args
    _lib = lib
    return lib


def load_test() -> C.CDLL:
    global _test_lib
    if _test_lib is not None:
        return _test_lib
    load()
    if not os.path.exists(TEST_LIB_PATH):
        raise NativeError(f"{TEST_LIB_PATH} not found: `make -C conzic_amd/csrc` builds it next to the product library")
    lib = C.CDLL(TEST_LIB_PATH, mode=C.RTLD_GLOBAL)
    for name, (res, args) in TEST_SIGNATURES.items():
        fn = getattr(lib, name)
        fn.restype = res
        fn.argtypes = args
    _test_lib = lib
    return lib


def check(rc: int, handle=None, what: str = ""):
    if rc != 0:
        lib = load()
        msg = lib.czc_last_error(handle)
        raise NativeError(f"{what} failed (status {rc}): {msg.decode() if msg else '?'}", code=rc)
```

Baseline: 83.57.

## Fuse prefix planning kernels and embed only distinct layer-0 rows

Merges the prefix plan, scan, finish and layer-0 count kernels into two launches: a per-image plan kernel with an in-block scan, and an offsets kernel. Separately, the CLIP token+position embedding and LN stats are computed only for distinct layer-0 rows and then spread to all rows. This also lets the later gather of distinct rows be skipped. The aim is fewer small launches and less redundant embedding work, at the cost of an extra spread pass and more complex index bookkeeping.

Result: no change. 83.89 (median of 6 runs) (+0.4%).

```diff
diff --git a/conzic_amd/csrc/bridge.hip b/conzic_amd/csrc/bridge.hip
--- a/conzic_amd/csrc/bridge.hip
+++ b/conzic_amd/csrc/bridge.hip
@@ -266,9 +266,9 @@
   return 0;
 }
 
-__global__ __launch_bounds__(256) void prefix_plan_kernel(const int* cids, const int* clen, int B, int K, int share,
-                                                          int* own_len, int* pre_len, int* seg_src, int* seg_pos0,
-                                                          int* max_len_out, int* img_max, int* rep, int* n_dup_out) {
+__device__ __forceinline__ int plan_image(const int* cids, const int* clen, int B, int K, int share, int* own_len, int* pre_len,
+                                          int* seg_src, int* seg_pos0, int* max_len_out, int* img_max, int* rep, int* n_dup_out,
+                                          int* s_own, int* mx_out) {
   __shared__ int s_p, s_max, s_keys, s_dup;
   __shared__ unsigned long long s_hash[1024];
   __shared__ short s_len[1024];
@@ -324,6 +324,7 @@
       if (r != k) { own = 0; ++dups; }
     }
     own_len[s] = own;
+    if (s_own) s_own[k] = own;
     pre_len[s] = pb;
     seg_src[s] = b * K + k;
     seg_pos0[s] = pb;
@@ -336,6 +337,15 @@
     atomicAdd(max_len_out + 4, s_keys + pb * (pb + 1) / 2);
     if (n_dup_out && s_dup) atomicAdd(n_dup_out, s_dup);
   }
+  *mx_out = s_max;
+  return pb;
+}
+
+__global__ __launch_bounds__(256) void prefix_plan_kernel(const int* cids, const int* clen, int B, int K, int share,
+                                                          int* own_len, int* pre_len, int* seg_src, int* seg_pos0,
+                                                          int* max_len_out, int* img_max, int* rep, int* n_dup_out) {
+  int mx;
+  plan_image(cids, clen, B, K, share, own_len, pre_len, seg_src, seg_pos0, max_len_out, img_max, rep, n_dup_out, nullptr, &mx);
 }
 
 int launch_prefix_plan(const int* clip_ids, const int* clip_len, int B, int K, int share, int* own_len, int* pre_len,
@@ -399,7 +409,7 @@
 }
 
 __global__ __launch_bounds__(256) void layer0_map_kernel(const int* cids, const int* own_off, const int* own_len, const int* pre_len,
-                                                         const int* dcount, int B, int K, int* rowmap, int* dist) {
+                                                         const int* dcount, int B, int K, int* rowmap, int* dist, int2* dsrc) {
   __shared__ unsigned s_mask[1024];
   __shared__ int s_pref[1024];
   __shared__ int s_base;
@@ -411,8 +421,11 @@
     for (int j = threadIdx.x; j < b; j += blockDim.x) n += dcount[j];
     if (n) atomicAdd(&s_base, n);
   }
-  for (int r = own_off[b] + threadIdx.x; r < own_off[b] + own_len[b]; r += blockDim.x) { rowmap[r] = r; dist[r] = r; }
   const int* cid = cids + (long)b * K * BR_LEN;
+  for (int r = own_off[b] + threadIdx.x; r < own_off[b] + own_len[b]; r += blockDim.x) {
+    rowmap[r] = r; dist[r] = r;
+    if (dsrc) dsrc[r] = make_int2(cid[r - own_off[b]], r - own_off[b]);
+  }
   const int* own = own_len + B + b * K;
   const int* off = own_off + B + b * K;
   const int pb = pre_len[B + b * K];
@@ -433,15 +446,111 @@
       const int j = (s_mask[k] >> i) & 1 ? k : layer0_rep(cid, own, pb, k, i);
       const int c = base + s_pref[j] + __popc(s_mask[j] & ((1u << i) - 1u));
       rowmap[off[k] + i] = c;
-      if (j == k) dist[c] = off[k] + i;
+      if (j == k) {
+        dist[c] = off[k] + i;
+        if (dsrc) dsrc[c] = make_int2(cid[(long)k * BR_LEN + pb + i], pb + i);
+      }
     }
   }
 }
 
 int launch_layer0_map(const int* clip_ids, const int* own_off, const int* own_len, const int* pre_len, const int* dcount, int B, int K,
-                      int* rowmap, int* dist, hipStream_t st) {
+                      int* rowmap, int* dist, hipStream_t st, int2* dsrc) {
   if (K > 1024) { snprintf(g_err, sizeof(g_err), "layer-0 row map: K <= 1024"); return 1; }
-  hipLaunchKernelGGL(layer0_map_kernel, dim3(B), dim3(256), 0, st, clip_ids, own_off, own_len, pre_len, dcount, B, K, rowmap, dist);
+  hipLaunchKernelGGL(layer0_map_kernel, dim3(B), dim3(256), 0, st, clip_ids, own_off, own_len, pre_len, dcount, B, K, rowmap, dist, dsrc);
+  CZC_HIP_CHECK(hipGetLastError());
+  return 0;
+}
+
+__global__ __launch_bounds__(256) void plan_fused_kernel(const int* cids, const int* clen, int B, int K, int share, int* own_len,
+                                                         int* pre_len, int* seg_src, int* seg_pos0, int* totals, int* img_max, int* rep,
+                                                         int* rel, int* img_rows, int* dcount) {
+  __shared__ int s_own[1024];
+  __shared__ int s_part[256];
+  __shared__ int s_n;
+  const int b = blockIdx.x, tid = threadIdx.x;
+  if (tid == 0) s_n = 0;
+  int mx;
+  const int pb = plan_image(cids, clen, B, K, share, own_len, pre_len, seg_src, seg_pos0, totals + 3, img_max, rep, totals + 5, s_own, &mx);
+  const int k0 = tid * 4;
+  int sum = 0;
+#pragma unroll
+  for (int i = 0; i < 4; ++i) sum += k0 + i < K ? s_own[k0 + i] : 0;
+  s_part[tid] = sum;
+  __syncthreads();
+  for (int o = 1; o < 256; o <<= 1) {
+    const int v = tid >= o ? s_part[tid - o] : 0;
+    __syncthreads();
+    s_part[tid] += v;
+    __syncthreads();
+  }
+  int run = s_part[tid] - sum;
+#pragma unroll
+  for (int i = 0; i < 4; ++i)
+    if (k0 + i < K) { rel[b * K + k0 + i] = run; run += s_own[k0 + i]; }
+  if (tid == 255) img_rows[b] = s_part[255];
+  if (tid == 0) atomicMax(totals + 1, max(pb, mx - pb));
+  if (dcount) {
+    const int* cid = cids + (long)b * K * BR_LEN;
+    int n = 0;
+    for (int k = tid; k < K; k += blockDim.x)
+      for (int i = 0; i < min(s_own[k], 32); ++i) n += layer0_rep(cid, s_own, pb, k, i) == k;
+    if (n) atomicAdd(&s_n, n);
+    __syncthreads();
+    if (tid == 0) { dcount[b] = s_n; if (s_n) atomicAdd(totals + 8, s_n); }
+  }
+}
+
+__global__ __launch_bounds__(256) void plan_offsets_kernel(const int* own_len, const int* rel, const int* img_rows, const int* rep, int B,
+                                                           int K, int* own_off, int* pre_off, int* eos_idx, int* totals) {
+  __shared__ int s_red[3][256];
+  __shared__ int s_base[257], s_trunk[257];
+  const int tid = threadIdx.x;
+  const long i0 = (long)blockIdx.x * 256;
+  const int n = B * K;
+  const int b0 = (int)(i0 / K), b1 = (int)(min(i0 + 255, (long)n - 1) / K);
+  int all = 0, tr = 0, rows = 0;
+  for (int j = tid; j < B; j += 256) {
+    const int t = own_len[j];
+    all += t;
+    if (j < b0) { tr += t; rows += img_rows[j]; }
+  }
+  s_red[0][tid] = all; s_red[1][tid] = tr; s_red[2][tid] = rows;
+  __syncthreads();
+  for (int o = 128; o > 0; o >>= 1) {
+    if (tid < o) { s_red[0][tid] += s_red[0][tid + o]; s_red[1][tid] += s_red[1][tid + o]; s_red[2][tid] += s_red[2][tid + o]; }
+    __syncthreads();
+  }
+  const int n_trunk = s_red[0][0];
+  if (tid == 0) {
+    int t = s_red[1][0], r = n_trunk + s_red[2][0];
+    for (int bb = b0; bb <= b1; ++bb) { s_trunk[bb - b0] = t; s_base[bb - b0] = r; t += own_len[bb]; r += img_rows[bb]; }
+  }
+  __syncthreads();
+  const long i = i0 + tid;
+  if (i >= n) return;
+  const int b = (int)(i / K), k = (int)(i - (long)b * K);
+  const int base = s_base[b - b0], s = B + (int)i;
+  own_off[s] = base + rel[i];
+  pre_off[s] = s_trunk[b - b0];
+  if (k == 0) { own_off[b] = s_trunk[b - b0]; pre_off[b] = 0; }
+  const int ir = rep ? b * K + rep[i] : (int)i;
+  eos_idx[i] = base + rel[ir] + own_len[B + ir] - 1;
+  if (i == n - 1) {
+    const int M = base + rel[i] + own_len[s];
+    own_off[B + n] = M; totals[0] = M; totals[6] = n_trunk;
+  }
+}
+
+int launch_plan_fused(const int* clip_ids, const int* clip_len, int B, int K, int share, int* own_len, int* pre_len, int* seg_src,
+                      int* seg_pos0, int* own_off, int* pre_off, int* eos_idx, int* img_max, int* rep, int* rel, int* img_rows,
+                      int* dcount, int* totals, hipStream_t st) {
+  if (B <= 0 || K <= 0 || K > 1024) { snprintf(g_err, sizeof(g_err), "fused plan: B > 0, 0 < K <= 1024"); return 1; }
+  hipLaunchKernelGGL(plan_fused_kernel, dim3(B), dim3(256), 0, st, clip_ids, clip_len, B, K, share, own_len, pre_len, seg_src, seg_pos0,
+                     totals, img_max, rep, rel, img_rows, dcount);
+  CZC_HIP_CHECK(hipGetLastError());
+  hipLaunchKernelGGL(plan_offsets_kernel, dim3(cdiv((long)B * K, 256)), dim3(256), 0, st, own_len, rel, img_rows, rep, B, K, own_off,
+                     pre_off, eos_idx, totals);
   CZC_HIP_CHECK(hipGetLastError());
   return 0;
 }
diff --git a/conzic_amd/csrc/engine.hip b/conzic_amd/csrc/engine.hip
--- a/conzic_amd/csrc/engine.hip
+++ b/conzic_amd/csrc/engine.hip
@@ -110,6 +110,8 @@
   int pack_branches = 1;
   int pool_last_layer = 1;
   int share_layer0 = 1;
+  int embed_distinct = 1;
+  int plan_fused = 1;
   int pool_last_qkv = 1;
   int fuse_ln = 1;
   int resid16 = 1;
@@ -296,7 +298,7 @@
   return 0;
 }
 
-struct Layer0Rows { const int* rowmap = nullptr; const int* dist = nullptr; int n = 0; };
+struct Layer0Rows { const int* rowmap = nullptr; const int* dist = nullptr; int n = 0; bool embedded = false; };
 
 int clip_stack(czc_engine* e, int P, const char* gk, std::vector<LayerW>& L, float* x, int M, int H, int I, int heads,
                float eps, const SegTable& tab, int max_keys, int causal, int plan_B = 0, int plan_K = 0,
@@ -392,7 +394,8 @@
       void* xg; float* sg;
       E_CHECK(ensure(e, "cs_xg", (size_t)l0.n * H * 2, &xg));
       E_CHECK(ensure(e, "cs_sg", (size_t)l0.n * 8 + 256, (void**)&sg));
-      { ProfScope ps(e, rk, 0);
+      if (!l0.embedded) {
+        ProfScope ps(e, rk, 0);
         E_CHECK(launch_gather_rows_bytes(x, l0.dist, l0.n, H * 2, xg, e->st));
         E_CHECK(launch_gather_rows_w32(ln_stat0, l0.dist, l0.n, 2, sg, e->st)); }
       E_CHECK(folded_gemm(xg, l.qkv_wf, l.qkv_bf, sg, qkv, l0.n, 3 * H, ACT_NONE));
@@ -603,13 +606,20 @@
   const int S = B + B * K;
   { ProfScope ps(e, "bridge", 0);
     int* rep = e->dedup && share && K > 1 ? p.rep : nullptr;
-    E_CHECK(launch_prefix_plan(cids, clen, B, K, share, p.own_len, p.pre_len, p.src, p.pos0, totals + 3, p.img_max, e->st, rep, totals + 5));
-    E_CHECK(launch_scan(p.own_len, S, p.own_off, totals, e->st));
-    E_CHECK(launch_prefix_finish(p.own_off, p.own_len, B, K, p.pre_off, p.eidx, totals + 6, e->st, rep));
-    if (e->share_layer0 && share && K > 1 && K <= 1024 && e->fold_ln && e->pack_branches) {
-      int* dcount;
+    int* dcount = nullptr;
+    if (e->share_layer0 && share && K > 1 && K <= 1024 && e->fold_ln && e->pack_branches)
       E_CHECK(ensure(e, "p_dcount", (size_t)B * 4, (void**)&dcount));
-      E_CHECK(launch_layer0_count(cids, p.own_len, p.pre_len, B, K, dcount, totals + 8, e->st));
+    if (e->plan_fused && K <= 1024) {
+      int *rel, *img_rows;
+      E_CHECK(ensure(e, "p_rel", (size_t)B * K * 4, (void**)&rel));
+      E_CHECK(ensure(e, "p_img_rows", (size_t)B * 4, (void**)&img_rows));
+      E_CHECK(launch_plan_fused(cids, clen, B, K, share, p.own_len, p.pre_len, p.src, p.pos0, p.own_off, p.pre_off, p.eidx, p.img_max, rep,
+                                rel, img_rows, dcount, totals, e->st));
+    } else {
+      E_CHECK(launch_prefix_plan(cids, clen, B, K, share, p.own_len, p.pre_len, p.src, p.pos0, totals + 3, p.img_max, e->st, rep, totals + 5));
+      E_CHECK(launch_scan(p.own_len, S, p.own_off, totals, e->st));
+      E_CHECK(launch_prefix_finish(p.own_off, p.own_len, B, K, p.pre_off, p.eidx, totals + 6, e->st, rep));
+      if (dcount) E_CHECK(launch_layer0_count(cids, p.own_len, p.pre_len, B, K, dcount, totals + 8, e->st));
     } }
   E_HIP(hipMemcpyAsync(e->h_totals + HT_PLAN, totals, PLAN_TOTALS, hipMemcpyDeviceToHost, e->st));
   int* flag;
@@ -635,22 +645,33 @@
                                 (P == PREC_F16 && refine_rows16_now(e)));
   float* stat0 = nullptr;
   if (r16 && e->fold_ln && !L.empty() && L[0].qkv_wf) E_CHECK(ensure(e, "c_stat0", (size_t)M * 8 + 256, (void**)&stat0));
-  { ProfScope ps(e, "rowops_clip_text", 0);
-    E_CHECK(launch_clip_embed(cids, CZC_CLIP_MAX_LEN, p.src, p.pos0, p.own_off, p.own_len, n_seg, max_len, H, tok, pos, x, e->st, r16 ? 1 : 0,
-                              stat0, c.clip_eps)); }
   SegTable tab{p.pre_off, p.pre_len, p.own_off, p.own_len, n_seg, 0, plan_B > 0 ? p.img_max : nullptr};
   float* pooled = nullptr;
   Layer0Rows l0;
   if (n_dist > 0 && n_dist <= M && e->share_layer0 && stat0 && L.size() > 1 && plan_B > 0 && prec_is_half(P) && g_use_mfma_attention &&
       e->pack_branches && attention_image_serves(plan_B, plan_K, max_branch, max_len, c.clip_heads) &&
       (long)n_dist * 3 * H * 2 < (1L << 31)) {
-    int *rowmap, *dist, *dcount;
+    int *rowmap, *dist, *dcount; int2* dsrc = nullptr;
     E_CHECK(ensure(e, "c_l0map", (size_t)M * 4, (void**)&rowmap));
     E_CHECK(ensure(e, "c_l0dist", (size_t)n_dist * 4, (void**)&dist));
     E_CHECK(ensure(e, "p_dcount", (size_t)plan_B * 4, (void**)&dcount));
+    if (e->embed_distinct) E_CHECK(ensure(e, "c_l0src", (size_t)n_dist * 8, (void**)&dsrc));
     { ProfScope ps(e, "bridge", 0);
-      E_CHECK(launch_layer0_map(cids, p.own_off, p.own_len, p.pre_len, dcount, plan_B, plan_K, rowmap, dist, e->st)); }
+      E_CHECK(launch_layer0_map(cids, p.own_off, p.own_len, p.pre_len, dcount, plan_B, plan_K, rowmap, dist, e->st, dsrc)); }
     l0.rowmap = rowmap; l0.dist = dist; l0.n = n_dist;
+    if (dsrc) {
+      void* xg; float* sg;
+      E_CHECK(ensure(e, "cs_xg", (size_t)l0.n * H * 2, &xg));
+      E_CHECK(ensure(e, "cs_sg", (size_t)l0.n * 8 + 256, (void**)&sg));
+      ProfScope ps(e, "rowops_clip_text", 0);
+      E_CHECK(launch_clip_embed_distinct(dsrc, l0.n, rowmap, M, H, tok, pos, xg, sg, x, stat0, c.clip_eps, e->st));
+      l0.embedded = true;
+    }
+  }
+  if (!l0.embedded) {
+    ProfScope ps(e, "rowops_clip_text", 0);
+    E_CHECK(launch_clip_embed(cids, CZC_CLIP_MAX_LEN, p.src, p.pos0, p.own_off, p.own_len, n_seg, max_len, H, tok, pos, x, e->st, r16 ? 1 : 0,
+                              stat0, c.clip_eps));
   }
   E_CHECK(clip_stack(e, P, gk, L, x, M, H, c.clip_inter, c.clip_heads, c.clip_eps, tab, max_len, 1, plan_B,
                      plan_K, max_branch, p.eidx, n_pool, &pooled, r16, stat0, l0, rep));
@@ -2764,6 +2785,8 @@
   if (!strcmp(name, "pack_branches")) { e->pack_branches = value ? 1 : 0; return CZC_OK; }
   if (!strcmp(name, "pool_last_layer")) { e->pool_last_layer = value ? 1 : 0; return CZC_OK; }
   if (!strcmp(name, "share_layer0")) { e->share_layer0 = value ? 1 : 0; return CZC_OK; }
+  if (!strcmp(name, "embed_distinct")) { e->embed_distinct = value ? 1 : 0; return CZC_OK; }
+  if (!strcmp(name, "plan_fused")) { e->plan_fused = value ? 1 : 0; return CZC_OK; }
   if (!strcmp(name, "pool_last_qkv")) { e->pool_last_qkv = value ? 1 : 0; return CZC_OK; }
   if (!strcmp(name, "fuse_ln")) { e->fuse_ln = value; return CZC_OK; }
   const auto fold_ready = [&]() -> int {
@@ -2807,7 +2830,7 @@
   const float f16x = r16 ? e->refine_rows16_factor : 1.f;
   struct { const char* n; int v; } tab[] = {
       {"share_prefix", e->share_prefix}, {"bert_prune", e->bert_prune}, {"pack_branches", e->pack_branches},
-      {"dedup", e->dedup}, {"pool_last_layer", e->pool_last_layer}, {"pool_last_qkv", e->pool_last_qkv}, {"share_layer0", e->share_layer0}, {"bert_fuse_splitk_ln", e->bert_fuse_splitk_ln}, {"fuse_ln", e->fuse_ln}, {"resid16", e->resid16}, {"fold_ln", e->fold_ln},
+      {"dedup", e->dedup}, {"pool_last_layer", e->pool_last_layer}, {"pool_last_qkv", e->pool_last_qkv}, {"share_layer0", e->share_layer0}, {"embed_distinct", e->embed_distinct}, {"plan_fused", e->plan_fused}, {"bert_fuse_splitk_ln", e->bert_fuse_splitk_ln}, {"fuse_ln", e->fuse_ln}, {"resid16", e->resid16}, {"fold_ln", e->fold_ln},
       {"refine_samples", e->refine_samples}, {"refine_samples_step", e->refine_samples_step}, {"refine_theta_x1000", (int)lrintf(e->refine_theta_x * 1000.f)},
       {"refine_theta_gen_x1000", (int)lrintf(e->refine_theta_gen * 1000.f)},
       {"refine_guard_x1e6", (int)lrintf(e->refine_guard_dev * 1e6f)}, {"refine_gate_x1e6", (int)lrintf(e->refine_gate_delta * 1e6f)},
@@ -2968,6 +2991,18 @@
   if (n_dup) *n_dup = e->h_totals[HT_PLAN + 5];
   E_HIP(hipMemcpyAsync(out, feat, (size_t)n * e->cfg.clip_proj * 4, hipMemcpyDefault, e->st));
   E_HIP(hipStreamSynchronize(e->st));
+  return CZC_OK;
+}
+
+static int test_engine_buffer(void* engine, const char* name, size_t offset, size_t bytes, void* out) {
+  czc_engine* e = (czc_engine*)engine;
+  if (!e || !name || !out) return CZC_ERR_ARG;
+  E_HIP(hipSetDevice(e->dev));
+  const auto it = e->ws.find(name);
+  if (it == e->ws.end() || !it->second.p) return fail(e, CZC_ERR_ARG, "no workspace buffer %s", name);
+  if (offset > it->second.bytes || bytes > it->second.bytes - offset) return fail(e, CZC_ERR_ARG, "window outside workspace buffer %s", name);
+  E_HIP(hipStreamSynchronize(e->st));
+  E_HIP(hipMemcpy(out, (const char*)it->second.p + offset, bytes, hipMemcpyDeviceToHost));
   return CZC_OK;
 }
 
@@ -2992,7 +3027,8 @@
       &fluency_expand_tables, &launch_expand_mask_rows, &launch_logprob_target,
       &launch_bridge_rows, &launch_bridge_rows_hp, &launch_softmax_mask_topk_rows, &launch_softmax_mask_topk_rows_hp,
       &launch_softmax_mask_topk_rows_vocab,
-      []() -> int { return czc::g_gemm_family; }};
+      []() -> int { return czc::g_gemm_family; },
+      &test_engine_buffer, &launch_plan_fused, &launch_clip_embed_distinct};
   return abi == HOOKS_ABI ? &h : nullptr;
 }
 
diff --git a/conzic_amd/csrc/kernels.h b/conzic_amd/csrc/kernels.h
--- a/conzic_amd/csrc/kernels.h
+++ b/conzic_amd/csrc/kernels.h
@@ -78,6 +78,8 @@
 int launch_clip_embed(const int* ids, int ids_stride, const int* seg_src, const int* seg_pos0, const int* own_off,
                       const int* own_len, int n_seg, int max_len, int H, const float* tok, const float* pos, float* x,
                       hipStream_t st, int x16 = 0, float* stat = nullptr, float eps = 0.f);
+int launch_clip_embed_distinct(const int2* dsrc, int n_dist, const int* rowmap, int M, int H, const float* tok, const float* pos,
+                               void* xg, float* sg, void* x, float* stat, float eps, hipStream_t st);
 int launch_ln_finalize(const float* part, long part_ld, int nblk, int M, float eps, float* stat, hipStream_t st);
 int launch_fold_ln(const float* W, const float* gamma, const float* beta, const float* b, int N, int K, void* Wf16, float* rowsum, float* bf,
                    hipStream_t st);
@@ -205,7 +207,10 @@
                        int* rep = nullptr, int* n_dup_out = nullptr);
 int launch_layer0_count(const int* clip_ids, const int* own_len, const int* pre_len, int B, int K, int* dcount, int* total, hipStream_t st);
 int launch_layer0_map(const int* clip_ids, const int* own_off, const int* own_len, const int* pre_len, const int* dcount, int B, int K,
-                      int* rowmap, int* dist, hipStream_t st);
+                      int* rowmap, int* dist, hipStream_t st, int2* dsrc = nullptr);
+int launch_plan_fused(const int* clip_ids, const int* clip_len, int B, int K, int share, int* own_len, int* pre_len, int* seg_src,
+                      int* seg_pos0, int* own_off, int* pre_off, int* eos_idx, int* img_max, int* rep, int* rel, int* img_rows,
+                      int* dcount, int* totals, hipStream_t st);
 int launch_prefix_finish(const int* own_off, const int* own_len, int B, int K, int* pre_off, int* eos_idx,
                          int* n_trunk_rows, hipStream_t st, const int* rep = nullptr);
 
@@ -272,7 +277,7 @@
                           int* rank, int* nonfinite, hipStream_t st);
 int launch_pll_sum(const float* logp, int R, int Lmax, const int* len_of_row, float* pll, hipStream_t st);
 
-constexpr int HOOKS_ABI = 0x060d;
+constexpr int HOOKS_ABI = 0x060e;
 struct Hooks {
   char* (*err_buf)();
   decltype(&launch_gemm) gemm;
@@ -338,6 +343,9 @@
   decltype(&launch_softmax_mask_topk_rows_hp) softmax_mask_topk_rows_hp;
   decltype(&launch_softmax_mask_topk_rows_vocab) softmax_mask_topk_rows_vocab;
   int (*gemm_family)();
+  int (*engine_buffer)(void* engine, const char* name, size_t offset, size_t bytes, void* out);
+  decltype(&launch_plan_fused) plan_fused;
+  decltype(&launch_clip_embed_distinct) clip_embed_distinct;
 };
 
 }
diff --git a/conzic_amd/csrc/rowops.hip b/conzic_amd/csrc/rowops.hip
--- a/conzic_amd/csrc/rowops.hip
+++ b/conzic_amd/csrc/rowops.hip
@@ -372,6 +372,36 @@
   return 0;
 }
 
+__device__ __forceinline__ void clip_embed_row16(const float* tr, const float* pr, int H, int lane, f16_t* xh, float* st, float eps) {
+  float sm = 0.f;
+  float4 keep[LN_MAXV];
+#pragma unroll
+  for (int t = 0; t < LN_MAXV; ++t) {
+    const int c = lane * 4 + t * 256;
+    keep[t] = make_float4(0.f, 0.f, 0.f, 0.f);
+    if (c < H) {
+      const float4 a = *(const float4*)(tr + c), b = *(const float4*)(pr + c);
+      const uint2 pk = make_uint2(pack2_f16(a.x + b.x, a.y + b.y), pack2_f16(a.z + b.z, a.w + b.w));
+      *(uint2*)(xh + c) = pk;
+      keep[t] = make_float4(f16lo(pk.x), f16hi(pk.x), f16lo(pk.y), f16hi(pk.y));
+      sm += (keep[t].x + keep[t].y) + (keep[t].z + keep[t].w);
+    }
+  }
+  if (st) {
+    const float mean = wave_sum(sm) / (float)H;
+    float q = 0.f;
+#pragma unroll
+    for (int t = 0; t < LN_MAXV; ++t) {
+      if (lane * 4 + t * 256 < H) {
+        const float a = keep[t].x - mean, b = keep[t].y - mean, c2 = keep[t].z - mean, d = keep[t].w - mean;
+        q += (a * a + b * b) + (c2 * c2 + d * d);
+      }
+    }
+    const float rstd = rsqrtf(wave_sum(q) / (float)H + eps);
+    if (lane == 0) *(float2*)st = make_float2(mean, rstd);
+  }
+}
+
 __global__ __launch_bounds__(256) void clip_embed_kernel(const int* ids, int ids_stride, const int* seg_src,
                                                          const int* seg_pos0, const int* own_off, const int* own_len,
                                                          int n_seg, int max_len, int H, const float* tok,
@@ -385,34 +415,7 @@
   const float* tr = tok + (long)id * H;
   const float* pr = pos + (long)p * H;
   if (x16) {
-    f16_t* xh = (f16_t*)x + ((long)own_off[s] + i) * H;
-    float sm = 0.f;
-    float4 keep[LN_MAXV];
-#pragma unroll
-    for (int t = 0; t < LN_MAXV; ++t) {
-      const int c = lane * 4 + t * 256;
-      keep[t] = make_float4(0.f, 0.f, 0.f, 0.f);
-      if (c < H) {
-        const float4 a = *(const float4*)(tr + c), b = *(const float4*)(pr + c);
-        const uint2 pk = make_uint2(pack2_f16(a.x + b.x, a.y + b.y), pack2_f16(a.z + b.z, a.w + b.w));
-        *(uint2*)(xh + c) = pk;
-        keep[t] = make_float4(f16lo(pk.x), f16hi(pk.x), f16lo(pk.y), f16hi(pk.y));
-        sm += (keep[t].x + keep[t].y) + (keep[t].z + keep[t].w);
-      }
-    }
-    if (stat) {
-      const float mean = wave_sum(sm) / (float)H;
-      float q = 0.f;
-#pragma unroll
-      for (int t = 0; t < LN_MAXV; ++t) {
-        if (lane * 4 + t * 256 < H) {
-          const float a = keep[t].x - mean, b = keep[t].y - mean, c2 = keep[t].z - mean, d = keep[t].w - mean;
-          q += (a * a + b * b) + (c2 * c2 + d * d);
-        }
-      }
-      const float rstd = rsqrtf(wave_sum(q) / (float)H + eps);
-      if (lane == 0) *(float2*)(stat + ((long)own_off[s] + i) * 2) = make_float2(mean, rstd);
-    }
+    clip_embed_row16(tr, pr, H, lane, (f16_t*)x + ((long)own_off[s] + i) * H, stat ? stat + ((long)own_off[s] + i) * 2 : nullptr, eps);
     return;
   }
   float* xr = x + ((long)own_off[s] + i) * H;
@@ -433,6 +436,42 @@
   dim3 grid(cdiv((long)n_seg * max_len, 4)), block(256);
   hipLaunchKernelGGL(clip_embed_kernel, grid, block, 0, st, ids, ids_stride, seg_src, seg_pos0, own_off, own_len, n_seg,
                      max_len, H, tok, pos, x, x16, stat, eps);
+  CZC_HIP_CHECK(hipGetLastError());
+  return 0;
+}
+
+__global__ __launch_bounds__(256) void clip_embed_distinct_kernel(const int2* dsrc, int n_dist, int H, const float* tok, const float* pos,
+                                                                  f16_t* xg, float* sg, float eps) {
+  const int lane = threadIdx.x & 63;
+  const int c = blockIdx.x * 4 + (threadIdx.x >> 6);
+  if (c >= n_dist) return;
+  const int2 ip = dsrc[c];
+  clip_embed_row16(tok + (long)ip.x * H, pos + (long)ip.y * H, H, lane, xg + (long)c * H, sg + (long)c * 2, eps);
+}
+
+__global__ __launch_bounds__(256) void clip_embed_spread_kernel(const unsigned char* xg, const float2* sg, const int* rowmap, int M,
+                                                                int row_bytes, unsigned char* x, float2* stat) {
+  const int lane = threadIdx.x & 63;
+  const int r = blockIdx.x * 4 + (threadIdx.x >> 6);
+  if (r >= M) return;
+  const int c = rowmap[r];
+  const unsigned char* s = xg + (long)c * row_bytes;
+  unsigned char* d = x + (long)r * row_bytes;
+  for (int o = lane * 16; o < row_bytes; o += 1024) *(uint4*)(d + o) = *(const uint4*)(s + o);
+  if (lane == 0) stat[r] = sg[c];
+}
+
+int launch_clip_embed_distinct(const int2* dsrc, int n_dist, const int* rowmap, int M, int H, const float* tok, const float* pos,
+                               void* xg, float* sg, void* x, float* stat, float eps, hipStream_t st) {
+  if (n_dist <= 0 || M <= 0) return 0;
+  if (H <= 0 || H % 8 || H > LN_MAXV * 256) {
+    snprintf(g_err, sizeof(g_err), "clip_embed_distinct: unsupported H=%d", H);
+    return 1;
+  }
+  hipLaunchKernelGGL(clip_embed_distinct_kernel, dim3(cdiv(n_dist, 4)), dim3(256), 0, st, dsrc, n_dist, H, tok, pos, (f16_t*)xg, sg, eps);
+  CZC_HIP_CHECK(hipGetLastError());
+  hipLaunchKernelGGL(clip_embed_spread_kernel, dim3(cdiv(M, 4)), dim3(256), 0, st, (const unsigned char*)xg, (const float2*)sg, rowmap, M,
+                     H * 2, (unsigned char*)x, (float2*)stat);
   CZC_HIP_CHECK(hipGetLastError());
   return 0;
 }
diff --git a/conzic_amd/native.py b/conzic_amd/native.py
--- a/conzic_amd/native.py
+++ b/conzic_amd/native.py
@@ -163,6 +163,9 @@
     "czc_test_attention_mapped": (_I, [_I, _I, _I, _I, C.c_float, _P, _P, _P, _I, _P, _P]),
     "czc_test_layer0_plan": (_I, [_I, _I, _P, _P, _I, _P, _P, _P, _P, _I, _P, _I, _P]),
     "czc_test_text_tower": (_I, [_P, _I, _I, _P, _P, _P, _P]),
+    "czc_test_engine_buffer": (_I, [_P, C.c_char_p, C.c_size_t, C.c_size_t, _P]),
+    "czc_test_plan_chain": (_I, [_I] * 6 + [_P] * 13),
+    "czc_test_embed_rows": (_I, [_I, _I, _I, _P, _P, _I, _I, _I, _I, _P, _P, C.c_float, _I, _I, _P, _P, _P, _P, _P, _P]),
     "czc_test_topk": (_I, [_I, _I, _I, _P, _P, C.c_float, _I, _I, _P, _P, _P]),
     "czc_test_bridge": (_I, [C.POINTER(BridgeTables), C.POINTER(Config), _I, _I, _P, _P, _P]),
     "czc_test_combine": (_I, [_I, _I, _I, _P, _P, C.c_float, _P, _P, _P, C.POINTER(Hyper), _P, _P, _P, _P]),
```
